# 07350100647/nvbio-gpl

Measured on AMD Instinct MI355X. Metric: aligned reads/sec (150 bp single-end, 3 Gbp ref); GCUPS of the banded extend pass in `extend`, higher is better.
Workload: dtype u32 (FM-index coordinates) / i16x2 (band-31 DP, two alignments per 32-bit lane: 16-bit integer scores, held in binary16 lanes where every score is an integer of magnitude <= 2040 -- exact -- and in int16 lanes otherwise; bound-checked on the host)

## Files before the change

### include/nvbio_amd.h

```cpp
#ifndef NVBIO_AMD_H
#define NVBIO_AMD_H

#include <stdint.h>

#ifdef __cplusplus
extern "C" {
#endif

#define NVBIO_AMD_VERSION 100

typedef enum
{
    NVBIO_OK              = 0,
    NVBIO_ERR_INVALID     = 1,
    NVBIO_ERR_HIP         = 2,
    NVBIO_ERR_NOMEM       = 3,
    NVBIO_ERR_UNSUPPORTED = 4,
    NVBIO_ERR_NO_DEVICE   = 5
} nvbio_status;

int         nvbio_amd_version(void);
const char* nvbio_amd_last_error(void);
nvbio_status nvbio_amd_device_count(int* count);
nvbio_status nvbio_amd_device_arch(int device, char* name, uint32_t name_len);
// ... 350 lines not shown
nvbio_status nvbio_best_approx_init(int device, uint32_t n_reads, int32_t worst_score, int32_t* best_dev, uint8_t* best_rc_dev, void* stream);
nvbio_status nvbio_read_queue_begin(int device, const uint32_t* queue_dev, uint32_t n, uint32_t read_len, uint32_t first_offset, uint32_t top_seed,
                                    uint32_t max_effort_init, uint32_t* seed_offsets_dev, uint32_t* active_dev, uint32_t* trys_dev, void* stream);
nvbio_status nvbio_read_queue_filter(int device, const uint32_t* queue_dev, uint32_t n, const uint8_t* read_flags_dev, uint32_t* queue_out_dev,
                                     uint32_t* count_dev, void* stream);

typedef struct
{
    const uint32_t* read_offsets_dev;
    const uint32_t* seed_intervals_dev;
    uint32_t        seeds_per_read;
    uint32_t        seeding_pass;
    uint32_t        max_reseed;
    uint32_t        seed_len;
    uint32_t        min_read_len;
} nvbio_ragged_seed_layout;

nvbio_status nvbio_read_queue_begin_ragged(int device, const uint32_t* queue_dev, uint32_t n, const nvbio_ragged_seed_layout* layout, uint32_t n_symbols,
                                           uint32_t top_seed, uint32_t max_effort_init, uint32_t* seed_offsets_dev, uint32_t* active_dev, uint32_t* trys_dev,
                                           void* stream);
nvbio_status nvbio_seed_hits_map_ragged(int device, const nvbio_uint2* fw_ranges_dev, const nvbio_uint2* rc_ranges_dev, const uint32_t* read_queue_dev,
                                        uint32_t n_reads, const nvbio_ragged_seed_layout* layout, uint32_t max_hits, uint32_t rep_seeds,
                                        nvbio_uint2* deques_dev, uint32_t* sizes_dev, uint8_t* reseed_dev, void* stream);
nvbio_status nvbio_best_approx_init_ragged(int device, uint32_t n_reads, const int32_t* min_scores_dev, int32_t* best_dev, uint8_t* best_rc_dev, void* stream);
nvbio_status nvbio_score_reduce_effort_ragged(int device, const uint32_t* active_dev, const nvbio_hit_queues* hits, const uint32_t* read_offsets_dev,
                                              uint32_t n_ext, const nvbio_seed_hits_params* params, int32_t* best_dev, uint8_t* best_rc_dev,
                                              uint32_t* trys_dev, uint32_t* sizes_dev, void* stream);
nvbio_status nvbio_score_reduce_effort_multi_ragged(int device, const uint32_t* active_dev, uint32_t n_active, const uint32_t* hits_first_dev,
                                                    const uint32_t* hits_count_dev, const nvbio_hit_queues* hits, const uint32_t* read_offsets_dev,
                                                    uint32_t n_ext, const nvbio_seed_hits_params* params, int32_t* best_dev, uint8_t* best_rc_dev,
                                                    uint32_t* trys_dev, uint32_t* sizes_dev, void* stream);

typedef struct
{
    uint32_t seeds_per_read;
    uint32_t first_offset;
    uint32_t seed_interval;
    uint32_t seed_len;
    uint32_t read_len;
} nvbio_all_hits_params;

nvbio_status nvbio_all_hits_scan_temp_bytes(uint32_t n_reads, uint32_t seeds_per_read, uint64_t* bytes);
nvbio_status nvbio_all_hits_scan(int device, const nvbio_uint2* fw_ranges_dev, const nvbio_uint2* rc_ranges_dev, uint32_t n_reads,
                                 const nvbio_all_hits_params* params, uint64_t* slots_dev, uint64_t* n_hits_dev, void* temp_dev, uint64_t temp_bytes,
                                 void* stream);

nvbio_status nvbio_all_hits_select(int device, const nvbio_uint2* fw_ranges_dev, const nvbio_uint2* rc_ranges_dev, uint32_t n_reads,
                                   const nvbio_all_hits_params* params, const uint64_t* slots_dev, uint64_t begin, uint64_t end,
                                   const nvbio_hit_queues* hits, void* stream);

nvbio_status nvbio_all_hits_unique_temp_bytes(uint32_t n, uint64_t* bytes);
nvbio_status nvbio_all_hits_unique(int device, const nvbio_hit_queues* hits, const nvbio_hit_queues* hits_out, uint32_t* n_out_dev, void* temp_dev,
                                   uint64_t temp_bytes, void* stream);

nvbio_status nvbio_all_score_output_temp_bytes(uint32_t n, uint64_t* bytes);
nvbio_status nvbio_all_score_output(int device, const nvbio_hit_queues* hits, const int32_t* scores_dev, int32_t min_score, uint32_t* out_read_id_dev,
                                    uint8_t* out_rc_dev, uint32_t* out_loc_dev, int32_t* out_score_dev, uint64_t out_offset, uint64_t out_capacity,
                                    uint64_t* count_dev, void* temp_dev, uint64_t temp_bytes, void* stream);

nvbio_status nvbio_all_traceback_flatten(int device, const uint32_t* rec_read_id_dev, const uint8_t* rec_rc_dev, const uint32_t* rec_loc_dev, uint32_t n,
                                         const uint32_t* read_index_dev, uint32_t band_len, uint32_t genome_len, uint32_t reads_reversed,
                                         uint32_t* read_id_dev, uint8_t* flags_dev, uint32_t* win_begin_dev, uint32_t* win_end_dev, void* stream);

typedef struct
{
    uint32_t anchor;
    uint32_t anchor_len, opposite_len;
    int32_t  anchor_perfect_score, opposite_perfect_score;
    int32_t  anchor_min_score, opposite_min_score;
    int32_t  score_limit;
    int32_t  worst_score;
    int32_t  match, txt_gap_open, txt_gap_ext;
    uint32_t band, genome_len;
    uint32_t policy, min_frag_len, max_frag_len, overlap, unpaired;
    uint32_t max_effort, min_ext, max_ext;
} nvbio_pe_params;
nvbio_status nvbio_pe_init(int device, uint32_t n_reads, int32_t worst_score_mate1, int32_t worst_score_mate2, int32_t* best_a_dev, int32_t* best_o_dev, void* stream);
nvbio_status nvbio_pe_anchor_flatten(int device, const nvbio_pe_params* params, const nvbio_hit_queues* hits, const int32_t* best_a_dev, const int32_t* best_o_dev,
                                     uint32_t* read_id_dev, uint8_t* flags_dev, uint32_t* win_begin_dev, uint32_t* win_end_dev, int32_t* min_scores_dev,
                                     void* stream);
nvbio_status nvbio_pe_anchor_output(int device, const nvbio_pe_params* params, const nvbio_hit_queues* hits, const int32_t* scores_dev, const nvbio_uint2* sinks_dev,
                                    const uint32_t* win_begin_dev, const int32_t* min_scores_dev, int32_t* hit_opposite_score_dev, uint8_t* valid_dev,
                                    void* stream);
nvbio_status nvbio_pe_opposite_flatten(int device, const nvbio_pe_params* params, const uint32_t* queue_dev, uint32_t n, const nvbio_hit_queues* hits,
                                       const int32_t* best_a_dev, const int32_t* best_o_dev, uint32_t* read_id_dev, uint8_t* flags_dev,
                                       uint32_t* win_begin_dev, uint32_t* win_end_dev, int32_t* min_scores_dev, void* stream);
nvbio_status nvbio_pe_opposite_output(int device, const nvbio_pe_params* params, const uint32_t* queue_dev, uint32_t n, const int32_t* scores_dev,
                                      const nvbio_uint2* sinks_dev, const uint32_t* win_begin_dev, const uint32_t* win_end_dev, const int32_t* min_scores_dev,
                                      int32_t* hit_opposite_score_dev, uint32_t* hit_opposite_loc_dev, uint32_t* hit_opposite_sink_dev, void* stream);
nvbio_status nvbio_pe_score_reduce(int device, const nvbio_pe_params* params, const uint32_t* active_dev, uint32_t n_active, const uint32_t* hits_first_dev,
                                   const uint32_t* hits_count_dev, const nvbio_hit_queues* hits, const int32_t* hit_opposite_score_dev,
                                   const uint32_t* hit_opposite_loc_dev, const uint32_t* hit_opposite_sink_dev, uint32_t n_ext, int32_t* best_a_dev,
                                   int32_t* best_o_dev, uint32_t* trys_dev, uint32_t* sizes_dev, void* stream);
nvbio_status nvbio_select_flagged_indices(int device, const uint8_t* flags_dev, uint32_t n, uint32_t* queue_out_dev, uint32_t* count_dev, void* stream);

nvbio_status nvbio_text_2bit_le_to_be(int device, const uint32_t* in_dev, uint32_t n_words, uint32_t* out_dev, void* stream);
nvbio_status nvbio_scores_to_int16(int device, const int32_t* scores_dev, uint32_t n, int16_t* out_dev, void* stream);

typedef enum { NVBIO_GLOBAL = 0, NVBIO_LOCAL = 1, NVBIO_SEMI_GLOBAL = 2 } nvbio_alignment_type;

typedef struct
{
    int32_t match;
    int32_t mm_min, mm_max;
    int32_t pat_gap_open, pat_gap_ext;
    int32_t txt_gap_open, txt_gap_ext;
} nvbio_gotoh_scheme;

typedef struct
{
    int32_t match, mismatch, deletion, insertion;
} nvbio_sw_scheme;

#define NVBIO_SCORE_MIN (-(1 << 30))

typedef struct
{
    const void*     reads_dev;
    uint32_t        read_bits;
    const uint32_t* read_offsets_dev;
    const uint8_t*  quals_dev;
    const uint32_t* read_id_dev;
    const uint8_t*  flags_dev;
    const void*     text_dev;
    uint32_t        text_bits;
    const uint32_t* win_begin_dev;
    const uint32_t* win_end_dev;
    uint32_t        n;
    uint32_t        max_read_len;
    uint32_t        algo_flags;
} nvbio_alignment_batch;


enum
{
    NVBIO_ALN_NO_UNGAPPED_SCORE     = 1,
    NVBIO_ALN_NO_THIRD_CHANCE       = 2,
    NVBIO_ALN_NO_PACKED_DP          = 4,
    NVBIO_ALN_FORCE_PACKED_DP       = 8,
    NVBIO_ALN_NO_UNGAPPED_TRACEBACK = 16,
    NVBIO_ALN_PK_THREE_WAVES        = 32,
    NVBIO_ALN_NO_SECOND_CHANCE      = 128,
    NVBIO_ALN_NO_NARROW_SCORE       = 512,
    NVBIO_ALN_NO_BAND_ROUTE         = 1024,
    NVBIO_ALN_PK_STRIPE8            = 256,
    NVBIO_ALN_RAGGED_READS          = 4096,
    NVBIO_ALN_NO_LENGTH_SORT        = 8192,
    NVBIO_ALN_NO_QUALITY_SHORTCUT   = 2048,
    NVBIO_ALN_NO_GAP_CHANCE         = 65536,
    NVBIO_ALN_NO_COOPERATIVE_DP     = 32768,
    NVBIO_ALN_NO_F16_DP             = 16384,
    NVBIO_ALN_SPLIT_CHANCES         = 131072,
    NVBIO_ALN_NO_PAIRED_GAP_CHANCE  = 262144,
    NVBIO_ALN_NO_NARROW_TRACEBACK   = 64
};

enum { NVBIO_READ_REVERSE = 1, NVBIO_READ_COMPLEMENT = 2 };

nvbio_status nvbio_best_candidate_reduce(int device, const uint64_t* keys_dev, const int32_t* scores_dev, const nvbio_uint2* sinks_dev,
                                         const uint32_t* win_begin_dev, uint64_t n, uint64_t* best_dev, void* stream);

nvbio_status nvbio_best_candidate_unpack(int device, const uint64_t* best_dev, uint32_t n_reads, int32_t* scores_dev,
                                         int64_t* end_pos_dev, uint8_t* rc_dev, void* stream);

nvbio_status nvbio_best_candidate_windows(int device, const uint64_t* keys_dev, const int32_t* scores_dev, const nvbio_uint2* sinks_dev,
                                          const uint32_t* win_begin_dev, uint64_t n, const uint64_t* best_dev, int64_t* best_wb_dev,
                                          int64_t* best_locus_dev, void* stream);

nvbio_status nvbio_traceback_best_batch(int device, const uint64_t* best_dev, const int64_t* best_wb_dev, uint32_t n_reads, uint32_t read_len,
                                        uint32_t band, uint32_t genome_len, int32_t min_score, uint8_t* flags_dev, uint32_t* win_begin_dev,
                                        uint32_t* win_end_dev, int32_t* scores_dev, nvbio_uint2* sinks_dev, void* stream);

nvbio_status nvbio_second_candidate_reduce(int device, const uint64_t* keys_dev, const int32_t* scores_dev, const nvbio_uint2* sinks_dev,
                                           const uint32_t* win_begin_dev, uint64_t n, const uint64_t* best_dev,
                                           uint32_t distinct_dist, int32_t worst_score, uint64_t* second_dev, void* stream);

typedef struct
{
    int32_t version;
    int32_t monotone;
    int32_t perfect_score;
    int32_t min_score;
} nvbio_mapq_params;
nvbio_status nvbio_mapq(int device, const uint64_t* best_dev, const uint64_t* second_dev, uint32_t n_reads,
                        const nvbio_mapq_params* params, int32_t* second_scores_dev, uint8_t* mapq_dev, void* stream);

nvbio_status nvbio_finish_reads_tiles_per_group(uint32_t reads_per_tile, uint32_t* tiles_per_group);
nvbio_status nvbio_finish_reads(int device, const uint64_t* keys_dev, const int32_t* scores_dev, const nvbio_uint2* sinks_dev,
                                const uint32_t* win_begin_dev, uint64_t n, const uint32_t* tile_offsets_dev, uint32_t n_tiles,
                                uint32_t reads_per_tile, uint32_t n_reads, uint32_t distinct_dist, int32_t worst_score,
                                const nvbio_mapq_params* params, int32_t match, const uint32_t* read_offsets_dev, const int32_t* min_scores_dev,
                                uint64_t* best_dev, uint64_t* second_dev, int32_t* scores_out_dev, int64_t* end_pos_dev, uint8_t* rc_dev,
                                uint8_t* mapq_dev, int32_t* second_scores_dev, uint32_t* status_dev, void* stream);

enum { NVBIO_PE_POLICY_FF = 0, NVBIO_PE_POLICY_FR = 1, NVBIO_PE_POLICY_RF = 2, NVBIO_PE_POLICY_RR = 3 };
nvbio_status nvbio_opposite_mate_windows(int device, const uint32_t* g_pos_dev, const uint8_t* anchor_rc_dev, uint32_t n,
                                         uint32_t anchor_len, uint32_t opposite_gapped_len, uint32_t anchor, uint32_t policy,
                                         uint32_t min_frag_len, uint32_t max_frag_len, uint32_t overlap, uint32_t genome_len,
                                         uint32_t* win_begin_dev, uint32_t* win_end_dev, uint8_t* flags_dev, uint8_t* valid_dev,
                                         void* stream);

#define NVBIO_GAP_PAIR_MAX_SHIFT 5
nvbio_status nvbio_banded_gap_pairs(int device, const nvbio_alignment_batch* batch, uint32_t* partner_dev, void* stream);

nvbio_status nvbio_banded_gotoh_score(int device, uint32_t band, nvbio_alignment_type type,
                                      const nvbio_gotoh_scheme* scheme, const nvbio_alignment_batch* batch,
                                      int32_t* scores_dev, nvbio_uint2* sinks_dev, void* stream);

nvbio_status nvbio_banded_gotoh_score_staged(int device, uint32_t band, nvbio_alignment_type type,
                                             const nvbio_gotoh_scheme* scheme, const nvbio_alignment_batch* batch,
                                             const int32_t* min_scores_dev, int32_t min_score,
                                             int32_t* scores_dev, nvbio_uint2* sinks_dev, void* stream);

enum { NVBIO_TRACEBACK_SINKS_GIVEN = 1 };
nvbio_status nvbio_banded_gotoh_traceback_temp_bytes(const nvbio_alignment_batch* batch_host_sizes, uint32_t band, uint64_t* bytes);
nvbio_status nvbio_banded_gotoh_traceback(int device, uint32_t band, nvbio_alignment_type type,
                                          const nvbio_gotoh_scheme* scheme, const nvbio_alignment_batch* batch,
                                          int32_t* scores_dev, nvbio_uint2* sources_dev, nvbio_uint2* sinks_dev,
                                          uint16_t* cigars_dev, uint32_t cigar_stride, uint32_t* cigar_lens_dev,
                                          uint32_t flags, void* temp_dev, uint64_t temp_bytes, void* stream);

nvbio_status nvbio_banded_sw_traceback(int device, uint32_t band, nvbio_alignment_type type,
                                       const nvbio_sw_scheme* scheme, const nvbio_alignment_batch* batch,
                                       int32_t* scores_dev, nvbio_uint2* sources_dev, nvbio_uint2* sinks_dev,
                                       uint16_t* cigars_dev, uint32_t cigar_stride, uint32_t* cigar_lens_dev,
                                       uint32_t flags, void* temp_dev, uint64_t temp_bytes, void* stream);

nvbio_status nvbio_full_gotoh_traceback_temp_bytes(const nvbio_alignment_batch* batch_host_sizes, uint32_t max_pattern_len,
                                                   uint32_t max_text_len, uint64_t* bytes);
nvbio_status nvbio_full_gotoh_traceback(int device, nvbio_alignment_type type, const nvbio_gotoh_scheme* scheme,
                                        const nvbio_alignment_batch* batch, uint32_t max_pattern_len, uint32_t max_text_len,
                                        const int32_t* min_scores_dev,
                                        int32_t* scores_dev, nvbio_uint2* sources_dev, nvbio_uint2* sinks_dev,
                                        uint16_t* cigars_dev, uint32_t cigar_stride, uint32_t* cigar_lens_dev,
                                        uint32_t flags, void* temp_dev, uint64_t temp_bytes, void* stream);

nvbio_status nvbio_full_sw_traceback(int device, nvbio_alignment_type type, const nvbio_sw_scheme* scheme,
                                     const nvbio_alignment_batch* batch, uint32_t max_pattern_len, uint32_t max_text_len,
                                     const int32_t* min_scores_dev,
                                     int32_t* scores_dev, nvbio_uint2* sources_dev, nvbio_uint2* sinks_dev,
                                     uint16_t* cigars_dev, uint32_t cigar_stride, uint32_t* cigar_lens_dev,
                                     uint32_t flags, void* temp_dev, uint64_t temp_bytes, void* stream);

nvbio_status nvbio_finish_alignment(int device, const nvbio_alignment_batch* batch, const nvbio_uint2* sources_dev,
                                    const uint16_t* cigars_dev, uint32_t cigar_stride, const uint32_t* cigar_lens_dev,
                                    uint32_t* ed_dev, uint8_t* mds_dev, uint32_t mds_stride, uint32_t* mds_lens_dev, void* stream);

nvbio_status nvbio_full_gotoh_temp_bytes(const nvbio_alignment_batch* batch_host_sizes, uint32_t max_pattern_len,
                                         uint32_t max_text_len, int text_blocking, uint64_t* bytes);
nvbio_status nvbio_full_gotoh_score(int device, nvbio_alignment_type type, int text_blocking,
                                    const nvbio_gotoh_scheme* scheme, const nvbio_alignment_batch* batch,
                                    uint32_t max_pattern_len, uint32_t max_text_len,
                                    const int32_t* min_scores_dev, int32_t* scores_dev, nvbio_uint2* sinks_dev,
                                    void* temp_dev, uint64_t temp_bytes, void* stream);

nvbio_status nvbio_banded_myers_score(int device, uint32_t band, nvbio_alignment_type type, const nvbio_alignment_batch* batch, int32_t min_score,
                                      int32_t* scores_dev, nvbio_uint2* sinks_dev, void* stream);

nvbio_status nvbio_banded_gotoh_score_best2(int device, uint32_t band, nvbio_alignment_type type,
                                            const nvbio_gotoh_scheme* scheme, const nvbio_alignment_batch* batch, uint32_t distinct_dist,
                                            int32_t* scores_dev, nvbio_uint2* sinks_dev, int32_t* scores2_dev, nvbio_uint2* sinks2_dev,
                                            void* stream);
nvbio_status nvbio_full_gotoh_score_best2(int device, nvbio_alignment_type type, int text_blocking,
                                          const nvbio_gotoh_scheme* scheme, const nvbio_alignment_batch* batch,
                                          uint32_t max_pattern_len, uint32_t max_text_len, const int32_t* min_scores_dev,
                                          uint32_t distinct_dist, int32_t* scores_dev, nvbio_uint2* sinks_dev,
                                          int32_t* scores2_dev, nvbio_uint2* sinks2_dev, void* stream);

nvbio_status nvbio_banded_sw_score(int device, uint32_t band, nvbio_alignment_type type,
                                   const nvbio_sw_scheme* scheme, const nvbio_alignment_batch* batch,
                                   int32_t* scores_dev, nvbio_uint2* sinks_dev, void* stream);
nvbio_status nvbio_full_sw_score(int device, nvbio_alignment_type type, int text_blocking,
                                 const nvbio_sw_scheme* scheme, const nvbio_alignment_batch* batch,
                                 uint32_t max_pattern_len, uint32_t max_text_len,
                                 const int32_t* min_scores_dev, int32_t* scores_dev, nvbio_uint2* sinks_dev,
                                 void* temp_dev, uint64_t temp_bytes, void* stream);

#ifdef __cplusplus
}
#endif
#endif
```

### nvbio-gpl_amd/__init__.py

```python
import ctypes
import os

import numpy as np

_HERE = os.path.dirname(os.path.abspath(__file__))
LIB_PATH = os.path.join(_HERE, "lib", "libnvbio_amd.so")
HEADER_PATH = os.path.join(os.path.dirname(_HERE), "include", "nvbio_amd.h")

GLOBAL, LOCAL, SEMI_GLOBAL = 0, 1, 2
SCORE_MIN = -(1 << 30)
FM_SCAN_FORWARD, FM_COMPLEMENT, FM_NO_KMER_TABLE, FM_NO_VERIFY, FM_COUNT_SECTORS, FM_NO_PIPELINE, FM_DEFER_HEAVY = 1, 2, 4, 8, 16, 32, 64
FM_TABLE_NO_DIRECT, FM_TABLE_NO_CONTEXT, FM_TABLE_NO_GROUPS, FM_TABLE_CANONICAL, FM_TABLE_CANONICAL_WIDE = 1, 2, 4, 8, 16
READ_REVERSE, READ_COMPLEMENT = 1, 2
TRACEBACK_SINKS_GIVEN = 1
ALN_NO_UNGAPPED_SCORE, ALN_NO_THIRD_CHANCE, ALN_NO_PACKED_DP, ALN_FORCE_PACKED_DP, ALN_NO_UNGAPPED_TRACEBACK, ALN_PK_THREE_WAVES = 1, 2, 4, 8, 16, 32
ALN_NO_NARROW_TRACEBACK, ALN_NO_SECOND_CHANCE, ALN_PK_STRIPE8, ALN_NO_NARROW_SCORE, ALN_NO_BAND_ROUTE = 64, 128, 256, 512, 1024
ALN_NO_QUALITY_SHORTCUT, ALN_RAGGED_READS, ALN_NO_LENGTH_SORT, ALN_NO_F16_DP, ALN_NO_COOPERATIVE_DP, ALN_NO_GAP_CHANCE = 2048, 4096, 8192, 16384, 32768, 65536
ALN_SPLIT_CHANCES, ALN_NO_PAIRED_GAP_CHANCE = 131072, 262144
DEFAULT_ALGO_FLAGS = 0
BACKTRACK_REFERENCE_QUIRKS = 1

_STATUS = {0: "OK", 1: "INVALID", 2: "HIP", 3: "NOMEM", 4: "UNSUPPORTED", 5: "NO_DEVICE"}


class NvbioError(RuntimeError):
    def __init__(self, status, msg):
        super().__init__("nvbio_amd: %s: %s" % (_STATUS.get(status, status), msg))
        self.status = status


class _View(ctypes.Structure):
    _fields_ = [("length", ctypes.c_uint32), ("primary", ctypes.c_uint32), ("L2", ctypes.c_uint32 * 5),
                ("bwt_occ_dev", ctypes.c_void_p), ("bwt_occ_words", ctypes.c_uint64),
                ("ssa_dev", ctypes.c_void_p), ("ssa_words", ctypes.c_uint64), ("sa_int", ctypes.c_uint32)]


class _BuildOptions(ctypes.Structure):
    _fields_ = [("kmer_len", ctypes.c_uint32), ("sa_int", ctypes.c_uint32), ("max_lcp", ctypes.c_uint32),
                ("verify", ctypes.c_uint32), ("table_flags", ctypes.c_uint32), ("bucket_symbols", ctypes.c_uint32)]


class _StringSet(ctypes.Structure):
    _fields_ = [("symbols_dev", ctypes.c_void_p), ("symbol_bits", ctypes.c_uint32),
                ("offsets_dev", ctypes.c_void_p), ("offsets_are_ranges", ctypes.c_uint32),
                ("fixed_len", ctypes.c_uint32), ("stride", ctypes.c_uint32), ("n", ctypes.c_uint32),
                ("seeds_per_string", ctypes.c_uint32), ("seed_interval", ctypes.c_uint32),
                ("seed_intervals_dev", ctypes.c_void_p)]


class _Scheme(ctypes.Structure):
    _fields_ = [("match", ctypes.c_int32), ("mm_min", ctypes.c_int32), ("mm_max", ctypes.c_int32),
                ("pat_gap_open", ctypes.c_int32), ("pat_gap_ext", ctypes.c_int32),
                ("txt_gap_open", ctypes.c_int32), ("txt_gap_ext", ctypes.c_int32)]


class _SWScheme(ctypes.Structure):
    _fields_ = [("match", ctypes.c_int32), ("mismatch", ctypes.c_int32), ("deletion", ctypes.c_int32),
                ("insertion", ctypes.c_int32)]


class _Batch(ctypes.Structure):
    _fields_ = [("reads_dev", ctypes.c_void_p), ("read_bits", ctypes.c_uint32),
                ("read_offsets_dev", ctypes.c_void_p), ("quals_dev", ctypes.c_void_p),
                ("read_id_dev", ctypes.c_void_p), ("flags_dev", ctypes.c_void_p),
                ("text_dev", ctypes.c_void_p), ("text_bits", ctypes.c_uint32),
                ("win_begin_dev", ctypes.c_void_p), ("win_end_dev", ctypes.c_void_p), ("n", ctypes.c_uint32),
                ("max_read_len", ctypes.c_uint32), ("algo_flags", ctypes.c_uint32)]


class _HitQueues(ctypes.Structure):
    _fields_ = [("idx_queue_dev", ctypes.c_void_p), ("hit_read_id_dev", ctypes.c_void_p), ("hit_seed_dev", ctypes.c_void_p),
                ("hit_loc_dev", ctypes.c_void_p), ("hit_score_dev", ctypes.c_void_p), ("hit_sink_dev", ctypes.c_void_p),
                ("n", ctypes.c_uint32)]


class _SeedHitsParams(ctypes.Structure):
    _fields_ = [(n, ctypes.c_uint32) for n in ("seeds_per_read", "first_offset", "seed_interval", "seed_len", "read_len", "max_hits",
                                                "rep_seeds", "max_effort", "min_ext", "max_ext")]


class _RaggedSeedLayout(ctypes.Structure):
    _fields_ = [("read_offsets_dev", ctypes.c_void_p), ("seed_intervals_dev", ctypes.c_void_p)] + \
               [(n, ctypes.c_uint32) for n in ("seeds_per_read", "seeding_pass", "max_reseed", "seed_len", "min_read_len")]


class _RankDict(ctypes.Structure):
    _fields_ = [("text_dev", ctypes.c_void_p), ("word_bits", ctypes.c_uint32), ("occ_dev", ctypes.c_void_p), ("index_bits", ctypes.c_uint32),
                ("K", ctypes.c_uint32), ("length", ctypes.c_uint64)]


_lib = None


def lib():
    global _lib
    if _lib is None:
        if not os.path.exists(LIB_PATH):
            raise NvbioError(5, "%s is missing: build it with __graft_entry__.build() "
                                "(there is no CPU fallback)" % LIB_PATH)
        import torch
        L = ctypes.CDLL(LIB_PATH)
        L.nvbio_amd_last_error.restype = ctypes.c_char_p
        L.nvbio_amd_version.restype = ctypes.c_int
        _lib = L
    return _lib


def release_scratch():
    _check(lib().nvbio_amd_release_scratch())


def set_scratch_check(enable, fill_byte=0):
    _check(lib().nvbio_amd_set_scratch_check(ctypes.c_int(1 if enable else 0), ctypes.c_uint32(fill_byte)))


def scratch_check_report():
    buf = ctypes.create_string_buffer(1 << 16)
    _check(lib().nvbio_amd_scratch_check_report(buf, ctypes.c_uint64(len(buf))))
    out = {}
    for line in buf.value.decode().splitlines():
        tag, checked, damaged, sub, off = line.split()
        out[tag] = (int(checked), int(damaged), None if sub == "-" else int(sub), None if off == "-" else int(off))
    return out


def _check(status):
    if status != 0:
        raise NvbioError(status, lib().nvbio_amd_last_error().decode())


def _torch():
    import torch
    return torch


_SCRATCH = {}


def _scratch(device, nbytes, cap=8 << 30):
    torch = _torch()
    nbytes = int(min(max(nbytes, 1 << 20), cap))
    key = str(device)
    t = _SCRATCH.get(key)
    if t is None or t.numel() < nbytes:
        _SCRATCH[key] = None
        t = _SCRATCH[key] = torch.empty(nbytes, dtype=torch.uint8, device=device)
    return t


def _ptr(t):
    return None if t is None else ctypes.c_void_p(t.data_ptr())


def _stream_ptr(device):
    torch = _torch()
    return ctypes.c_void_p(torch.cuda.current_stream(device).cuda_stream)


def device_count():
    n = ctypes.c_int(0)
    lib().nvbio_amd_device_count(ctypes.byref(n))
    return n.value


def _dev_tensor(a, dtype, device):
    torch = _torch()
    if a is None:
        return None
    if isinstance(a, torch.Tensor):
        t = a
        if t.dtype != dtype:
# ... 733 lines not shown
        cols = 4 if self._index.IS_SET else 2
        if hits is None:
            hits = torch.empty((max(end - begin, 0), cols), dtype=torch.int32, device=self._index.device)
        if end > begin:
            _check(lib().nvbio_qgram_filter_locate(self._index._h, _ptr(self._ranges), _ptr(self._slots), _ptr(self._indices),
                                                   ctypes.c_uint32(self._n_queries), ctypes.c_uint64(begin), ctypes.c_uint64(end), _ptr(hits),
                                                   _stream_ptr(self._index.device)))
        return hits

    def merge(self, interval, hits, is_set=None):
        torch = _torch()
        if is_set is None:
            is_set = hits.dim() == 2 and hits.shape[1] == 4
        dev = hits.device
        n = hits.shape[0]
        tb = ctypes.c_uint64(0)
        _check(lib().nvbio_qgram_filter_merge_temp_bytes(ctypes.c_int(1 if is_set else 0), ctypes.c_uint32(n), ctypes.byref(tb)))
        self._grow_temp(tb.value, dev)
        if self._merged is None or self._merged.shape[0] < max(n, 1) or self._merged.device != dev:
            self._merged = torch.empty((max(n, 1), 2), dtype=torch.int32, device=dev)
            self._counts = torch.empty(max(n, 1), dtype=torch.int32, device=dev)
        nm = ctypes.c_uint32(0)
        hits = hits.contiguous()
        _check(lib().nvbio_qgram_filter_merge(FMIndex._dev_index(dev), ctypes.c_int(1 if is_set else 0), ctypes.c_uint32(interval), _ptr(hits),
                                              ctypes.c_uint32(n), _ptr(self._merged), _ptr(self._counts), ctypes.byref(nm), _ptr(self._temp),
                                              ctypes.c_uint64(self._temp.numel()), _stream_ptr(dev)))
        m = nm.value
        merged = self._merged.view(-1)[:2 * m].view(m, 2) if is_set else self._merged.view(-1)[:m]
        return merged.clone(), self._counts[:m].clone()


class GotohScheme:

    def __init__(self, match, mm_min, mm_max, pat_gap_open, pat_gap_ext, txt_gap_open, txt_gap_ext):
        self.c = _Scheme(match, mm_min, mm_max, pat_gap_open, pat_gap_ext, txt_gap_open, txt_gap_ext)


def SimpleGotohScheme(match, mismatch, gap_open, gap_ext):
    return GotohScheme(match, -mismatch, -mismatch, gap_open, gap_ext, gap_open, gap_ext)


def EditDistanceScheme():
    return GotohScheme(0, 1, 1, -1, -1, -1, -1)


class SimpleSmithWatermanScheme:

    def __init__(self, match, mismatch, deletion, insertion):
        self.c = _SWScheme(match, mismatch, deletion, insertion)


class SmithWatermanAligner:

    def __init__(self, type, scheme):
        self.type, self.sw = type, scheme
        c = scheme.c
        self.scheme = (GotohScheme(c.match, -c.mismatch, -c.mismatch, c.deletion, c.deletion, c.deletion, c.deletion)
                       if c.deletion == c.insertion else None)


def make_smith_waterman_aligner(type, scheme):
    return SmithWatermanAligner(type, scheme)


def make_edit_distance_aligner(type):
    return SmithWatermanAligner(type, SimpleSmithWatermanScheme(0, -1, -1, -1))


class GotohAligner:

    def __init__(self, type, scheme):
        self.type, self.scheme = type, scheme


def make_gotoh_aligner(type, scheme):
    return GotohAligner(type, scheme)


class AlignmentBatch:

    def __init__(self, reads, read_bits, read_offsets, text, text_bits, win_begin, win_end, quals=None, read_id=None,
                 flags=None, device="cuda:0", max_read_len=0, algo_flags=None):
        torch = _torch()
        self.device = device
        self.algo_flags = DEFAULT_ALGO_FLAGS if algo_flags is None else int(algo_flags)
        self.read_bits, self.text_bits = int(read_bits), int(text_bits)
        self.reads = _dev_tensor(reads, torch.uint8 if read_bits == 8 else torch.int32, device)
        self.read_offsets = _dev_tensor(read_offsets, torch.int32, device)
        self.text = _dev_tensor(text, torch.uint8 if text_bits == 8 else torch.int32, device)
        self.win_begin = _dev_tensor(win_begin, torch.int32, device)
        self.win_end = _dev_tensor(win_end, torch.int32, device)
        self.quals = _dev_tensor(quals, torch.uint8, device)
        self.read_id = _dev_tensor(read_id, torch.int32, device)
        self.flags = _dev_tensor(flags, torch.uint8, device)
        self.n = int(self.win_begin.numel())
        self.max_read_len = int(max_read_len)

    def size(self):
        return self.n

    def c_struct(self):
        return _Batch(_ptr(self.reads), self.read_bits, _ptr(self.read_offsets), _ptr(self.quals), _ptr(self.read_id),
                      _ptr(self.flags), _ptr(self.text), self.text_bits, _ptr(self.win_begin), _ptr(self.win_end),
                      self.n, self.max_read_len, self.algo_flags)


DEVICE_THREAD_SCHEDULER = "DeviceThreadScheduler"
DEVICE_STAGED_THREAD_SCHEDULER = "DeviceStagedThreadScheduler"


class BatchedBandedAlignmentScore:

    def __init__(self, band_len, aligner, scheduler=DEVICE_THREAD_SCHEDULER):
        self.band_len, self.aligner, self.scheduler = int(band_len), aligner, scheduler
        if scheduler not in (DEVICE_THREAD_SCHEDULER, DEVICE_STAGED_THREAD_SCHEDULER):
            raise NvbioError(1, "unknown scheduler %r" % (scheduler,))

    def min_temp_storage(self, max_pattern_len, max_text_len, stream_size):
        return 0

    max_temp_storage = min_temp_storage

    def enact(self, batch, scores=None, sinks=None, min_scores=None):
        torch = _torch()
        if scores is None:
            scores = torch.empty(batch.n, dtype=torch.int32, device=batch.device)
        if sinks is None:
            sinks = torch.empty((batch.n, 2), dtype=torch.int32, device=batch.device)
        bs = batch.c_struct()
        sw = getattr(self.aligner, "sw", None)
        if self.scheduler == DEVICE_STAGED_THREAD_SCHEDULER:
            if sw is not None:
                raise NvbioError(4, "the staged scheduler is instantiated for Gotoh aligners")
            per_job = min_scores is not None and not isinstance(min_scores, int)
            if per_job and (min_scores.dtype != torch.int32 or min_scores.numel() != batch.n):
                raise NvbioError(1, "min_scores: int32 per job")
            _check(lib().nvbio_banded_gotoh_score_staged(
                FMIndex._dev_index(batch.device), ctypes.c_uint32(self.band_len), ctypes.c_int(self.aligner.type),
                ctypes.byref(self.aligner.scheme.c), ctypes.byref(bs), _ptr(min_scores) if per_job else None,
                ctypes.c_int32(SCORE_MIN if min_scores is None else (0 if per_job else int(min_scores))),
                _ptr(scores), _ptr(sinks), _stream_ptr(batch.device)))
            return scores, sinks
        fn = lib().nvbio_banded_sw_score if sw is not None else lib().nvbio_banded_gotoh_score
        _check(fn(FMIndex._dev_index(batch.device), ctypes.c_uint32(self.band_len), ctypes.c_int(self.aligner.type),
                  ctypes.byref(sw.c if sw is not None else self.aligner.scheme.c),
                  ctypes.byref(bs), _ptr(scores), _ptr(sinks), _stream_ptr(batch.device)))
        return scores, sinks


def batch_banded_alignment_score(band_len, aligner, batch):
    return BatchedBandedAlignmentScore(band_len, aligner).enact(batch)


GAP_PAIR_MAX_SHIFT = 5
NO_PARTNER = 0xFFFFFFFF


def banded_gap_pairs(batch):
    torch = _torch()
    partner = torch.empty(batch.n, dtype=torch.int32, device=batch.device)
    bs = batch.c_struct()
    _check(lib().nvbio_banded_gap_pairs(FMIndex._dev_index(batch.device), ctypes.byref(bs), _ptr(partner), _stream_ptr(batch.device)))
    return partner


class BatchedBandedAlignmentTraceback:

    def __init__(self, band_len, aligner):
        self.band_len, self.aligner = int(band_len), aligner

    def min_temp_storage(self, batch):
        out = ctypes.c_uint64(0)
        bs = batch.c_struct()
        _check(lib().nvbio_banded_gotoh_traceback_temp_bytes(ctypes.byref(bs), ctypes.c_uint32(self.band_len), ctypes.byref(out)))
        return int(out.value)

    def enact(self, batch, cigar_stride=64, temp=None, scores=None, sinks=None):
        torch = _torch()
        n, dev = batch.n, batch.device
        given = scores is not None and sinks is not None
        if not given:
            scores = torch.empty(n, dtype=torch.int32, device=dev)
            sinks = torch.empty((n, 2), dtype=torch.int32, device=dev)
        sources = torch.empty((n, 2), dtype=torch.int32, device=dev)
        cigars = torch.zeros((n, cigar_stride), dtype=torch.int16, device=dev)
        lens = torch.empty(n, dtype=torch.int32, device=dev)
        bs = batch.c_struct()
        sw = getattr(self.aligner, "sw", None)
        fn = lib().nvbio_banded_sw_traceback if sw is not None else lib().nvbio_banded_gotoh_traceback
        _check(fn(
            FMIndex._dev_index(dev), ctypes.c_uint32(self.band_len), ctypes.c_int(self.aligner.type),
            ctypes.byref(sw.c if sw is not None else self.aligner.scheme.c), ctypes.byref(bs), _ptr(scores), _ptr(sources), _ptr(sinks), _ptr(cigars),
            ctypes.c_uint32(cigar_stride), _ptr(lens), ctypes.c_uint32(TRACEBACK_SINKS_GIVEN if given else 0), _ptr(temp),
            ctypes.c_uint64(0 if temp is None else temp.numel() * temp.element_size()), _stream_ptr(dev)))
        return scores, sources, sinks, cigars, lens


class BatchedAlignmentTraceback:

    def __init__(self, aligner):
        self.aligner = aligner

    def min_temp_storage(self, batch, max_pattern_len, max_text_len):
        out = ctypes.c_uint64(0)
        bs = batch.c_struct()
        _check(lib().nvbio_full_gotoh_traceback_temp_bytes(ctypes.byref(bs), ctypes.c_uint32(max_pattern_len),
                                                           ctypes.c_uint32(max_text_len), ctypes.byref(out)))
        return int(out.value)

    def enact(self, batch, max_pattern_len, max_text_len, min_scores=None, cigar_stride=64, temp=None, scores=None, sinks=None):
        torch = _torch()
        n, dev = batch.n, batch.device
        given = scores is not None and sinks is not None
        if not given:
            scores = torch.empty(n, dtype=torch.int32, device=dev)
            sinks = torch.empty((n, 2), dtype=torch.int32, device=dev)
        sources = torch.empty((n, 2), dtype=torch.int32, device=dev)
        cigars = torch.zeros((n, cigar_stride), dtype=torch.int16, device=dev)
        lens = torch.empty(n, dtype=torch.int32, device=dev)
        ms = _dev_tensor(min_scores, torch.int32, dev)
        bs = batch.c_struct()
        if temp is None and n:
            temp = _scratch(dev, self.min_temp_storage(batch, max_pattern_len, max_text_len))
        sw = getattr(self.aligner, "sw", None)
        fn = lib().nvbio_full_sw_traceback if sw is not None else lib().nvbio_full_gotoh_traceback
        _check(fn(
            FMIndex._dev_index(dev), ctypes.c_int(self.aligner.type), ctypes.byref(sw.c if sw is not None else self.aligner.scheme.c), ctypes.byref(bs),
            ctypes.c_uint32(max_pattern_len), ctypes.c_uint32(max_text_len), _ptr(ms), _ptr(scores), _ptr(sources), _ptr(sinks),
            _ptr(cigars), ctypes.c_uint32(cigar_stride), _ptr(lens), ctypes.c_uint32(TRACEBACK_SINKS_GIVEN if given else 0),
            _ptr(temp), ctypes.c_uint64(0 if temp is None else temp.numel() * temp.element_size()), _stream_ptr(dev)))
        return scores, sources, sinks, cigars, lens


def finish_alignment(batch, sources, cigars, cigar_lens, mds_stride=0):
    torch = _torch()
    n, dev = batch.n, batch.device
    ed = torch.empty(n, dtype=torch.int32, device=dev)
    mds = torch.zeros((n, mds_stride), dtype=torch.uint8, device=dev) if mds_stride else None
    ml = torch.empty(n, dtype=torch.int32, device=dev) if mds_stride else None
    bs = batch.c_struct()
    _check(lib().nvbio_finish_alignment(FMIndex._dev_index(dev), ctypes.byref(bs), _ptr(sources), _ptr(cigars), ctypes.c_uint32(cigars.shape[1]),
                                        _ptr(cigar_lens), _ptr(ed), _ptr(mds), ctypes.c_uint32(mds_stride), _ptr(ml), _stream_ptr(dev)))
    return ed, mds, ml


def cigar_string(cigar_row, length, forward=True):
    els = [int(c) & 0xFFFF for c in cigar_row[:length]]
    if forward:
        els = els[::-1]
    return "".join("%d%s" % (c >> 2, "MIDS"[c & 3]) for c in els)


class BatchedAlignmentScore:

    def __init__(self, aligner, text_blocking=True):
        self.aligner, self.text_blocking = aligner, bool(text_blocking)

    def enact(self, batch, max_pattern_len, max_text_len, min_scores=None, scores=None, sinks=None):
        torch = _torch()
        if scores is None:
            scores = torch.empty(batch.n, dtype=torch.int32, device=batch.device)
        if sinks is None:
            sinks = torch.empty((batch.n, 2), dtype=torch.int32, device=batch.device)
        ms = _dev_tensor(min_scores, torch.int32, batch.device)
        bs = batch.c_struct()
        sw = getattr(self.aligner, "sw", None)
        fn = lib().nvbio_full_sw_score if sw is not None else lib().nvbio_full_gotoh_score
        rows = max_pattern_len if self.text_blocking else max_text_len
        temp = _scratch(batch.device, batch.n * max(rows, 1) * 4)
        _check(fn(FMIndex._dev_index(batch.device), ctypes.c_int(self.aligner.type),
                  ctypes.c_int(1 if self.text_blocking else 0),
                  ctypes.byref(sw.c if sw is not None else self.aligner.scheme.c), ctypes.byref(bs),
                  ctypes.c_uint32(max_pattern_len), ctypes.c_uint32(max_text_len), _ptr(ms),
                  _ptr(scores), _ptr(sinks), _ptr(temp), ctypes.c_uint64(temp.numel()), _stream_ptr(batch.device)))
        return scores, sinks


def batch_banded_alignment_score_best2(band_len, aligner, batch, distinct_dist=0):
    torch = _torch()
    sc = [torch.empty(batch.n, dtype=torch.int32, device=batch.device) for _ in range(2)]
    sk = [torch.empty((batch.n, 2), dtype=torch.int32, device=batch.device) for _ in range(2)]
    bs = batch.c_struct()
    _check(lib().nvbio_banded_gotoh_score_best2(FMIndex._dev_index(batch.device), ctypes.c_uint32(band_len), ctypes.c_int(aligner.type),
                                                ctypes.byref(aligner.scheme.c), ctypes.byref(bs), ctypes.c_uint32(distinct_dist),
                                                _ptr(sc[0]), _ptr(sk[0]), _ptr(sc[1]), _ptr(sk[1]), _stream_ptr(batch.device)))
    return sc[0], sk[0], sc[1], sk[1]


def batch_alignment_score_best2(aligner, batch, max_pattern_len, max_text_len, distinct_dist=0, text_blocking=False, min_scores=None):
    torch = _torch()
    sc = [torch.empty(batch.n, dtype=torch.int32, device=batch.device) for _ in range(2)]
    sk = [torch.empty((batch.n, 2), dtype=torch.int32, device=batch.device) for _ in range(2)]
    ms = _dev_tensor(min_scores, torch.int32, batch.device)
    bs = batch.c_struct()
    _check(lib().nvbio_full_gotoh_score_best2(FMIndex._dev_index(batch.device), ctypes.c_int(aligner.type), ctypes.c_int(1 if text_blocking else 0),
                                              ctypes.byref(aligner.scheme.c), ctypes.byref(bs), ctypes.c_uint32(max_pattern_len),
                                              ctypes.c_uint32(max_text_len), _ptr(ms), ctypes.c_uint32(distinct_dist),
                                              _ptr(sc[0]), _ptr(sk[0]), _ptr(sc[1]), _ptr(sk[1]), _stream_ptr(batch.device)))
    return sc[0], sk[0], sc[1], sk[1]


def hits_to_diagonals(hits, seeds_per_read, seed_interval, seed_len, read_len, strand):
    torch = _torch()
    keys = torch.empty(hits.shape[0], dtype=torch.int64, device=hits.device)
    _check(lib().nvbio_hits_to_diagonals(FMIndex._dev_index(hits.device), _ptr(hits), ctypes.c_uint64(hits.shape[0]),
                                         ctypes.c_uint32(seeds_per_read), ctypes.c_uint32(seed_interval),
# ... 503 lines not shown
```

### nvbio-gpl_amd/csrc/gotoh_banded.hip

```cpp
#include "gotoh_common.h"
#include "bitplanes.h"
#include <hipcub/hipcub.hpp>
#include <stdlib.h>

namespace nvbio_amd {

template <int BAND, int TYPE, int RBITS, int TBITS, bool BEST2 = false, bool STAGED = false>
__global__ void __launch_bounds__(128)
banded_gotoh_kernel(const BatchDev b, const SchemeDev sc, int32_t* __restrict__ scores, uint2* __restrict__ sinks,
                    const uint32_t distinct_dist, int32_t* __restrict__ scores2, uint2* __restrict__ sinks2,
                    const int32_t* __restrict__ min_scores, const int32_t min_score_all)
{
    __shared__ int32_t s_mm[64];
    if (threadIdx.x < 64) s_mm[threadIdx.x] = mismatch_score( sc, threadIdx.x );
    __syncthreads();

    const uint32_t job = blockIdx.x * blockDim.x + threadIdx.x;
    if (job >= b.n) return;

    const uint32_t rid   = b.read_id ? b.read_id[job] : job;
    const uint32_t first = b.read_offsets[rid];
    const uint32_t M     = b.read_offsets[rid + 1] - first;
    const uint32_t fl    = b.flags ? b.flags[job] : 0u;
    const bool     rev   = (fl & NVBIO_READ_REVERSE) != 0;
// ... 34 lines not shown
    }

    const int32_t G_o = sc.pat_go, G_e = sc.pat_ge;
    const int32_t I_o = sc.ins_go, I_e = sc.ins_ge;
    const int32_t infimum = -32768 - max2( max2( G_o, G_e ), max2( sc.txt_go, sc.txt_ge ) );
    const int32_t V = sc.match;

    int32_t H[BAND], F[BAND];
    H[0] = 0;
    #pragma unroll
    for (int j = 1; j < BAND; ++j) H[j] = (TYPE == NVBIO_GLOBAL) ? sc.txt_go + (j - 1) * sc.txt_ge : 0;
    #pragma unroll
    for (int j = 0; j < BAND; ++j) F[j] = infimum;

    bool stopped = false;
    const int32_t min_score = STAGED ? (min_scores ? min_scores[job] : min_score_all) : 0;
    for (uint32_t i = 0; i < M; ++i)
    {
        if (STAGED && i && (i & 31u) == 0u)
        {
            int32_t mx = H[0];
            #pragma unroll
            for (int j = 1; j < BAND; ++j) mx = max2( mx, H[j] );
            const int32_t thr = (int32_t)((uint32_t)min_score + (M - i) * (uint32_t)V);
            if (mx < thr) { stopped = true; break; }
            #pragma unroll
            for (int j = 0; j < BAND; ++j)
            {
                H[j] = (int32_t)(int16_t)max2( H[j], -32768 + 32 );
                F[j] = (int32_t)(int16_t)max2( F[j], -32768 + 32 );
            }
        }
        const uint32_t pidx = rev ? first + M - 1u - i : first + i;
        uint32_t q = prd.get( pidx );
        if (comp && q < 4u) q = 3u - q;
        const uint32_t qq = b.quals ? b.quals[pidx] : 0u;
        const int32_t  S  = s_mm[qq < 63u ? qq : 63u];

        const uint32_t g_new = (i + (uint32_t)(BAND - 1) < N) ? trd.get( tb + i + (BAND - 1) ) : 255u;

        uint64_t eq_bits = 0;
        if (PACKED)
        {
            if (q < 4u)
            {
                const uint64_t t = cache_bits ^ ((uint64_t)q * 0x5555555555555555ull);
                eq_bits = ~(t | (t >> 1)) & 0x5555555555555555ull;
            }
        }

        int32_t E = 0;
        int32_t row_key = -1;
        #pragma unroll
        for (int j = 0; j < BAND; ++j)
        {
            const int32_t f = (j < BAND - 1) ? max2( F[j + 1] + G_e, H[j + 1] + G_o ) : infimum;
            F[j] = f;

            bool eq;
            if (j == BAND - 1)   eq = (g_new == q);
            else if (PACKED)     eq = ((eq_bits >> (2 * j)) & 1ull) != 0;
            else                 eq = (cache_raw[j] == q);
            const int32_t d = H[j] + (eq ? V : S);

            int32_t h;
            if (j == 0)             h = max2( f, d );
            else if (j == BAND - 1) h = max2( E, d );
            else                    h = max3( f, E, d );
            if (TYPE == NVBIO_LOCAL)
            {
                h = max2( h, 0 );
                if (BEST2) report2( h, i + (uint32_t)j + 1u, i + 1u );
                else       row_key = max2( row_key, (h << 5) | j );
            }
            H[j] = h;
            E = (j == 0) ? h + I_o : max2( h + I_o, E + I_e );
        }

        if (PACKED) cache_bits = (cache_bits >> 2) | ((uint64_t)(g_new & 3u) << (2 * (BAND - 2)));
        else
        {
            #pragma unroll
            for (int j = 0; j < BAND - 2; ++j) cache_raw[j] = cache_raw[j + 1];
            cache_raw[BAND - 2] = g_new;
        }

        if (TYPE == NVBIO_LOCAL && !BEST2)
        {
            const int32_t h = row_key >> 5;
            if (h >= best) { best = h; best_x = i + (uint32_t)(row_key & 31) + 1u; best_y = i + 1u; }
        }
    }

    if (STAGED && stopped) {  }
    else if (TYPE == NVBIO_GLOBAL)
    {
        if (BEST2) report2( H[BAND - 1], M + BAND - 1, M );
        else if (best <= H[BAND - 1]) { best = H[BAND - 1]; best_x = M + BAND - 1; best_y = M; }
    }
    else if (TYPE == NVBIO_SEMI_GLOBAL)
    {
        const uint32_t mb = M + (uint32_t)(BAND - 1);
        const uint32_t m  = (mb < N ? mb : N) - (M - 1u);
        #pragma unroll
        for (int j = 0; j < BAND; ++j)
            if (j == 0 || (uint32_t)j < m)
            {
                if (BEST2) report2( H[j], M + j, M );
                else if (best <= H[j]) { best = H[j]; best_x = M + j; best_y = M; }
            }
    }
    scores[job] = best;
    sinks[job]  = make_uint2( best_x, best_y );
    if (BEST2) { scores2[job] = sec; sinks2[job] = make_uint2( sec_x, sec_y ); }
}

typedef short    v2s __attribute__((ext_vector_type(2)));
typedef unsigned short v2u __attribute__((ext_vector_type(2)));

__device__ __forceinline__ v2s pk(const int a, const int b) { v2s r; r.x = (short)a; r.y = (short)b; return r; }
__device__ __forceinline__ v2s pk_max(const v2s a, const v2s b) { return __builtin_elementwise_max( a, b ); }
__device__ __forceinline__ v2s pk_from_bits(const uint32_t u) { return __builtin_bit_cast( v2s, u ); }
typedef _Float16 v2h __attribute__((ext_vector_type(2)));
__device__ __forceinline__ v2h pk_max(const v2h a, const v2h b) { return __builtin_elementwise_maximum( a, b ); }
__device__ __forceinline__ v2s pk_max3(const v2s a, const v2s b, const v2s c) { return pk_max( pk_max( a, b ), c ); }
__device__ __forceinline__ v2h pk_max3(const v2h a, const v2h b, const v2h c) { return __builtin_elementwise_maximum( __builtin_elementwise_maximum( a, b ), c ); }
template <typename V> __device__ __forceinline__ V pk_of(const int a, const int b);
template <> __device__ __forceinline__ v2s pk_of<v2s>(const int a, const int b) { return pk( a, b ); }
template <> __device__ __forceinline__ v2h pk_of<v2h>(const int a, const int b) { v2h r; r.x = (_Float16)a; r.y = (_Float16)b; return r; }
template <bool FP> struct PkLanes { typedef v2s type; };
template <> struct PkLanes<true> { typedef v2h type; };

__device__ __forceinline__ uint32_t funnel32(const uint32_t a, const uint32_t b, const uint32_t bit)
{
    const uint32_t sh = bit & 31u;
    return sh ? ((a << sh) | (b >> (32u - sh))) : a;
}
__device__ __forceinline__ uint32_t clamp_u32(const int64_t v, const uint32_t lo, const uint32_t hi)
{
    return v < (int64_t)lo ? lo : (v > (int64_t)hi ? hi : (uint32_t)v);
}

__device__ __forceinline__ uint32_t even_bits64(uint64_t x)
{
    x &= 0x5555555555555555ull;
    x = (x | (x >> 1)) & 0x3333333333333333ull;
    x = (x | (x >> 2)) & 0x0F0F0F0F0F0F0F0Full;
    x = (x | (x >> 4)) & 0x00FF00FF00FF00FFull;
    x = (x | (x >> 8)) & 0x0000FFFF0000FFFFull;
    x = (x | (x >> 16));
    return (uint32_t)x;
}

template <int TYPE, int RBITS, int MINW = 3, bool M0 = false, bool RAGGED = false, bool FP = false>
__global__ void __launch_bounds__(128) __attribute__((amdgpu_waves_per_eu(MINW, 3)))
banded_gotoh_band31_pk_kernel(const BatchDev b, const SchemeDev sc, int32_t* __restrict__ scores, uint2* __restrict__ sinks,
                              const uint32_t* __restrict__ job_list, const uint32_t* __restrict__ job_count)
{
    constexpr int BAND = 31;
    constexpr uint32_t RMASK = (1u << RBITS) - 1u;
    static_assert( !FP || (M0 && TYPE != NVBIO_LOCAL), "the binary16 build: match = 0, GLOBAL / SEMI_GLOBAL" );
    typedef typename PkLanes<FP>::type v2;
    __shared__ int32_t s_mm[64];
    if (threadIdx.x < 64) s_mm[threadIdx.x] = mismatch_score( sc, threadIdx.x );
    __syncthreads();

    const uint32_t n_jobs = job_list ? *job_count : b.n;
    const uint32_t pair = blockIdx.x * blockDim.x + threadIdx.x;
    if (2u * pair >= n_jobs) return;
    const uint32_t* __restrict__ rwords = (const uint32_t*)b.reads;
    const uint32_t* __restrict__ twords = (const uint32_t*)b.text;

    uint32_t first[2], M[2], tb[2], N[2], rows_all[2], out_id[2];
    bool     rev[2], comp[2], valid[2];
    #pragma unroll
    for (int u = 0; u < 2; ++u)
    {
        const uint32_t slot = 2u * pair + u;
        valid[u] = slot < n_jobs;
        const uint32_t ss  = valid[u] ? slot : 2u * pair;
        const uint32_t jj  = job_list ? job_list[ss] : ss;
        out_id[u] = jj;
        const uint32_t rid = b.read_id ? b.read_id[jj] : jj;
        first[u] = b.read_offsets[rid];
        M[u]     = b.read_offsets[rid + 1] - first[u];
        const uint32_t fl = b.flags ? b.flags[jj] : 0u;
        rev[u]  = (fl & NVBIO_READ_REVERSE) != 0;
        comp[u] = (fl & NVBIO_READ_COMPLEMENT) != 0;
        tb[u]   = b.win_begin[jj];
        N[u]    = (b.max_read_len && M[u] > b.max_read_len) ? 0u : b.win_end[jj] - tb[u];
        rows_all[u] = (valid[u] && N[u] >= M[u]) ? M[u] : 0u;
    }

    uint32_t r_lo[2], r_hi[2], t_lo[2], t_hi[2];
    #pragma unroll
    for (int u = 0; u < 2; ++u)
    {
        r_lo[u] = (uint32_t)(((uint64_t)first[u] * RBITS) >> 5);
        r_hi[u] = (uint32_t)(((uint64_t)(first[u] + (M[u] ? M[u] - 1u : 0u)) * RBITS) >> 5);
        t_lo[u] = tb[u] >> 4;
        t_hi[u] = (tb[u] + (N[u] ? N[u] - 1u : 0u)) >> 4;
    }

    auto read_chunk_start = [&](const int u, const uint32_t r0) -> int64_t {
        return rev[u] ? (int64_t)first[u] + (int64_t)M[u] - 1 - (int64_t)r0 - 7 : (int64_t)first[u] + r0;
    };
    auto read_chunk_start_at = [&](const int u, const int64_t r0) -> int64_t {
        return rev[u] ? (int64_t)first[u] + (int64_t)M[u] - 1 - r0 - 7 : (int64_t)first[u] + r0;
    };

    const uint32_t qadj = (uint32_t)((uintptr_t)b.quals & 3u);
    const uint32_t* __restrict__ qwords = (const uint32_t*)((uintptr_t)b.quals - qadj);
    const bool has_quals = (b.quals != nullptr);

    const v2 GO = pk_of<v2>( sc.pat_go, sc.pat_go ), GE = pk_of<v2>( sc.pat_ge, sc.pat_ge );
    const v2 INF = pk_of<v2>( -16384, -16384 ), ZERO = pk_of<v2>( 0, 0 );
    const v2s K32 = pk( 32, 32 );
    const int V = sc.match;
    const int S_noq = s_mm[0];
    uint32_t cx[2], lim[2];
    #pragma unroll
    for (int u = 0; u < 2; ++u)
    {
        cx[u]  = comp[u] ? 3u : 0u;
        lim[u] = N[u] > (uint32_t)(BAND - 1) ? N[u] - (uint32_t)(BAND - 1) : 0u;
    }

    int32_t  best[2]   = { NVBIO_SCORE_MIN, NVBIO_SCORE_MIN };
    uint32_t best_x[2] = { 0xFFFFFFFFu, 0xFFFFFFFFu }, best_y[2] = { 0xFFFFFFFFu, 0xFFFFFFFFu };

    const bool want0 = valid[0] && N[0] >= M[0], want1 = valid[1] && N[1] >= M[1];
    const bool split = (TYPE != NVBIO_LOCAL) && !RAGGED && want0 && want1 && M[0] != M[1];
    const uint32_t rows_max = rows_all[0] > rows_all[1] ? rows_all[0] : rows_all[1];
    uint32_t pad[2] = { 0u, 0u };
    if (RAGGED && TYPE != NVBIO_LOCAL) { pad[0] = rows_max - rows_all[0]; pad[1] = rows_max - rows_all[1]; }

    for (int pass = 0; pass < (split ? 2 : 1); ++pass)
    {
        uint32_t rows_u[2];
        rows_u[0] = (split && pass != 0) ? 0u : rows_all[0];
        rows_u[1] = (split && pass != 1) ? 0u : rows_all[1];
        const uint32_t rows = rows_u[0] > rows_u[1] ? rows_u[0] : rows_u[1];

        uint32_t c0[2], c1[2], c0i[2] = { 0, 0 }, c1i[2] = { 0, 0 };
        #pragma unroll
        for (int u = 0; u < 2; ++u)
        {
            const uint32_t w  = tb[u] >> 4;
            const uint32_t w0 = twords[clamp_u32( w,      t_lo[u], t_hi[u] )];
            const uint32_t w1 = twords[clamp_u32( w + 1u, t_lo[u], t_hi[u] )];
            const uint32_t w2 = twords[clamp_u32( w + 2u, t_lo[u], t_hi[u] )];
            const uint32_t bit = (tb[u] & 15u) * 2u;
            const uint64_t hi = ((uint64_t)funnel32( w0, w1, bit ) << 32) | funnel32( w1, w2, bit );
            uint64_t c = hi & ~0xFull;
            if (N[u] < 30u) c |= (~0ull >> (2u * N[u])) & ~0xFull;
            c0[u] = even_bits64( c ) >> 2;
            c1[u] = even_bits64( c >> 1 ) >> 2;
            if (RAGGED) { c0i[u] = c0[u]; c1i[u] = c1[u]; }
        }

        uint32_t ra[2], rb[2], ta[2], tbw[2];
        uint32_t qa[2] = { 0, 0 }, qb[2] = { 0, 0 }, qc[2] = { 0, 0 };
        auto issue_loads = [&](const uint32_t r0) {
            if (has_quals)
            {
                #pragma unroll
                for (int u = 0; u < 2; ++u)
                {
                    const int64_t qw  = ((RAGGED ? read_chunk_start_at( u, (int64_t)r0 - pad[u] ) : read_chunk_start( u, r0 )) + qadj) >> 2;
                    const uint32_t lo = (first[u] + qadj) >> 2, hi = (first[u] + qadj + (M[u] ? M[u] - 1u : 0u)) >> 2;
                    qa[u] = qwords[clamp_u32( qw,     lo, hi )];
                    qb[u] = qwords[clamp_u32( qw + 1, lo, hi )];
                    qc[u] = qwords[clamp_u32( qw + 2, lo, hi )];
                }
            }
            #pragma unroll
            for (int u = 0; u < 2; ++u)
            {
                const int64_t  rbit = (RAGGED ? read_chunk_start_at( u, (int64_t)r0 - pad[u] ) : read_chunk_start( u, r0 )) * RBITS;
                const int64_t  rw   = rbit >> 5;
                ra[u]  = rwords[clamp_u32( rw,     r_lo[u], r_hi[u] )];
                rb[u]  = rwords[clamp_u32( rw + 1, r_lo[u], r_hi[u] )];
                const int64_t  tw   = RAGGED ? (((int64_t)tb[u] + (int64_t)r0 - pad[u] + (BAND - 1)) >> 4)
                                             : (int64_t)(((uint64_t)tb[u] + r0 + (BAND - 1)) >> 4);
                ta[u]  = twords[clamp_u32( tw,     t_lo[u], t_hi[u] )];
                tbw[u] = twords[clamp_u32( tw + 1, t_lo[u], t_hi[u] )];
            }
        };
        issue_loads( 0 );

        v2 H[BAND], Hg[BAND], F[BAND];
        #pragma unroll
        for (int j = 0; j < BAND; ++j)
        {
            const int h0 = (TYPE == NVBIO_GLOBAL && j > 0) ? sc.txt_go + (j - 1) * sc.txt_ge : 0;
            H[j] = pk_of<v2>( h0, h0 ); F[j] = INF; Hg[j] = H[j] + GO;
        }

        for (uint32_t r0 = 0; r0 < rows; r0 += 8u)
        {
            uint32_t rchunk[2], tchunk[2], tchunk1[2]; int rsh[2], rstep[2];
            uint64_t qchunk[2] = { 0, 0 }; int qsh[2], qstep[2];
            #pragma unroll
            for (int u = 0; u < 2; ++u)
            {
                if (has_quals)
                {
                    const uint32_t bs = ((uint32_t)(((RAGGED ? read_chunk_start_at( u, (int64_t)r0 - pad[u] ) : read_chunk_start( u, r0 )) + qadj) & 3)) * 8u;
                    const uint32_t lo = bs ? ((qa[u] >> bs) | (qb[u] << (32u - bs))) : qa[u];
                    const uint32_t hi = bs ? ((qb[u] >> bs) | (qc[u] << (32u - bs))) : qb[u];
                    qchunk[u] = ((uint64_t)hi << 32) | lo;
                }
                qsh[u] = rev[u] ? 56 : 0; qstep[u] = rev[u] ? -8 : 8;
                const int64_t rbit = (RAGGED ? read_chunk_start_at( u, (int64_t)r0 - pad[u] ) : read_chunk_start( u, r0 )) * RBITS;
                rchunk[u] = funnel32( ra[u], rb[u], (uint32_t)(rbit & 31) );
                rsh[u]    = rev[u] ? (32 - RBITS) - 7 * RBITS : (32 - RBITS);
                rstep[u]  = rev[u] ? RBITS : -RBITS;
                const uint32_t tsym = RAGGED ? (uint32_t)(((int64_t)tb[u] + (int64_t)r0 - pad[u] + (BAND - 1)) & 15)
                                             : (uint32_t)(((uint64_t)tb[u] + r0 + (BAND - 1)) & 15u);
                uint32_t tc = funnel32( ta[u], tbw[u], tsym * 2u );
                const int64_t kk = RAGGED ? (int64_t)N[u] - (int64_t)(BAND - 1) - ((int64_t)r0 - pad[u]) : (int64_t)N[u] - (int64_t)(BAND - 1) - (int64_t)r0;
                if (kk < 16) tc |= (kk <= 0) ? 0xFFFFFFFFu : (0xFFFFFFFFu >> (2u * (uint32_t)kk));
                tchunk[u]  = tc;
                tchunk1[u] = tc << 1;
            }
            if (r0 + 8u < rows) issue_loads( r0 + 8u );

            const uint32_t r_end = (r0 + 8u < rows) ? 8u : rows - r0;
            for (uint32_t t = 0; t < r_end; ++t)
            {
                const uint32_t i = r0 + t;
                if (RAGGED && TYPE != NVBIO_LOCAL)
                {
                    const bool s0 = pad[0] != 0u && i == pad[0], s1 = pad[1] != 0u && i == pad[1];
                    if (s0 || s1)
                    {
                        #pragma unroll
                        for (int j = 0; j < BAND; ++j)
                        {
                            const int h0 = (TYPE == NVBIO_GLOBAL && j > 0) ? sc.txt_go + (j - 1) * sc.txt_ge : 0;
                            const v2 hh = pk_of<v2>( h0, h0 ), hhg = pk_of<v2>( h0 + sc.pat_go, h0 + sc.pat_go );
                            if (s0) { H[j].x = hh.x; F[j].x = INF.x; Hg[j].x = hhg.x; }
                            if (s1) { H[j].y = hh.y; F[j].y = INF.y; Hg[j].y = hhg.y; }
                        }
                        if (s0) { c0[0] = c0i[0]; c1[0] = c1i[0]; }
                        if (s1) { c0[1] = c0i[1]; c1[1] = c1i[1]; }
                    }
                }
                uint32_t nq[2]; int S[2];
                if (has_quals)
                {
                    #pragma unroll
                    for (int u = 0; u < 2; ++u)
                    {
                        const uint32_t ql = (uint32_t)(qchunk[u] >> qsh[u]) & 0xFFu; qsh[u] += qstep[u];
                        S[u] = s_mm[ql < 63u ? ql : 63u];
                    }
                }
                else S[0] = S[1] = S_noq;
                #pragma unroll
                for (int u = 0; u < 2; ++u)
                {
                    const uint32_t q = ((rchunk[u] >> rsh[u]) & RMASK) ^ cx[u]; rsh[u] += rstep[u];
                    c1[u] = __builtin_amdgcn_alignbit( c1[u], tchunk[u],  31 );
                    c0[u] = __builtin_amdgcn_alignbit( c0[u], tchunk1[u], 31 );
                    tchunk[u] <<= 2; tchunk1[u] <<= 2;
                    uint32_t x = (c0[u] ^ (0u - (q & 1u))) | (c1[u] ^ (0u - ((q >> 1) & 1u)));
                    if (RBITS > 2 && q >= 4u) x = 0xFFFFFFFFu;
                    if (i >= (RAGGED ? lim[u] + pad[u] : lim[u])) x |= 1u;
                    nq[u] = x;
                }
                const uint32_t NWa = __builtin_amdgcn_perm( nq[1], nq[0], 0x05040100u );
                const uint32_t NWb = __builtin_amdgcn_perm( nq[1], nq[0], 0x07060302u );

                const v2 SS = FP ? pk_of<v2>( S[0] * 128, S[1] * 128 ) : pk_of<v2>( S[0], S[1] );
                const v2 SD = pk_of<v2>( S[0] - V, S[1] - V );
                const v2 VV = pk_of<v2>( V, V );
                auto flags_at = [&](const int j) -> uint32_t {
                    const uint32_t w = (j < 15) ? NWb : NWa;
                    const int bit = (j < 15) ? 14 - j : 30 - j;
                    const int to  = FP ? 13 : 0;
                    return bit >= to ? w >> (bit - to) : w << (to - bit);
                };
                auto flags_in = [&](const uint32_t q) -> v2 { return __builtin_bit_cast( v2, q & (FP ? 0x20002000u : 0x00010001u) ); };
                auto flags_of = [&](const int j) -> v2 { return flags_in( flags_at( j ) ); };
                auto diag_of = [&](const v2 h, const v2 t) -> v2 {
                    if (FP) return __builtin_bit_cast( v2, __builtin_elementwise_fma( __builtin_bit_cast( v2h, t ), __builtin_bit_cast( v2h, SS ), __builtin_bit_cast( v2h, h ) ) );
                    return M0 ? h + t * SS : (h + VV) + t * SD;
                };

                v2 E = ZERO, a = ZERO, tt, ff = INF, dd = ZERO;
                v2s key = pk( -1, -1 );
                {
                    const v2 x  = F[1] + GE;
                    const v2 t0 = flags_of( 0 );
                    const v2 d  = diag_of( H[0], t0 );
                    const v2 f  = pk_max( x, Hg[1] );
                    F[0] = f;
                    if (FP) { ff = f; dd = d; tt = ZERO; }
                    else
                    {
                        tt = pk_max( f, d );
                        if (TYPE == NVBIO_LOCAL) tt = pk_max( tt, ZERO );
                    }
                }
                #pragma unroll
                for (int j = 0; j < BAND; ++j)
                {
                    constexpr int Z = 0;
                    const int j1 = j + 1, j2 = j + 2;
                    v2 x = INF, d = ZERO, f = INF, t1 = ZERO, tn = ZERO, an = ZERO;
                    uint32_t q1 = 0;
                    if (j2 < BAND) x  = F[j2] + GE;
                    __builtin_amdgcn_sched_barrier( Z );
                    const v2 h = FP ? ((j == 0) ? pk_max( ff, dd ) : pk_max3( ff, dd, E )) : ((j == 0) ? tt : pk_max( tt, E ));
                    if (j1 < BAND) q1 = flags_at( j1 );
                    __builtin_amdgcn_sched_barrier( Z );
                    const v2 hg = h + GO;
                    if (!FP && j1 < BAND) t1 = flags_in( q1 );
                    if (j2 < BAND) f  = pk_max( x, Hg[j2] );
                    __builtin_amdgcn_sched_barrier( Z );
                    const v2 En = (j == 0) ? hg : pk_max( hg, a );
                    if (FP) __builtin_amdgcn_sched_barrier( Z );
                    if (FP && j1 < BAND) t1 = flags_in( q1 );
                    if (j1 < BAND) d  = diag_of( H[j1], t1 );
                    __builtin_amdgcn_sched_barrier( Z );
                    if (j1 < BAND) an = En + GE;
                    if (TYPE == NVBIO_LOCAL) key = pk_max( key, __builtin_bit_cast( v2s, h ) * K32 + pk( j, j ) );
                    __builtin_amdgcn_sched_barrier( Z );
                    if (j1 < BAND)
                    {
                        if (FP) { ff = (j2 < BAND) ? f : d; dd = d; }
                        else
                        {
                            tn = (j2 < BAND) ? pk_max( f, d ) : d;
                            if (TYPE == NVBIO_LOCAL) tn = pk_max( tn, ZERO );
                        }
                        F[j1] = f;
                    }
                    H[j] = h; Hg[j] = hg;
                    E = En; a = an; tt = tn;
                    __builtin_amdgcn_sched_barrier( Z );
                }

                if (TYPE == NVBIO_LOCAL)
                {
                    const int k0 = key.x, k1 = key.y;
                    if (i < rows_u[0] && (k0 >> 5) >= best[0]) { best[0] = k0 >> 5; best_x[0] = i + (uint32_t)(k0 & 31) + 1u; best_y[0] = i + 1u; }
                    if (i < rows_u[1] && (k1 >> 5) >= best[1]) { best[1] = k1 >> 5; best_x[1] = i + (uint32_t)(k1 & 31) + 1u; best_y[1] = i + 1u; }
                }
            }
        }

        if (TYPE != NVBIO_LOCAL)
        {
            #pragma unroll
            for (int u = 0; u < 2; ++u)
            {
                const bool active = (u ? want1 : want0) && (!split || u == pass);
                if (!active) continue;
                if (TYPE == NVBIO_GLOBAL)
                {
                    const int v = u ? (int)H[BAND - 1].y : (int)H[BAND - 1].x;
                    if (best[u] <= v) { best[u] = v; best_x[u] = M[u] + BAND - 1; best_y[u] = M[u]; }
                }
                else
                {
                    const uint32_t mb = M[u] + (uint32_t)(BAND - 1);
                    const uint32_t m  = (mb < N[u] ? mb : N[u]) - (M[u] - 1u);
                    #pragma unroll
                    for (int j = 0; j < BAND; ++j)
                        if (j == 0 || (uint32_t)j < m)
                        {
                            const int v = u ? (int)H[j].y : (int)H[j].x;
                            if (best[u] <= v) { best[u] = v; best_x[u] = M[u] + j; best_y[u] = M[u]; }
                        }
                }
            }
        }
    }
    #pragma unroll
    for (int u = 0; u < 2; ++u)
        if (valid[u]) { scores[out_id[u]] = best[u]; sinks[out_id[u]] = make_uint2( best_x[u], best_y[u] ); }
}

constexpr int GAP_CHANCE_GA = 5;
__host__ __device__ __forceinline__ int32_t gap_chance_unknown_cost(const int32_t P, const int32_t go, const int32_t ge)
{
    auto cg = [&](const int g) -> int32_t { return -(go + (g - 1) * ge); };
    int32_t c = cg( 1 ) + 3 * P;
    const int32_t others[] = { cg( GAP_CHANCE_GA + 1 ), 3 * cg( 1 ), 2 * cg( 1 ) + P, cg( 1 ) + cg( 3 ), 2 * cg( 2 ) };
    #pragma unroll
    for (int k = 0; k < 5; ++k) c = others[k] < c ? others[k] : c;
    return c;
}
struct GapLadder { int32_t c_unk_u, c_unk_n; };
static GapLadder gap_ladder(const int32_t P, const int32_t G, const int32_t go, const int32_t ge)
{
    const int64_t floor_u = 3 * (int64_t)(G < go ? G : go) - P;
    const int32_t cap = P > 0 ? (int32_t)((-floor_u - 1) / (int64_t)P) : 0;
    GapLadder l;
    l.c_unk_u = gap_chance_unknown_cost( P, go, ge );
    l.c_unk_n = (cap + 1) * P < l.c_unk_u ? (cap + 1) * P : l.c_unk_u;
    return l;
}

constexpr uint32_t JOB_COUNT_STRIDE = 32u;
constexpr uint32_t JOB_LIST_COUNT   = 4u;
#ifndef NVB_JOB_LIST_CHUNKS
#define NVB_JOB_LIST_CHUNKS 1
#endif
constexpr int JOB_LIST_CHUNKS = NVB_JOB_LIST_CHUNKS;
static inline uint32_t job_list_grid(const uint32_t n) { return (n + 256u * JOB_LIST_CHUNKS - 1u) / (256u * JOB_LIST_CHUNKS); }

struct JobLists { uint32_t *dp, *second, *third, *pairs; uint32_t* counts; };

template <int NL>
struct JobAppend
{
    static_assert( NL >= 1 && NL <= 4 && JOB_LIST_CHUNKS >= 1 && JOB_LIST_CHUNKS <= 4, "JobAppend: up to 4 lists, up to 4 chunks" );
    struct Lds { uint32_t cnt[NL][4 * JOB_LIST_CHUNKS]; uint32_t base[NL]; };
    static constexpr int SLOT = NL <= 3 ? 8 : 16;
    typedef typename std::conditional<NL <= 3, uint32_t, uint64_t>::type Mine;
    Mine mine = 0;
    __device__ __forceinline__ void note(Lds& lds, const int k, const int which)
    {
        const uint32_t lane = threadIdx.x & 63u, wave = threadIdx.x >> 6;
        #pragma unroll
        for (int l = 0; l < NL; ++l)
        {
            const uint64_t m = __ballot( which == l );
            if (lane == 0) lds.cnt[l][4 * k + wave] = (uint32_t)__popcll( m );
            if (which == l) mine |= (Mine)(((uint32_t)(l + 1) << 6) | (uint32_t)__popcll( m & ((1ull << lane) - 1ull) )) << (SLOT * k);
        }
    }
    template <typename JobOf>
    __device__ __forceinline__ void flush(Lds& lds, const JobLists& out, JobOf job_of)
    {
        __syncthreads();
        if (threadIdx.x < (uint32_t)NL)
        {
            uint32_t tot = 0;
            for (int i = 0; i < 4 * JOB_LIST_CHUNKS; ++i) { const uint32_t c = lds.cnt[threadIdx.x][i]; lds.cnt[threadIdx.x][i] = tot; tot += c; }
            lds.base[threadIdx.x] = tot ? atomicAdd( out.counts + JOB_COUNT_STRIDE * threadIdx.x, (unsigned int)tot ) : 0u;
        }
        __syncthreads();
        const uint32_t wave = threadIdx.x >> 6;
        #pragma unroll
        for (int k = 0; k < JOB_LIST_CHUNKS; ++k)
        {
            const uint32_t e = (uint32_t)(mine >> (SLOT * k)) & ((1u << SLOT) - 1u);
            if (e)
            {
                const uint32_t l = (e >> 6) - 1u;
                uint32_t* const list = l == 0u ? out.dp : (l == 1u ? out.second : (l == 2u ? out.third : out.pairs));
                list[lds.base[l] + lds.cnt[l][4 * k + wave] + (e & 63u)] = job_of( k );
            }
        }
    }
};

struct JobAppendTwo
{
    struct Lds { uint32_t cnt[2 * 4 * JOB_LIST_CHUNKS]; uint32_t base; };
    uint64_t mine = 0;
    __device__ __forceinline__ void note(Lds& lds, const int k, const bool first, const bool second)
    {
        const uint32_t lane = threadIdx.x & 63u, wave = threadIdx.x >> 6;
        #pragma unroll
        for (int r = 0; r < 2; ++r)
        {
            const bool on = r ? second : first;
            const uint64_t m = __ballot( on );
            if (lane == 0) lds.cnt[4 * (2 * k + r) + wave] = (uint32_t)__popcll( m );
            if (on) mine |= (uint64_t)(64u | (uint32_t)__popcll( m & ((1ull << lane) - 1ull) )) << (16 * k + 8 * r);
        }
    }
    template <typename JobOf>
    __device__ __forceinline__ void flush(Lds& lds, const JobLists& out, JobOf job_of)
    {
        __syncthreads();
        if (threadIdx.x == 0)
        {
            uint32_t tot = 0;
            for (int i = 0; i < 2 * 4 * JOB_LIST_CHUNKS; ++i) { const uint32_t c = lds.cnt[i]; lds.cnt[i] = tot; tot += c; }
            lds.base = tot ? atomicAdd( out.counts, (unsigned int)tot ) : 0u;
        }
        __syncthreads();
        const uint32_t wave = threadIdx.x >> 6;
        #pragma unroll
        for (int k = 0; k < JOB_LIST_CHUNKS; ++k)
            #pragma unroll
            for (int r = 0; r < 2; ++r)
            {
                const uint32_t e = (uint32_t)(mine >> (16 * k + 8 * r)) & 255u;
                if (e) out.dp[lds.base + lds.cnt[4 * (2 * k + r) + wave] + (e & 63u)] = job_of( k, r );
            }
    }
};

constexpr uint32_t PAIR_MAX_SHIFT = NVBIO_GAP_PAIR_MAX_SHIFT;

__device__ __forceinline__ int gap_pair_role(const BatchDev& b, const uint32_t job, const bool live)
{
    uint32_t rid = 0, fl = 0, tb = 0, whole = 0;
    if (live)
    {
        rid = b.read_id ? b.read_id[job] : job;
        const uint32_t M = b.read_offsets[rid + 1] - b.read_offsets[rid];
        fl = b.flags ? b.flags[job] : 0u;
        tb = b.win_begin[job];
        whole = (M >= 1u && M <= PLANE_MAX_READ && b.win_end[job] - tb == M + 31u) ? 1u : 0u;
    }
    const uint32_t lane = threadIdx.x & 63u;
    const uint32_t rid_n = __shfl_down( rid, 1 ), fl_n = __shfl_down( fl, 1 ), tb_n = __shfl_down( tb, 1 ), whole_n = __shfl_down( whole, 1 );
    const uint32_t shift = tb_n > tb ? tb_n - tb : tb - tb_n;
    const bool link = lane < 63u && whole && whole_n && rid_n == rid && fl_n == fl && shift >= 1u && shift <= PAIR_MAX_SHIFT;
    const uint64_t links = __ballot( link );
    const uint32_t run = lane ? (uint32_t)__clzll( (long long)~(links << (64u - lane)) ) : 0u;
    const bool lower = link && !(run & 1u);
    const uint64_t lowers = __ballot( lower );
    if (lower) return 1;
    return (lane && ((lowers >> (lane - 1u)) & 1ull)) ? -1 : 0;
}

__global__ void __launch_bounds__(256)
gap_pairs_kernel(const BatchDev b, uint32_t* __restrict__ partner)
{
    const uint32_t job = blockIdx.x * 256u + threadIdx.x;
    const int role = gap_pair_role( b, job, job < b.n );
    if (job < b.n) partner[job] = role ? (role > 0 ? job + 1u : job - 1u) : 0xFFFFFFFFu;
}

template <int RBITS, int MODE, bool QUAL>
__device__ __forceinline__ uint32_t
ungapped_e2e31_job(const BatchDev& b, const int32_t P, const int32_t G, const int32_t gap_open, const int32_t gap_ext,
                   int32_t* __restrict__ scores, uint2* __restrict__ sinks, const uint32_t job, const int32_t* s_pen)
{
    constexpr bool LIST = MODE != 0;
    const uint32_t rid   = b.read_id ? b.read_id[job] : job;
    const uint32_t first = b.read_offsets[rid];
    const uint32_t M     = b.read_offsets[rid + 1] - first;
    const uint32_t fl    = b.flags ? b.flags[job] : 0u;
    const bool     rev   = (fl & NVBIO_READ_REVERSE) != 0;
    const bool     comp  = (fl & NVBIO_READ_COMPLEMENT) != 0;
    const uint32_t tb    = b.win_begin[job];
    const uint32_t N     = (b.max_read_len && M > b.max_read_len) ? 0u : b.win_end[job] - tb;

    if (N < M)
    {
        scores[job] = NVBIO_SCORE_MIN; sinks[job] = make_uint2( 0xFFFFFFFFu, 0xFFFFFFFFu );
        return 0u;
    }
    if (M == 0u || M > 161u) return 1u;

    uint64_t rlo[3], rhi[3], rn[3], tlo[4], thi[4];
    {
        ReadWords<RBITS> rw; TextWords13 tw;
        load_read_words<RBITS>( b.reads, first, M, rw );
        load_text_words13( b.text, tb, N < 192u ? N : 192u, tw );
        read_planes192<RBITS>( rw, first, M, rev, comp, rlo, rhi, rn );
        text_planes208( tw, tb, tlo, thi );
    }
    uint64_t rmask[3];
    #pragma unroll
    for (int k = 0; k < 3; ++k)
    {
        const int32_t left = (int32_t)M - 64 * k;
        rmask[k] = left >= 64 ? ~0ull : (left > 0 ? ((1ull << left) - 1ull) : 0ull);
    }

    const uint32_t mb = M + 30u;
    const uint32_t m  = (mb < N ? mb : N) - (M - 1u);
    uint32_t pl[6], ph[6], pn[6], pm[6], ql[7], qh[7];
    #pragma unroll
    for (int k = 0; k < 3; ++k)
    {
        pl[2*k] = (uint32_t)rlo[k]; pl[2*k+1] = (uint32_t)(rlo[k] >> 32);
        ph[2*k] = (uint32_t)rhi[k]; ph[2*k+1] = (uint32_t)(rhi[k] >> 32);
        pm[2*k] = (uint32_t)rmask[k]; pm[2*k+1] = (uint32_t)(rmask[k] >> 32);
        pn[2*k] = (uint32_t)rn[k] & pm[2*k]; pn[2*k+1] = (uint32_t)(rn[k] >> 32) & pm[2*k+1];
    }
    #pragma unroll
    for (int k = 0; k < 3; ++k)
    {
        ql[2*k] = (uint32_t)tlo[k]; ql[2*k+1] = (uint32_t)(tlo[k] >> 32);
        qh[2*k] = (uint32_t)thi[k]; qh[2*k+1] = (uint32_t)(thi[k] >> 32);
    }
    ql[6] = (uint32_t)tlo[3]; qh[6] = (uint32_t)thi[3];
    uint32_t ql0[7], qh0[7];
    #pragma unroll
    for (int k = 0; k < 7; ++k) { ql0[k] = ql[k]; qh0[k] = qh[k]; }

    uint32_t best_cnt = 0xFFFFFFFFu, best_d = 0;
    int64_t U = 0;
    if (LIST)
    {
        U      = scores[job];
        best_d = sinks[job].x - M;
    }
    else
    {
        const int64_t floor_u = 3 * (int64_t)(G < gap_open ? G : gap_open) - P;
        const uint32_t cap = P > 0 ? (uint32_t)((-floor_u - 1) / (int64_t)P) : 0xFFFFFFFEu;
        uint32_t cnt_d[QUAL ? 31 : 1];
        #pragma unroll
        for (uint32_t d = 0; d < 31u; ++d)
        {
            const bool on = (d == 0u || d < m);
            uint32_t cnt;
            {
                const uint32_t tl = d ? __builtin_amdgcn_alignbit( ql0[1], ql0[0], d ) : ql0[0], th = d ? __builtin_amdgcn_alignbit( qh0[1], qh0[0], d ) : qh0[0];
                cnt = (uint32_t)__popc( (((pl[0] ^ tl) | (ph[0] ^ th)) & pm[0]) | pn[0] );
            }
            const uint32_t thr = QUAL ? cap : (best_cnt < cap ? best_cnt : cap);
            if (__any( on && cnt <= thr ))
            {
                #pragma unroll
                for (int k = 1; k < 6; ++k)
                {
                    const uint32_t tl = d ? __builtin_amdgcn_alignbit( ql0[k + 1], ql0[k], d ) : ql0[k], th = d ? __builtin_amdgcn_alignbit( qh0[k + 1], qh0[k], d ) : qh0[k];
                    cnt += (uint32_t)__popc( (((pl[k] ^ tl) | (ph[k] ^ th)) & pm[k]) | pn[k] );
                }
            }
            else cnt = 0xFFFFFFFFu;
            if (QUAL) cnt_d[d] = on ? cnt : 0xFFFFFFFFu;
            if (on && cnt <= best_cnt) { best_cnt = cnt; best_d = d; }
        }
        if (best_cnt > cap)
        {
            const bool gap_chance = !QUAL && P > 0 && N >= M + 30u && gap_ext < 0 && gap_open <= gap_ext && !(b.algo & NVBIO_ALN_NO_GAP_CHANCE);
            return gap_chance ? 4u : 1u;
        }
        U = -(int64_t)P * (int64_t)best_cnt;
        if (QUAL)
        {
            if (U <= 3 * (int64_t)G - P) return 1u;
            const uint32_t pmax  = (uint32_t)s_pen[63];
            const uint64_t bound = (uint64_t)pmax * best_cnt;
            uint32_t cand = 0;
            #pragma unroll
            for (uint32_t d = 0; d < 31u; ++d)
                if (cnt_d[d] != 0xFFFFFFFFu && (uint64_t)(uint32_t)P * cnt_d[d] <= bound) cand |= 1u << d;
            uint32_t best_w = 0xFFFFFFFFu;
            while (cand)
            {
                const uint32_t d = (uint32_t)__builtin_ctz( cand );
                cand &= cand - 1u;
                uint32_t w = 0;
                #pragma unroll
                for (int k = 0; k < 6; ++k)
                {
                    const uint32_t tl = __builtin_amdgcn_alignbit( ql0[k + 1], ql0[k], d ), th = __builtin_amdgcn_alignbit( qh0[k + 1], qh0[k], d );
                    uint32_t mm = (((pl[k] ^ tl) | (ph[k] ^ th)) & pm[k]) | pn[k];
                    while (mm)
                    {
                        const uint32_t row = 32u * k + (uint32_t)__builtin_ctz( mm );
                        mm &= mm - 1u;
                        const uint32_t qq = b.quals[rev ? first + M - 1u - row : first + row];
                        w += (uint32_t)s_pen[qq < 63u ? qq : 63u];
                    }
                }
                if (w <= best_w) { best_w = w; best_d = d; }
            }
            U = -(int64_t)best_w;
        }
    }
    bool settled = U > (int64_t)G;
    auto stash = [&]() { scores[job] = (int32_t)U; sinks[job] = make_uint2( M + best_d, M ); };
    const bool second_applies = !settled && (int64_t)G - P < U && 2 * (int64_t)G < U && N >= M + 30u && !(b.algo & NVBIO_ALN_NO_SECOND_CHANCE);
    if (MODE == 0 && second_applies)
    {
        int32_t gmax = 0;
        while (gmax < 5 && (int64_t)gap_open + (int64_t)gmax * gap_ext >= U) ++gmax;
        if (gmax >= 1 && gmax <= 4) { stash(); return 3u; }
    }
    if (MODE == 1 && second_applies)
    {
        int32_t gmax = 0;
        while (gmax < 5 && (int64_t)gap_open + (int64_t)gmax * gap_ext >= U) ++gmax;
        if (gmax >= 1 && gmax <= 4)
        {
            #pragma unroll
            for (int k = 0; k < 7; ++k) { ql[k] = ql0[k]; qh[k] = qh0[k]; }
            uint32_t lead_prev[4] = { 0, 0, 0, 0 }, tail_prev[4] = { 0, 0, 0, 0 };
            bool gapped = false;
            for (uint32_t d = 0; d < 31u && !gapped; ++d)
            {
                uint32_t first = M, last = 0xFFFFFFFFu;
                #pragma unroll
                for (int k = 0; k < 6; ++k)
                    if (first == M)
                    {
                        const uint32_t mm = (((pl[k] ^ ql[k]) | (ph[k] ^ qh[k])) & pm[k]) | pn[k];
                        if (mm) first = 32u * k + (uint32_t)__builtin_ctz( mm );
                    }
                #pragma unroll
                for (int k = 5; k >= 0; --k)
                    if (last == 0xFFFFFFFFu)
                    {
                        const uint32_t mm = (((pl[k] ^ ql[k]) | (ph[k] ^ qh[k])) & pm[k]) | pn[k];
                        if (mm) last = 32u * k + 31u - (uint32_t)__builtin_clz( mm );
                    }
                const uint32_t lead = first;
                const uint32_t tail = (last == 0xFFFFFFFFu) ? M : M - 1u - last;
                #pragma unroll
                for (int g = 1; g <= 4; ++g)
                    if (g <= gmax && d >= (uint32_t)g)
                    {
                        if (lead_prev[g - 1] + tail >= M) gapped = true;
                        if (lead + tail_prev[g - 1] + (uint32_t)g >= M) gapped = true;
                    }
                #pragma unroll
                for (int k = 3; k > 0; --k) { lead_prev[k] = lead_prev[k - 1]; tail_prev[k] = tail_prev[k - 1]; }
                lead_prev[0] = lead; tail_prev[0] = tail;
                #pragma unroll
                for (int k = 0; k < 6; ++k)
                {
                    ql[k] = __builtin_amdgcn_alignbit( ql[k + 1], ql[k], 1u );
                    qh[k] = __builtin_amdgcn_alignbit( qh[k + 1], qh[k], 1u );
                }
                ql[6] >>= 1; qh[6] >>= 1;
            }
            settled = !gapped;
        }
    }
    const int64_t go = gap_open, ge = gap_ext;
    int32_t gmax0 = 0, gmax1 = 0;
    while (gmax0 < 5 && go + (int64_t)gmax0 * ge >= U) ++gmax0;
    while (gmax1 < 5 && go + (int64_t)gmax1 * ge - P >= U) ++gmax1;
    const bool two11  = 2 * go >= U;
    const bool beyond = gmax0 > 4 || gmax1 > 4 || go - 2 * (int64_t)P >= U || 2 * go + ge >= U || 2 * go - P >= U || 3 * go >= U || ge < go;
    const bool third_applies = !settled && N >= M + 30u && !beyond && gmax0 >= 1 && (gmax1 >= 1 || two11);
    if (MODE == 0 && third_applies)
    {
        stash();
        return 2u;
    }
    if (MODE != 0 && third_applies)
    {
        #pragma unroll
        for (int k = 0; k < 7; ++k) { ql[k] = ql0[k]; qh[k] = qh0[k]; }
        uint32_t lead0_p[4] = { 0, 0, 0, 0 }, lead1_p[4] = { 0, 0, 0, 0 }, tail0_p[4] = { 0, 0, 0, 0 }, tail1_p[4] = { 0, 0, 0, 0 };
        bool gapped = false;
        uint32_t mwp[6] = { 0, 0, 0, 0, 0, 0 };
        for (uint32_t d = 0; d <= 31u && !gapped; ++d)
        {
            const bool have = d < 31u;
            uint32_t first = M, second = M, last = 0xFFFFFFFFu, last2 = 0xFFFFFFFFu;
            #pragma unroll
            for (int k = 0; k < 6; ++k)
                if (have && __any( second == M ))
                {
                    uint32_t w = (second == M) ? ((((pl[k] ^ ql[k]) | (ph[k] ^ qh[k])) & pm[k]) | pn[k]) : 0u;
                    if (first == M && w) { first = 32u * k + (uint32_t)__builtin_ctz( w ); w &= w - 1u; }
                    if (first != M && second == M && w) second = 32u * k + (uint32_t)__builtin_ctz( w );
                }
            #pragma unroll
            for (int k = 5; k >= 0; --k)
                if (have && __any( last2 == 0xFFFFFFFFu ))
                {
                    uint32_t w = (last2 == 0xFFFFFFFFu) ? ((((pl[k] ^ ql[k]) | (ph[k] ^ qh[k])) & pm[k]) | pn[k]) : 0u;
                    if (last == 0xFFFFFFFFu && w) { const uint32_t t = 31u - (uint32_t)__builtin_clz( w ); last = 32u * k + t; w &= ~(1u << t); }
                    if (last != 0xFFFFFFFFu && last2 == 0xFFFFFFFFu && w) last2 = 32u * k + 31u - (uint32_t)__builtin_clz( w );
                }
            const uint32_t lead0 = first, lead1 = second;
            const uint32_t tail0 = (last  == 0xFFFFFFFFu) ? M : M - 1u - last;
            const uint32_t tail1 = (last2 == 0xFFFFFFFFu) ? M : M - 1u - last2;
            if (have)
            {
                #pragma unroll
                for (int g = 1; g <= 4; ++g)
                    if (d >= (uint32_t)g)
                    {
                        if (g <= gmax0)
                        {
                            if (lead0_p[g - 1] + tail0 >= M) gapped = true;
                            if (lead0 + tail0_p[g - 1] + (uint32_t)g >= M) gapped = true;
                        }
                        if (g <= gmax1)
                        {
                            if (lead0_p[g - 1] + tail1 >= M || lead1_p[g - 1] + tail0 >= M) gapped = true;
                            if (lead0 + tail1_p[g - 1] + (uint32_t)g >= M || lead1 + tail0_p[g - 1] + (uint32_t)g >= M) gapped = true;
                        }
                    }
            }
            if (two11 && d >= 1u)
            {
                int32_t lo_c[2], hi_c[2]; int n_lo = 0, n_hi = 0;
                if (d >= 2u) { lo_c[n_lo++] = (int32_t)lead0_p[1];        hi_c[n_hi++] = (int32_t)M - (int32_t)tail0_p[1] - 1; }
                if (have)    { lo_c[n_lo++] = (int32_t)lead0 + 1;         hi_c[n_hi++] = (int32_t)M - (int32_t)tail0; }
                for (int x = 0; x < n_lo; ++x)
                    for (int y = 0; y < n_hi; ++y)
                    {
                        const int32_t lo = lo_c[x], hi = hi_c[y];
                        if (lo >= hi) { gapped = true; continue; }
                        const int32_t bf = (int32_t)lead0_p[0], bl = (int32_t)M - 1 - (int32_t)tail0_p[0];
                        bool any = (bf >= lo && bf < hi) || (tail0_p[0] < M && bl >= lo && bl < hi);
                        bool full = !any;
                        if (__any( !any ))
                        {
                            const uint32_t wi = (uint32_t)lo >> 5;
                            uint32_t w_lo = mwp[0], w_hi = mwp[1];
                            #pragma unroll
                            for (int k = 1; k < 6; ++k)
                            {
                                const uint32_t next = k < 5 ? mwp[k < 5 ? k + 1 : 5] : 0u;
                                w_lo = wi == (uint32_t)k ? mwp[k] : w_lo;
                                w_hi = wi == (uint32_t)k ? next   : w_hi;
                            }
                            uint32_t rows32 = __builtin_amdgcn_alignbit( w_hi, w_lo, (uint32_t)lo & 31u );
                            const int32_t span = hi - lo;
                            if (span < 32) rows32 &= (1u << span) - 1u;
                            if (!any && wi < 6u) { if (rows32) { any = true; full = false; } else if (span <= 32) full = false; }
                        }
                        if (full)
                        {
                            #pragma unroll
                            for (int k = 0; k < 6; ++k)
                            {
                                const int32_t a0 = lo - 32 * k > 0 ? lo - 32 * k : 0, a1 = hi - 32 * k < 32 ? hi - 32 * k : 32;
                                if (a0 < a1)
                                {
                                    const uint32_t hi_m = (a1 >= 32) ? 0xFFFFFFFFu : ((1u << a1) - 1u);
                                    const uint32_t lo_m = (1u << a0) - 1u;
                                    any = any || ((mwp[k] & hi_m & ~lo_m) != 0u);
                                }
                            }
                        }
                        if (!any) gapped = true;
                    }
            }
            #pragma unroll
            for (int k = 3; k > 0; --k) { lead0_p[k] = lead0_p[k - 1]; lead1_p[k] = lead1_p[k - 1]; tail0_p[k] = tail0_p[k - 1]; tail1_p[k] = tail1_p[k - 1]; }
            lead0_p[0] = lead0; lead1_p[0] = lead1; tail0_p[0] = tail0; tail1_p[0] = tail1;
            if (two11 && have)
            {
                #pragma unroll
                for (int k = 0; k < 6; ++k) mwp[k] = (((pl[k] ^ ql[k]) | (ph[k] ^ qh[k])) & pm[k]) | pn[k];
            }
            #pragma unroll
            for (int k = 0; k < 6; ++k)
            {
                ql[k] = __builtin_amdgcn_alignbit( ql[k + 1], ql[k], 1u );
                qh[k] = __builtin_amdgcn_alignbit( qh[k + 1], qh[k], 1u );
            }
            ql[6] >>= 1; qh[6] >>= 1;
        }
        settled = !gapped;
    }
    if (settled)
    {
        scores[job] = (int32_t)U; sinks[job] = make_uint2( M + best_d, M );
        return 0u;
    }
    return 1u;
}

template <int RBITS, int MODE, bool QUAL = false>
__global__ void __launch_bounds__(256)
ungapped_e2e31_kernel(const BatchDev b, const int32_t P, const int32_t G, const int32_t gap_open, const int32_t gap_ext,
                      int32_t* __restrict__ scores, uint2* __restrict__ sinks, uint8_t* __restrict__ need_dp,
                      const uint32_t* __restrict__ job_list, const uint32_t* __restrict__ job_count,
                      const SchemeDev sc, const JobLists out, const uint32_t third_mask)
{
    constexpr bool LIST = MODE != 0;
    constexpr int  NL   = LIST ? 1 : 4;
    __shared__ int32_t s_pen[QUAL ? 64 : 1];
    __shared__ typename JobAppend<NL>::Lds s_lists;
    const uint32_t n    = LIST ? *job_count : b.n;
    const uint32_t slot0 = blockIdx.x * (256u * JOB_LIST_CHUNKS);
    if (slot0 >= n) return;
    if (QUAL)
    {
        if (threadIdx.x < 64) s_pen[threadIdx.x] = -mismatch_score( sc, threadIdx.x );
        __syncthreads();
    }
    JobAppend<NL> app;
    auto job_of = [&](const int k) -> uint32_t { const uint32_t slot = slot0 + 256u * k + threadIdx.x; return LIST ? job_list[slot] : slot; };
    const bool pairing = ((third_mask >> 4) & 1u) && !(b.algo & (NVBIO_ALN_NO_PAIRED_GAP_CHANCE | NVBIO_ALN_RAGGED_READS));
    #pragma unroll 1
    for (int k = 0; k < JOB_LIST_CHUNKS; ++k)
    {
        int which = -1;
        uint32_t flag = 0;
        if (slot0 + 256u * k + threadIdx.x < n)
        {
            const uint32_t job  = job_of( k );
            flag = ungapped_e2e31_job<RBITS,MODE,QUAL>( b, P, G, gap_open, gap_ext, scores, sinks, job, s_pen );
            need_dp[job] = (uint8_t)flag;
            if (flag) which = LIST ? 0 : (flag == 3u ? 1 : (((third_mask >> flag) & 1u) ? 2 : 0));
        }
        if (MODE == 0 && !QUAL && pairing && __any( flag == 4u ))
        {
            const uint32_t slot = slot0 + 256u * k + threadIdx.x;
            const int role = gap_pair_role( b, slot, slot < n );
            const uint32_t flag_up = __shfl_down( flag, 1 ), flag_dn = __shfl_up( flag, 1 );
            if (role > 0 && flag == 4u && flag_up == 4u) which = 3;
            if (role < 0 && flag == 4u && flag_dn == 4u) which = -1;
        }
        app.note( s_lists, k, which );
    }
    app.flush( s_lists, out, job_of );
}

template <int RBITS>
__device__ __forceinline__ uint32_t
gap_chance_e2e31_job(const BatchDev& b, const int32_t P, const GapLadder lad, const int32_t gap_open, const int32_t gap_ext,
                     int32_t* __restrict__ scores, uint2* __restrict__ sinks, const uint32_t job, const bool has_u)
{
    const uint32_t rid   = b.read_id ? b.read_id[job] : job;
    const uint32_t first = b.read_offsets[rid];
    const uint32_t M     = b.read_offsets[rid + 1] - first;
    const uint32_t fl    = b.flags ? b.flags[job] : 0u;
    const bool     rev   = (fl & NVBIO_READ_REVERSE) != 0;
    const bool     comp  = (fl & NVBIO_READ_COMPLEMENT) != 0;
    const uint32_t tb    = b.win_begin[job];
    const uint32_t N     = b.win_end[job] - tb;
    const int32_t  cu   = has_u ? -scores[job] : 0x7FFFFFFF;
    const uint32_t cu_end = has_u ? sinks[job].x - M : 0u;

    uint32_t pl[6], ph[6], pn[6], pm[6], ql[7], qh[7];
    {
        uint64_t rlo[3], rhi[3], rn[3], tlo[4], thi[4];
        {
            ReadWords<RBITS> rw; TextWords13 tw;
            load_read_words<RBITS>( b.reads, first, M, rw );
            load_text_words13( b.text, tb, N < 192u ? N : 192u, tw );
            read_planes192<RBITS>( rw, first, M, rev, comp, rlo, rhi, rn );
            text_planes208( tw, tb, tlo, thi );
        }
        #pragma unroll
        for (int k = 0; k < 3; ++k)
        {
            const int32_t left = (int32_t)M - 64 * k;
            const uint64_t mask = left >= 64 ? ~0ull : (left > 0 ? ((1ull << left) - 1ull) : 0ull);
            pl[2*k] = (uint32_t)rlo[k]; pl[2*k+1] = (uint32_t)(rlo[k] >> 32);
            ph[2*k] = (uint32_t)rhi[k]; ph[2*k+1] = (uint32_t)(rhi[k] >> 32);
            pm[2*k] = (uint32_t)mask;   pm[2*k+1] = (uint32_t)(mask >> 32);
            pn[2*k] = (uint32_t)rn[k] & pm[2*k]; pn[2*k+1] = (uint32_t)(rn[k] >> 32) & pm[2*k+1];
            ql[2*k] = (uint32_t)tlo[k]; ql[2*k+1] = (uint32_t)(tlo[k] >> 32);
            qh[2*k] = (uint32_t)thi[k]; qh[2*k+1] = (uint32_t)(thi[k] >> 32);
        }
        ql[6] = (uint32_t)tlo[3]; qh[6] = (uint32_t)thi[3];
    }

    constexpr int GA = GAP_CHANCE_GA;
    const int32_t go = gap_open, ge = gap_ext;
    int32_t cg[GA + 2];
    #pragma unroll
    for (int g = 1; g <= GA + 1; ++g) cg[g] = -(go + (g - 1) * ge);
    cg[0] = 0;
    const int32_t c_unk = has_u ? lad.c_unk_u : lad.c_unk_n;
    const int32_t cost11 = 2 * cg[1], cost12 = cg[1] + cg[2];

    auto mmw = [&](const int k, const uint32_t x) -> uint32_t {
        const uint32_t tl = __builtin_amdgcn_alignbit( ql[k + 1], ql[k], x ), th = __builtin_amdgcn_alignbit( qh[k + 1], qh[k], x );
        return (((pl[k] ^ tl) | (ph[k] ^ th)) & pm[k]) | pn[k];
    };
    const uint32_t base = M >= 32u ? M - 32u : 0u;
    uint32_t plT, phT, pnT, pmT, qlT[2], qhT[2];
    {
        const uint32_t bw = base >> 5, bs = base & 31u;
        uint32_t a[4] = { 0, 0, 0, 0 }, c[4] = { 0, 0, 0, 0 }, t[3] = { 0, 0, 0 }, u[3] = { 0, 0, 0 };
        #pragma unroll
        for (int k = 0; k < 6; ++k)
            if (bw == (uint32_t)k)
            {
                a[0] = pl[k]; a[1] = k + 1 < 6 ? pl[k + 1] : 0u; a[2] = ph[k]; a[3] = k + 1 < 6 ? ph[k + 1] : 0u;
                c[0] = pn[k]; c[1] = k + 1 < 6 ? pn[k + 1] : 0u; c[2] = pm[k]; c[3] = k + 1 < 6 ? pm[k + 1] : 0u;
                t[0] = ql[k]; t[1] = k + 1 < 7 ? ql[k + 1] : 0u; t[2] = k + 2 < 7 ? ql[k + 2] : 0u;
                u[0] = qh[k]; u[1] = k + 1 < 7 ? qh[k + 1] : 0u; u[2] = k + 2 < 7 ? qh[k + 2] : 0u;
            }
        plT = __builtin_amdgcn_alignbit( a[1], a[0], bs ); phT = __builtin_amdgcn_alignbit( a[3], a[2], bs );
        pnT = __builtin_amdgcn_alignbit( c[1], c[0], bs ); pmT = __builtin_amdgcn_alignbit( c[3], c[2], bs );
        qlT[0] = __builtin_amdgcn_alignbit( t[1], t[0], bs ); qlT[1] = __builtin_amdgcn_alignbit( t[2], t[1], bs );
        qhT[0] = __builtin_amdgcn_alignbit( u[1], u[0], bs ); qhT[1] = __builtin_amdgcn_alignbit( u[2], u[1], bs );
    }
    auto pen_of = [&](const int32_t) -> int32_t { return P; };
    uint32_t Lp[GA], Tp[GA];
    #pragma unroll
    for (int k = 0; k < GA; ++k) { Lp[k] = 0; Tp[k] = 0; }
    uint32_t hot = 0;
    int32_t best_cost = 0x7FFFFFFF; uint32_t best_end = 0;
    bool ex11 = false, ex12 = false;
    uint32_t lng = 0, nmid = 0;
    const int32_t Mi = (int32_t)M;
    const int32_t hot_thr = (Mi - GA) / 2;

    auto clean = [&](const uint32_t x, const int32_t bf, const int32_t bl, const int32_t lo, const int32_t hi) -> bool {
        if (lo >= hi) return true;
        if ((bf >= lo && bf < hi) || (bl >= lo && bl < hi)) return false;
        bool any = false;
        #pragma unroll
        for (int k = 0; k < 6; ++k)
        {
            const int32_t a0 = lo - 32 * k > 0 ? lo - 32 * k : 0, a1 = hi - 32 * k < 32 ? hi - 32 * k : 32;
            if (a0 < a1)
            {
                const uint32_t hi_m = (a1 >= 32) ? 0xFFFFFFFFu : ((1u << a1) - 1u);
                const uint32_t lo_m = (1u << a0) - 1u;
                any = any || ((mmw( k, x ) & hi_m & ~lo_m) != 0u);
            }
        }
        return !any;
    };

    for (uint32_t d = 0; d <= 32u; ++d)
    {
        const bool have = d < 31u;
        uint32_t f0 = M, f1 = M, f2 = M, l0 = 0xFFFFFFFFu, l1 = 0xFFFFFFFFu, l2 = 0xFFFFFFFFu;
        bool mid_d = false;
        if (have)
        {
            uint32_t w = mmw( 0, d );
            if (w) { f0 = (uint32_t)__builtin_ctz( w ); w &= w - 1u; }
            if (w) { f1 = (uint32_t)__builtin_ctz( w ); w &= w - 1u; }
            if (w) f2 = (uint32_t)__builtin_ctz( w );
            const uint32_t tl = __builtin_amdgcn_alignbit( qlT[1], qlT[0], d ), th = __builtin_amdgcn_alignbit( qhT[1], qhT[0], d );
            w = (((plT ^ tl) | (phT ^ th)) & pmT) | pnT;
            if (w) { const uint32_t t = 31u - (uint32_t)__builtin_clz( w ); l0 = base + t; w &= ~(1u << t); }
            if (w) { const uint32_t t = 31u - (uint32_t)__builtin_clz( w ); l1 = base + t; w &= ~(1u << t); }
            if (w) l2 = base + 31u - (uint32_t)__builtin_clz( w );
            mid_d = M >= 96u && mmw( 1, d ) != 0u;
        }
        if (have && __any( M > 32u && (f2 == M || l2 == 0xFFFFFFFFu) ))
        {
            f0 = f1 = f2 = M; l0 = l1 = l2 = 0xFFFFFFFFu;
            #pragma unroll
            for (int k = 0; k < 6; ++k)
                if (__any( f2 == M && pm[k] != 0u ))
                {
                    uint32_t w = (f2 == M) ? mmw( k, d ) : 0u;
                    if (f0 == M && w) { f0 = 32u * k + (uint32_t)__builtin_ctz( w ); w &= w - 1u; }
                    if (f0 != M && f1 == M && w) { f1 = 32u * k + (uint32_t)__builtin_ctz( w ); w &= w - 1u; }
                    if (f1 != M && f2 == M && w) f2 = 32u * k + (uint32_t)__builtin_ctz( w );
                }
            #pragma unroll
            for (int k = 5; k >= 0; --k)
                if (__any( l2 == 0xFFFFFFFFu && pm[k] != 0u ))
                {
                    uint32_t w = (l2 == 0xFFFFFFFFu) ? mmw( k, d ) : 0u;
                    if (l0 == 0xFFFFFFFFu && w) { const uint32_t t = 31u - (uint32_t)__builtin_clz( w ); l0 = 32u * k + t; w &= ~(1u << t); }
                    if (l0 != 0xFFFFFFFFu && l1 == 0xFFFFFFFFu && w) { const uint32_t t = 31u - (uint32_t)__builtin_clz( w ); l1 = 32u * k + t; w &= ~(1u << t); }
// ... 399 lines not shown
template <int RBITS>
__global__ void __launch_bounds__(256) __attribute__((amdgpu_waves_per_eu(5)))
gap_chance_e2e31_kernel(const BatchDev b, const int32_t P, const GapLadder lad, const int32_t gap_open, const int32_t gap_ext,
                        int32_t* __restrict__ scores, uint2* __restrict__ sinks, uint8_t* __restrict__ need_dp,
                        const uint32_t* __restrict__ job_list, const uint32_t* __restrict__ job_count,
                        const uint32_t* __restrict__ list_p, const uint32_t* __restrict__ count_p, const JobLists out)
{
    __shared__ JobAppend<1>::Lds s_lists;
    __shared__ JobAppendTwo::Lds s_two;
    constexpr uint32_t W = 256u * JOB_LIST_CHUNKS;
    const uint32_t n = *job_count, np = *count_p;
    const uint32_t nbp = (np + W - 1u) / W;
    if (blockIdx.x < nbp)
    {
        gap_chance_pairs_chunks<RBITS>( b, P, lad, gap_open, gap_ext, scores, sinks, need_dp, list_p, np, blockIdx.x * W, out, s_two );
        return;
    }
    const uint32_t slot0 = (blockIdx.x - nbp) * W;
    if (slot0 >= n) return;
    JobAppend<1> app;
    auto job_of = [&](const int k) -> uint32_t { return job_list[slot0 + 256u * k + threadIdx.x]; };
    #pragma unroll 1
    for (int k = 0; k < JOB_LIST_CHUNKS; ++k)
    {
        int which = -1;
        if (slot0 + 256u * k + threadIdx.x < n)
        {
            const uint32_t job  = job_of( k );
            const uint32_t flag = gap_chance_e2e31_job<RBITS>( b, P, lad, gap_open, gap_ext, scores, sinks, job, need_dp[job] == 2 );
            need_dp[job] = (uint8_t)flag;
            if (flag) which = 0;
        }
        app.note( s_lists, k, which );
    }
    app.flush( s_lists, out, job_of );
}

template <int RBITS>
__global__ void __launch_bounds__(256) __attribute__((amdgpu_waves_per_eu(5)))
chances_e2e31_kernel(const BatchDev b, const int32_t P, const int32_t G, const GapLadder lad, const int32_t gap_open, const int32_t gap_ext,
                     int32_t* __restrict__ scores, uint2* __restrict__ sinks, uint8_t* __restrict__ need_dp,
                     const uint32_t* __restrict__ list_s, const uint32_t* __restrict__ count_s,
                     const uint32_t* __restrict__ list_t, const uint32_t* __restrict__ count_t,
                     const uint32_t* __restrict__ list_p, const uint32_t* __restrict__ count_p, const JobLists out)
{
    __shared__ JobAppend<1>::Lds s_lists;
    __shared__ JobAppendTwo::Lds s_two;
    constexpr uint32_t W = 256u * JOB_LIST_CHUNKS;
    const uint32_t n2 = *count_s, n3 = *count_t, np = *count_p;
    const uint32_t nb2 = (n2 + W - 1u) / W, nbp = (np + W - 1u) / W, nb3 = (n3 + W - 1u) / W + nbp, nb = nb2 + nb3;
    if (blockIdx.x >= nb) return;
    const uint32_t before = (uint32_t)((uint64_t)blockIdx.x * nb2 / nb);
    const bool     second = (uint32_t)((uint64_t)(blockIdx.x + 1u) * nb2 / nb) > before;
    if (!second && blockIdx.x - before < nbp)
    {
        gap_chance_pairs_chunks<RBITS>( b, P, lad, gap_open, gap_ext, scores, sinks, need_dp, list_p, np, (blockIdx.x - before) * W, out, s_two );
        return;
    }
    const uint32_t n      = second ? n2 : n3;
    const uint32_t* __restrict__ job_list = second ? list_s : list_t;
    const uint32_t slot0  = (second ? before : blockIdx.x - before - nbp) * W;
    JobAppend<1> app;
    auto job_of = [&](const int k) -> uint32_t { return job_list[slot0 + 256u * k + threadIdx.x]; };
    #pragma unroll 1
    for (int k = 0; k < JOB_LIST_CHUNKS; ++k)
    {
        int which = -1;
        if (slot0 + 256u * k + threadIdx.x < n)
        {
            const uint32_t job  = job_of( k );
            const uint32_t flag = second ? ungapped_e2e31_job<RBITS,1,false>( b, P, G, gap_open, gap_ext, scores, sinks, job, nullptr )
                                         : gap_chance_e2e31_job<RBITS>( b, P, lad, gap_open, gap_ext, scores, sinks, job, need_dp[job] == 2 );
            need_dp[job] = (uint8_t)flag;
            if (flag) which = 0;
        }
        app.note( s_lists, k, which );
    }
    app.flush( s_lists, out, job_of );
}

static bool ungapped_ok(const SchemeDev& sc, const BatchDev& b, int32_t* P, bool* by_quality)
{
    if (sc.match != 0) return false;
    if (sc.mm_min < 0 || sc.mm_max < 0) return false;
    *by_quality = b.quals != nullptr && sc.mm_min != sc.mm_max;
    if (*by_quality && (sc.mm_min <= 0 || sc.mm_max < sc.mm_min || (b.algo & NVBIO_ALN_NO_QUALITY_SHORTCUT))) return false;
    if (sc.pat_go >= 0 || sc.txt_go >= 0 || sc.pat_ge > 0 || sc.txt_ge > 0) return false;
    *P = sc.mm_min;
    return true;
}

static bool packed_ok(const int type, const SchemeDev& sc, const uint32_t max_read_len)
{
    if (max_read_len == 0) return false;
    const int lim = 4096;
    if (sc.mm_min < 0 || sc.mm_max < 0 || sc.mm_min > lim || sc.mm_max > lim) return false;
    if (sc.pat_go > 0 || sc.pat_ge > 0 || sc.pat_go < -lim || sc.pat_ge < -lim) return false;
    if (sc.match < 0) return false;
    if (type == NVBIO_LOCAL) return (uint64_t)sc.match * max_read_len <= 1000u;
    if (sc.txt_go > 0 || sc.txt_ge > 0 || sc.txt_go < -lim || sc.txt_ge < -lim) return false;
    int64_t step = sc.match;
    const int c[] = { sc.mm_min, sc.mm_max, -sc.pat_go, -sc.pat_ge, -sc.txt_go, -sc.txt_ge };
    for (int v : c) if (v > step) step = v;
    return ((int64_t)max_read_len + 32) * step <= 8000;
}

struct IsTwo { __host__ __device__ __forceinline__ uint8_t operator()(const uint8_t v) const { return v == 2u ? 1u : 0u; } };


__global__ void __launch_bounds__(256)
job_length_keys_kernel(const BatchDev b, const uint32_t* __restrict__ jobs, const uint32_t* __restrict__ job_count, uint16_t* __restrict__ keys,
                       uint32_t* __restrict__ jobs_all, uint32_t* __restrict__ count_all)
{
    const uint32_t n = jobs ? *job_count : b.n;
    if (!jobs && blockIdx.x == 0 && threadIdx.x == 0) *count_all = b.n;
    for (uint32_t i = blockIdx.x * blockDim.x + threadIdx.x; i < b.n; i += gridDim.x * blockDim.x)
    {
        uint32_t key = 0xFFFFu;
        if (i < n)
        {
            const uint32_t job = jobs ? jobs[i] : i;
            const uint32_t rid = b.read_id ? b.read_id[job] : job;
            const uint32_t M   = b.read_offsets[rid + 1] - b.read_offsets[rid];
            key = M < 0xFFFEu ? M : 0xFFFEu;
        }
        keys[i] = (uint16_t)key;
        if (!jobs) jobs_all[i] = i;
    }
}

static nvbio_status sort_jobs_by_length(const BatchDev& b, const uint32_t* job_list, const uint32_t* job_count, const uint32_t** list_out,
                                        const uint32_t** count_out, ScratchBlock* aux, hipStream_t s)
{
    size_t sort_bytes = 0;
    int bits = 1; while ((1u << bits) <= (b.max_read_len ? b.max_read_len : 0xFFFEu) && bits < 16) ++bits;
    bits = 16;
    NVB_HIP( hipcub::DeviceRadixSort::SortPairs( nullptr, sort_bytes, (const uint16_t*)nullptr, (uint16_t*)nullptr, (const uint32_t*)nullptr, (uint32_t*)nullptr,
                                                 (int)b.n, 0, bits, s ) );
    uint16_t *k_in, *k_out; uint32_t *l_all, *l_out, *c_all; void* tmp;
    NVB_CHECK( aux->alloc_layout( "banded_length_sort", s, "banded score: out of device memory for the length-sorted job list", [&](ScratchLayout& c)
    {
        k_in  = c.take<uint16_t>( b.n ); k_out = c.take<uint16_t>( b.n );
        l_all = c.take<uint32_t>( b.n ); l_out = c.take<uint32_t>( b.n );
        c_all = c.take<uint32_t>( 1 );
        tmp   = c.take<uint8_t>( sort_bytes );
    } ) );
    NVB_CHECK( NVB_LAUNCH( job_length_keys_kernel, dim3( (b.n + 255u) / 256u < 65536u ? (b.n + 255u) / 256u : 65536u ), dim3( 256 ), s, b, job_list, job_count, k_in, l_all, c_all ) );
    const hipError_t e = hipcub::DeviceRadixSort::SortPairs( tmp, sort_bytes, (const uint16_t*)k_in, k_out, job_list ? job_list : (const uint32_t*)l_all, l_out, (int)b.n, 0, bits, s );
    if (e != hipSuccess) { set_error( "job sort failed: %s", hipGetErrorString( e ) ); return NVBIO_ERR_HIP; }
    *list_out = l_out; *count_out = job_list ? job_count : c_all;
    return NVBIO_OK;
}

template <int TYPE, int RB>
static nvbio_status launch_pk_kernel(const BatchDev& b, const SchemeDev& sc, const uint32_t pairs, int32_t* scores, uint2* sinks,
                                     const uint32_t* job_list, const uint32_t* job_count, hipStream_t s)
{
    const dim3 grid( (pairs + 127u) / 128u ), block( 128 );
    const bool two = (b.algo & NVBIO_ALN_PK_THREE_WAVES) == 0;
    int64_t step = 0;
    { const int c[] = { sc.mm_min, sc.mm_max, -sc.pat_go, -sc.pat_ge, -sc.txt_go, -sc.txt_ge }; for (int v : c) if (v > step) step = v; }
    const bool fp = two && sc.match == 0 && TYPE == NVBIO_SEMI_GLOBAL && !(b.algo & NVBIO_ALN_NO_F16_DP) && ((int64_t)b.max_read_len + 32) * step <= 2040 && sc.mm_max <= 400;
    if (TYPE == NVBIO_SEMI_GLOBAL && sc.match == 0 && (b.algo & NVBIO_ALN_RAGGED_READS))
    {
        constexpr int T = (TYPE == NVBIO_SEMI_GLOBAL) ? TYPE : NVBIO_SEMI_GLOBAL;
        if (fp) return NVB_LAUNCH( (banded_gotoh_band31_pk_kernel<T,RB,2,true,true,true>), grid, block, s, b, sc, scores, sinks, job_list, job_count );
        return         NVB_LAUNCH( (banded_gotoh_band31_pk_kernel<T,RB,2,true,true>), grid, block, s, b, sc, scores, sinks, job_list, job_count );
    }
    if (TYPE != NVBIO_LOCAL && sc.match == 0)
    {
        constexpr int T = (TYPE == NVBIO_LOCAL) ? NVBIO_SEMI_GLOBAL : TYPE;
        if (fp)  return NVB_LAUNCH( (banded_gotoh_band31_pk_kernel<NVBIO_SEMI_GLOBAL,RB,2,true,false,true>), grid, block, s, b, sc, scores, sinks, job_list, job_count );
        if (two) return NVB_LAUNCH( (banded_gotoh_band31_pk_kernel<T,RB,2,true>), grid, block, s, b, sc, scores, sinks, job_list, job_count );
        return          NVB_LAUNCH( (banded_gotoh_band31_pk_kernel<T,RB,3,true>), grid, block, s, b, sc, scores, sinks, job_list, job_count );
    }
    if (two) return NVB_LAUNCH( (banded_gotoh_band31_pk_kernel<TYPE,RB,2,false>), grid, block, s, b, sc, scores, sinks, job_list, job_count );
    return          NVB_LAUNCH( (banded_gotoh_band31_pk_kernel<TYPE,RB,3,false>), grid, block, s, b, sc, scores, sinks, job_list, job_count );
}

template <int TYPE, int RB>
static nvbio_status launch_pk(const BatchDev& b, const SchemeDev& sc, int32_t* scores, uint2* sinks, hipStream_t s)
{
    const uint32_t pairs = (b.n + 1u) / 2u;
    int32_t P = 0; bool by_quality = false;
    if (TYPE == NVBIO_SEMI_GLOBAL && ungapped_ok( sc, b, &P, &by_quality ) && !(b.algo & NVBIO_ALN_NO_UNGAPPED_SCORE))
    {
        const int32_t G = sc.pat_go > sc.txt_go ? sc.pat_go : sc.txt_go;
        const bool third = !(b.algo & NVBIO_ALN_NO_THIRD_CHANCE);
        uint8_t* need_dp; uint32_t *job_list, *list_s, *list_t, *list_p, *counts;
        ScratchBlock aux;
        NVB_CHECK( aux.alloc_layout( "banded_job_list", s, "banded score: out of device memory for the job list", [&](ScratchLayout& c)
        {
            need_dp  = c.take<uint8_t>( b.n );
            job_list = c.take<uint32_t>( b.n );
            list_s   = c.take<uint32_t>( b.n );
            list_t   = c.take<uint32_t>( b.n );
            list_p   = c.take<uint32_t>( (b.n + 1u) / 2u );
            counts   = c.take<uint32_t>( JOB_LIST_COUNT * JOB_COUNT_STRIDE );
        } ) );
        const JobLists out = { job_list, list_s, list_t, list_p, counts };
        const uint32_t* job_count = counts;
        const uint32_t* count_s   = counts + JOB_COUNT_STRIDE;
        const uint32_t* count_t   = counts + 2u * JOB_COUNT_STRIDE;
        const uint32_t* count_p   = counts + 3u * JOB_COUNT_STRIDE;
        const bool gapc = !by_quality && !(b.algo & NVBIO_ALN_NO_GAP_CHANCE);
        const uint32_t third_mask = gapc ? ((third ? 1u << 2 : 0u) | 1u << 4) : (third ? 1u << 2 : 0u);
        const bool fused = gapc && third && !(b.algo & (NVBIO_ALN_NO_SECOND_CHANCE | NVBIO_ALN_SPLIT_CHANCES));
        const GapLadder lad = gap_ladder( P, G, sc.pat_go, sc.pat_ge );
        const dim3 grid( job_list_grid( b.n ) ), block( 256 );
        NVB_HIP( hipMemsetAsync( counts, 0, JOB_LIST_COUNT * JOB_COUNT_STRIDE * sizeof(uint32_t), s ) );
        if (by_quality)
            NVB_CHECK( NVB_LAUNCH( (ungapped_e2e31_kernel<RB,0,true>), grid, block, s, b, P, G, sc.pat_go, sc.pat_ge, scores, sinks, need_dp,
                                   (const uint32_t*)nullptr, (const uint32_t*)nullptr, sc, out, third_mask ) );
        else
            NVB_CHECK( NVB_LAUNCH( (ungapped_e2e31_kernel<RB,0>), grid, block, s, b, P, G, sc.pat_go, sc.pat_ge, scores, sinks, need_dp,
                                   (const uint32_t*)nullptr, (const uint32_t*)nullptr, sc, out, third_mask ) );
        if (fused)
            NVB_CHECK( NVB_LAUNCH( (chances_e2e31_kernel<RB>), dim3( job_list_grid( b.n ) + 2u ), block, s, b, P, G, lad, sc.pat_go, sc.pat_ge, scores, sinks,
                                   need_dp, (const uint32_t*)list_s, count_s, (const uint32_t*)list_t, count_t, (const uint32_t*)list_p, count_p, out ) );
        else
            NVB_CHECK( NVB_LAUNCH( (ungapped_e2e31_kernel<RB,1>), grid, block, s, b, P, G, sc.pat_go, sc.pat_ge, scores, sinks, need_dp,
                                   (const uint32_t*)list_s, count_s, SchemeDev{}, out, 0u ) );
        if (fused)
            ;
        else if (gapc)
            NVB_CHECK( NVB_LAUNCH( (gap_chance_e2e31_kernel<RB>), dim3( job_list_grid( b.n ) + 1u ), block, s, b, P, lad, sc.pat_go, sc.pat_ge, scores, sinks,
                                   need_dp, (const uint32_t*)list_t, count_t, (const uint32_t*)list_p, count_p, out ) );
        else if (third)
            NVB_CHECK( NVB_LAUNCH( (ungapped_e2e31_kernel<RB,2>), grid, block, s, b, P, G, sc.pat_go, sc.pat_ge, scores, sinks, need_dp,
                                   (const uint32_t*)list_t, count_t, SchemeDev{}, out, 0u ) );
        const uint32_t* jl = job_list; const uint32_t* jc = job_count; ScratchBlock sorted;
        if (TYPE == NVBIO_SEMI_GLOBAL && sc.match == 0 && (b.algo & NVBIO_ALN_RAGGED_READS) && !(b.algo & NVBIO_ALN_NO_LENGTH_SORT))
            NVB_CHECK( sort_jobs_by_length( b, job_list, job_count, &jl, &jc, &sorted, s ) );
        NVB_CHECK( (launch_pk_kernel<TYPE,RB>( b, sc, pairs, scores, sinks, jl, jc, s )) );
        return NVBIO_OK;
    }
    if (TYPE == NVBIO_SEMI_GLOBAL && sc.match == 0 && (b.algo & NVBIO_ALN_RAGGED_READS) && !(b.algo & NVBIO_ALN_NO_LENGTH_SORT) && b.n > 1u)
    {
        const uint32_t* jl = nullptr; const uint32_t* jc = nullptr; ScratchBlock sorted;
        NVB_CHECK( sort_jobs_by_length( b, nullptr, nullptr, &jl, &jc, &sorted, s ) );
        return launch_pk_kernel<TYPE,RB>( b, sc, pairs, scores, sinks, jl, jc, s );
    }
    return launch_pk_kernel<TYPE,RB>( b, sc, pairs, scores, sinks, nullptr, nullptr, s );
}

template <int BAND>
static nvbio_status launch_score(int type, const BatchDev& b, const SchemeDev& sc, uint32_t rbits, uint32_t tbits,
                                 int32_t* scores, uint2* sinks, hipStream_t s)
{
    return with_value( AlnTypes(), type, [&](auto TYPE)
    {
        if (BAND == 31 && plain_gotoh( sc ) && packed_ok( TYPE, sc, b.max_read_len ) && !(b.algo & NVBIO_ALN_NO_PACKED_DP) &&
            tbits == 2 && (rbits == 4 || rbits == 2))
            return rbits == 4 ? launch_pk<TYPE,4>( b, sc, scores, sinks, s ) : launch_pk<TYPE,2>( b, sc, scores, sinks, s );
        const dim3 grid( (b.n + 127u) / 128u ), block( 128 );
        return with_bits( BitsAll(), rbits, tbits, [&](auto P)
        {
            return NVB_LAUNCH( (banded_gotoh_kernel<BAND,TYPE,P.r,P.t>), grid, block, s, b, sc, scores, sinks, 0u, nullptr, nullptr, nullptr, 0 );
        }, [&] { return invalid_bits( rbits, tbits ); } );
    }, [&] { return invalid_type( type ); } );
}

template <int BAND>
static nvbio_status launch_staged(int type, const BatchDev& b, const SchemeDev& sc, uint32_t rbits, uint32_t tbits,
                                  const int32_t* min_scores, int32_t min_score, int32_t* scores, uint2* sinks, hipStream_t s)
{
    const dim3 grid( (b.n + 127u) / 128u ), block( 128 );
    return with_value( AlnTypes(), type, [&](auto TYPE)
    {
        return with_bits( BitsStaged(), rbits, tbits, [&](auto P)
        {
            return NVB_LAUNCH( (banded_gotoh_kernel<BAND,TYPE,P.r,P.t,false,true>), grid, block, s, b, sc, scores, sinks,
                               0u, (int32_t*)nullptr, (uint2*)nullptr, min_scores, min_score );
        }, [&] { set_error( "staged scoring: read_bits/text_bits %u/%u not instantiated (4/2, 2/2, 8/8)", rbits, tbits ); return NVBIO_ERR_UNSUPPORTED; } );
    }, [&] { return invalid_type( type ); } );
}

bool banded31_packed_ok(const SchemeDev& sc, const uint32_t max_read_len)
{
    return plain_gotoh( sc ) && packed_ok( NVBIO_SEMI_GLOBAL, sc, max_read_len );
}
nvbio_status banded31_packed_launch(const BatchDev& b, const SchemeDev& sc, const uint32_t read_bits, const uint32_t max_jobs, int32_t* scores, uint2* sinks,
                                    const uint32_t* job_list, const uint32_t* job_count, hipStream_t s)
{
    const uint32_t pairs = (max_jobs + 1u) / 2u;
    if (read_bits == 4) return launch_pk_kernel<NVBIO_SEMI_GLOBAL,4>( b, sc, pairs, scores, sinks, job_list, job_count, s );
    return                     launch_pk_kernel<NVBIO_SEMI_GLOBAL,2>( b, sc, pairs, scores, sinks, job_list, job_count, s );
}

nvbio_status make_batch(const nvbio_alignment_batch* in, BatchDev* b)
{
    NVB_REQUIRE( in != nullptr, "batch is NULL" );
    NVB_REQUIRE( in->read_bits == 2 || in->read_bits == 4 || in->read_bits == 8, "read_bits must be 2, 4 or 8" );
    NVB_REQUIRE( in->text_bits == 2 || in->text_bits == 8, "text_bits must be 2 or 8" );
    NVB_REQUIRE( in->n < (1u << 31), "at most 2^31 - 1 jobs per batch (the job lists are compacted with 32-bit signed counts)" );
    if (in->n)
    {
        NVB_REQUIRE( in->reads_dev && in->read_offsets_dev && in->text_dev && in->win_begin_dev && in->win_end_dev,
                     "NULL device pointer in batch" );
    }
    b->reads = in->reads_dev; b->read_offsets = in->read_offsets_dev; b->quals = in->quals_dev;
    b->read_id = in->read_id_dev; b->flags = in->flags_dev; b->text = in->text_dev;
    b->win_begin = in->win_begin_dev; b->win_end = in->win_end_dev; b->n = in->n; b->max_read_len = in->max_read_len; b->algo = in->algo_flags;
    return NVBIO_OK;
}

}

using namespace nvbio_amd;

template <int BAND>
static nvbio_status launch_best2(int type, const BatchDev& b, const SchemeDev& sc, uint32_t rbits, uint32_t tbits, uint32_t dist,
                                 int32_t* scores, uint2* sinks, int32_t* scores2, uint2* sinks2, hipStream_t s)
{
    const dim3 grid( (b.n + 127u) / 128u ), block( 128 );
    return with_value( AlnTypes(), type, [&](auto TYPE)
    {
        return with_bits( BitsBest2(), rbits, tbits, [&](auto P)
        {
            return NVB_LAUNCH( (banded_gotoh_kernel<BAND,TYPE,P.r,P.t,true>), grid, block, s, b, sc, scores, sinks, dist, scores2, sinks2, nullptr, 0 );
        }, [&] { set_error( "Best2Sink scoring: read_bits/text_bits %u/%u not instantiated (4/2, 2/2, 8/2, 8/8)", rbits, tbits ); return NVBIO_ERR_UNSUPPORTED; } );
    }, [&] { return invalid_type( type ); } );
}

extern "C" nvbio_status nvbio_banded_gotoh_score_best2(int device, uint32_t band, nvbio_alignment_type type,
                                                       const nvbio_gotoh_scheme* scheme, const nvbio_alignment_batch* batch, uint32_t distinct_dist,
                                                       int32_t* scores_dev, nvbio_uint2* sinks_dev, int32_t* scores2_dev, nvbio_uint2* sinks2_dev,
                                                       void* stream)
{
    NVB_REQUIRE( scheme != nullptr, "scheme is NULL" );
    BatchDev b; NVB_CHECK( make_batch( batch, &b ) );
    NVB_CHECK( check_band( band, NVBIO_ERR_UNSUPPORTED ) );
    if (b.n == 0) return NVBIO_OK;
    NVB_REQUIRE( scores_dev && sinks_dev && scores2_dev && sinks2_dev, "NULL output pointer" );
    DeviceGuard g( device ); if (!g.ok) return NVBIO_ERR_NO_DEVICE;
    const SchemeDev sc = scheme_dev( scheme );
    hipStream_t s = (hipStream_t)stream;
    return with_value( Bands(), band, [&](auto BAND)
    {
        return launch_best2<BAND>( type, b, sc, batch->read_bits, batch->text_bits, distinct_dist, scores_dev, (uint2*)sinks_dev, scores2_dev,
                                   (uint2*)sinks2_dev, s );
    }, [] { return NVBIO_ERR_UNSUPPORTED; } );
}

static nvbio_status banded_score(int device, uint32_t band, int type, const SchemeDev sc, const BatchDev& b, const nvbio_alignment_batch* batch,
                                 int32_t* scores_dev, nvbio_uint2* sinks_dev, void* stream)
{
    DeviceGuard g( device ); if (!g.ok) return NVBIO_ERR_NO_DEVICE;
    hipStream_t s = (hipStream_t)stream;
    return with_value( Bands(), band, [&](auto BAND)
    {
        return launch_score<BAND>( type, b, sc, batch->read_bits, batch->text_bits, scores_dev, (uint2*)sinks_dev, s );
    }, [] { return NVBIO_ERR_UNSUPPORTED; } );
}

extern "C" nvbio_status nvbio_banded_gotoh_score(int device, uint32_t band, nvbio_alignment_type type,
                                                 const nvbio_gotoh_scheme* scheme, const nvbio_alignment_batch* batch,
                                                 int32_t* scores_dev, nvbio_uint2* sinks_dev, void* stream)
{
    NVB_REQUIRE( scheme != nullptr, "scheme is NULL" );
    BatchDev b; NVB_CHECK( make_batch( batch, &b ) );
    NVB_CHECK( check_band( band, NVBIO_ERR_UNSUPPORTED ) );
    if (b.n == 0) return NVBIO_OK;
    NVB_REQUIRE( scores_dev && sinks_dev, "NULL output pointer" );
    return banded_score( device, band, type, scheme_dev( scheme ), b, batch, scores_dev, sinks_dev, stream );
}

extern "C" nvbio_status nvbio_banded_gap_pairs(int device, const nvbio_alignment_batch* batch, uint32_t* partner_dev, void* stream)
{
    BatchDev b; NVB_CHECK( make_batch( batch, &b ) );
    if (b.n == 0) return NVBIO_OK;
    NVB_REQUIRE( partner_dev != nullptr, "NULL output pointer" );
    DeviceGuard g( device ); if (!g.ok) return NVBIO_ERR_NO_DEVICE;
    return NVB_LAUNCH( gap_pairs_kernel, dim3( (b.n + 255u) / 256u ), dim3( 256 ), (hipStream_t)stream, b, partner_dev );
}

extern "C" nvbio_status nvbio_banded_gotoh_score_staged(int device, uint32_t band, nvbio_alignment_type type,
                                                        const nvbio_gotoh_scheme* scheme, const nvbio_alignment_batch* batch,
                                                        const int32_t* min_scores_dev, int32_t min_score,
                                                        int32_t* scores_dev, nvbio_uint2* sinks_dev, void* stream)
{
    NVB_REQUIRE( scheme != nullptr, "scheme is NULL" );
    BatchDev b; NVB_CHECK( make_batch( batch, &b ) );
    NVB_CHECK( check_band( band, NVBIO_ERR_UNSUPPORTED ) );
    if (b.n == 0) return NVBIO_OK;
    NVB_REQUIRE( scores_dev && sinks_dev, "NULL output pointer" );
    DeviceGuard g( device ); if (!g.ok) return NVBIO_ERR_NO_DEVICE;
    hipStream_t s = (hipStream_t)stream;
    const SchemeDev sc = scheme_dev( scheme );
    return with_value( Bands(), band, [&](auto BAND)
    {
        return launch_staged<BAND>( type, b, sc, batch->read_bits, batch->text_bits, min_scores_dev, min_score, scores_dev, (uint2*)sinks_dev, s );
    }, [] { return NVBIO_ERR_UNSUPPORTED; } );
}

extern "C" nvbio_status nvbio_banded_sw_score(int device, uint32_t band, nvbio_alignment_type type,
                                              const nvbio_sw_scheme* scheme, const nvbio_alignment_batch* batch,
                                              int32_t* scores_dev, nvbio_uint2* sinks_dev, void* stream)
{
    NVB_REQUIRE( scheme != nullptr, "scheme is NULL" );
    BatchDev b; NVB_CHECK( make_batch( batch, &b ) );
    NVB_CHECK( check_band( band, NVBIO_ERR_UNSUPPORTED ) );
    if (b.n == 0) return NVBIO_OK;
    NVB_REQUIRE( scores_dev && sinks_dev, "NULL output pointer" );
    SchemeDev sc = scheme_dev( scheme, false );
    sc.wide = 0;
    return banded_score( device, band, type, sc, b, batch, scores_dev, sinks_dev, stream );
}
```

Baseline: 1.949 billion.

## Add narrowed-band DP roles with monitored escape and redo list for band-31

Adds a NARROW variant of the packed binary16 band-31 SEMI_GLOBAL kernel. Jobs that the ungapped pre-pass classifies as near-diagonal (classes A and B) run the full band only for the first rows, then compute only the central 13 or 17 diagonals. A monitor tracks the best score that could leak in from the dropped diagonals; if that bound is not below the stored score, the job is pushed to a redo list instead of writing a result. The aim is to cut per-row DP work for most reads, at the cost of a classification step, extra job lists, a redo pass and many more kernel instantiations. It also adds a route-reporting score entry point.

Measured after the change: 1.989 billion (median of 6 runs). +2.0%, better.

```diff
diff --git a/include/nvbio_amd.h b/include/nvbio_amd.h
--- a/include/nvbio_amd.h
+++ b/include/nvbio_amd.h
@@ -526,6 +526,7 @@
     NVBIO_ALN_NO_F16_DP             = 16384,
     NVBIO_ALN_SPLIT_CHANCES         = 131072,
     NVBIO_ALN_NO_PAIRED_GAP_CHANCE  = 262144,
+    NVBIO_ALN_NO_NARROW_DP          = 524288,
     NVBIO_ALN_NO_NARROW_TRACEBACK   = 64
 };
 
@@ -580,6 +581,10 @@
 nvbio_status nvbio_banded_gotoh_score(int device, uint32_t band, nvbio_alignment_type type,
                                       const nvbio_gotoh_scheme* scheme, const nvbio_alignment_batch* batch,
                                       int32_t* scores_dev, nvbio_uint2* sinks_dev, void* stream);
+
+nvbio_status nvbio_banded_gotoh_score_routes(int device, uint32_t band, nvbio_alignment_type type,
+                                             const nvbio_gotoh_scheme* scheme, const nvbio_alignment_batch* batch,
+                                             int32_t* scores_dev, nvbio_uint2* sinks_dev, uint8_t* routes_dev, void* stream);
 
 nvbio_status nvbio_banded_gotoh_score_staged(int device, uint32_t band, nvbio_alignment_type type,
                                              const nvbio_gotoh_scheme* scheme, const nvbio_alignment_batch* batch,
diff --git a/nvbio-gpl_amd/__init__.py b/nvbio-gpl_amd/__init__.py
--- a/nvbio-gpl_amd/__init__.py
+++ b/nvbio-gpl_amd/__init__.py
@@ -17,6 +17,8 @@
 ALN_NO_NARROW_TRACEBACK, ALN_NO_SECOND_CHANCE, ALN_PK_STRIPE8, ALN_NO_NARROW_SCORE, ALN_NO_BAND_ROUTE = 64, 128, 256, 512, 1024
 ALN_NO_QUALITY_SHORTCUT, ALN_RAGGED_READS, ALN_NO_LENGTH_SORT, ALN_NO_F16_DP, ALN_NO_COOPERATIVE_DP, ALN_NO_GAP_CHANCE = 2048, 4096, 8192, 16384, 32768, 65536
 ALN_SPLIT_CHANCES, ALN_NO_PAIRED_GAP_CHANCE = 131072, 262144
+ALN_NO_NARROW_DP = 524288
+ROUTE_SETTLED, ROUTE_FULL_BAND, ROUTE_CLASS_A, ROUTE_CLASS_B, ROUTE_REDONE = 0, 1, 2, 3, 8
 DEFAULT_ALGO_FLAGS = 0
 BACKTRACK_REFERENCE_QUIRKS = 1
 
@@ -1056,6 +1058,18 @@
     return BatchedBandedAlignmentScore(band_len, aligner).enact(batch)
 
 
+def banded_gotoh_score_routes(band_len, aligner, batch):
+    torch = _torch()
+    scores = torch.empty(batch.n, dtype=torch.int32, device=batch.device)
+    sinks = torch.empty((batch.n, 2), dtype=torch.int32, device=batch.device)
+    routes = torch.empty(batch.n, dtype=torch.uint8, device=batch.device)
+    bs = batch.c_struct()
+    _check(lib().nvbio_banded_gotoh_score_routes(FMIndex._dev_index(batch.device), ctypes.c_uint32(int(band_len)), ctypes.c_int(aligner.type),
+                                                 ctypes.byref(aligner.scheme.c), ctypes.byref(bs), _ptr(scores), _ptr(sinks), _ptr(routes),
+                                                 _stream_ptr(batch.device)))
+    return scores, sinks, routes
+
+
 GAP_PAIR_MAX_SHIFT = 5
 NO_PARTNER = 0xFFFFFFFF
 
diff --git a/nvbio-gpl_amd/csrc/gotoh_banded.hip b/nvbio-gpl_amd/csrc/gotoh_banded.hip
--- a/nvbio-gpl_amd/csrc/gotoh_banded.hip
+++ b/nvbio-gpl_amd/csrc/gotoh_banded.hip
@@ -210,21 +210,37 @@
     return (uint32_t)x;
 }
 
-template <int TYPE, int RBITS, int MINW = 3, bool M0 = false, bool RAGGED = false, bool FP = false>
+constexpr uint32_t NARROW_FULL_ROWS = 24u;
+constexpr int NARROW_A_HALF = 6, NARROW_B_HALF = 8;
+struct NarrowJobs { const uint32_t *list_b, *count_b, *list_a, *count_a; uint32_t *redo, *redo_count; };
+
+template <int TYPE, int RBITS, int MINW = 3, bool M0 = false, bool RAGGED = false, bool FP = false, bool NARROW = false>
 __global__ void __launch_bounds__(128) __attribute__((amdgpu_waves_per_eu(MINW, 3)))
 banded_gotoh_band31_pk_kernel(const BatchDev b, const SchemeDev sc, int32_t* __restrict__ scores, uint2* __restrict__ sinks,
-                              const uint32_t* __restrict__ job_list, const uint32_t* __restrict__ job_count)
+                              const uint32_t* __restrict__ job_list, const uint32_t* __restrict__ job_count, const NarrowJobs nj)
 {
     constexpr int BAND = 31;
     constexpr uint32_t RMASK = (1u << RBITS) - 1u;
     static_assert( !FP || (M0 && TYPE != NVBIO_LOCAL), "the binary16 build: match = 0, GLOBAL / SEMI_GLOBAL" );
+    static_assert( !NARROW || (FP && !RAGGED && TYPE == NVBIO_SEMI_GLOBAL), "the narrow roles: the binary16 SEMI_GLOBAL build, equal read lengths" );
     typedef typename PkLanes<FP>::type v2;
     __shared__ int32_t s_mm[64];
     if (threadIdx.x < 64) s_mm[threadIdx.x] = mismatch_score( sc, threadIdx.x );
     __syncthreads();
 
-    const uint32_t n_jobs = job_list ? *job_count : b.n;
-    const uint32_t pair = blockIdx.x * blockDim.x + threadIdx.x;
+    uint32_t n_jobs = job_list ? *job_count : b.n;
+    uint32_t group = blockIdx.x;
+    int role = 0;
+    if (NARROW)
+    {
+        const uint32_t nb_full = (n_jobs + 255u) / 256u, n_b = *nj.count_b, nb_b = (n_b + 255u) / 256u;
+        if (group >= nb_full)
+        {
+            group -= nb_full; role = 1; job_list = nj.list_b; n_jobs = n_b;
+            if (group >= nb_b) { group -= nb_b; role = 2; job_list = nj.list_a; n_jobs = *nj.count_a; }
+        }
+    }
+    const uint32_t pair = group * blockDim.x + threadIdx.x;
     if (2u * pair >= n_jobs) return;
     const uint32_t* __restrict__ rwords = (const uint32_t*)b.reads;
     const uint32_t* __restrict__ twords = (const uint32_t*)b.text;
@@ -269,7 +285,7 @@
 
     const uint32_t qadj = (uint32_t)((uintptr_t)b.quals & 3u);
     const uint32_t* __restrict__ qwords = (const uint32_t*)((uintptr_t)b.quals - qadj);
-    const bool has_quals = (b.quals != nullptr);
+    const bool has_quals = !NARROW && (b.quals != nullptr);
 
     const v2 GO = pk_of<v2>( sc.pat_go, sc.pat_go ), GE = pk_of<v2>( sc.pat_ge, sc.pat_ge );
     const v2 INF = pk_of<v2>( -16384, -16384 ), ZERO = pk_of<v2>( 0, 0 );
@@ -286,6 +302,7 @@
 
     int32_t  best[2]   = { NVBIO_SCORE_MIN, NVBIO_SCORE_MIN };
     uint32_t best_x[2] = { 0xFFFFFFFFu, 0xFFFFFFFFu }, best_y[2] = { 0xFFFFFFFFu, 0xFFFFFFFFu };
+    v2 mon = INF;
 
     const bool want0 = valid[0] && N[0] >= M[0], want1 = valid[1] && N[1] >= M[1];
     const bool split = (TYPE != NVBIO_LOCAL) && !RAGGED && want0 && want1 && M[0] != M[1];
@@ -293,6 +310,9 @@
     uint32_t pad[2] = { 0u, 0u };
     if (RAGGED && TYPE != NVBIO_LOCAL) { pad[0] = rows_max - rows_all[0]; pad[1] = rows_max - rows_all[1]; }
 
+    auto run_passes = [&](auto ROLE_)
+    {
+    constexpr int ROLE = decltype(ROLE_)::value;
     for (int pass = 0; pass < (split ? 2 : 1); ++pass)
     {
         uint32_t rows_u[2];
@@ -355,7 +375,7 @@
             H[j] = pk_of<v2>( h0, h0 ); F[j] = INF; Hg[j] = H[j] + GO;
         }
 
-        for (uint32_t r0 = 0; r0 < rows; r0 += 8u)
+        auto do_chunk = [&](const uint32_t r0, auto LO_, auto HI_)
         {
             uint32_t rchunk[2], tchunk[2], tchunk1[2]; int rsh[2], rstep[2];
             uint64_t qchunk[2] = { 0, 0 }; int qsh[2], qstep[2];
@@ -385,6 +405,9 @@
             if (r0 + 8u < rows) issue_loads( r0 + 8u );
 
             const uint32_t r_end = (r0 + 8u < rows) ? 8u : rows - r0;
+            auto chunk_rows = [&](auto LO_, auto HI_)
+            {
+            constexpr int LO = decltype(LO_)::value, HI = decltype(HI_)::value;
             for (uint32_t t = 0; t < r_end; ++t)
             {
                 const uint32_t i = r0 + t;
@@ -450,11 +473,12 @@
                 v2 E = ZERO, a = ZERO, tt, ff = INF, dd = ZERO;
                 v2s key = pk( -1, -1 );
                 {
-                    const v2 x  = F[1] + GE;
-                    const v2 t0 = flags_of( 0 );
-                    const v2 d  = diag_of( H[0], t0 );
-                    const v2 f  = pk_max( x, Hg[1] );
-                    F[0] = f;
+                    if (NARROW && LO > 0) mon = pk_max3( mon, Hg[LO], F[LO] + GE );
+                    const v2 x  = F[LO + 1] + GE;
+                    const v2 t0 = flags_of( LO );
+                    const v2 d  = diag_of( H[LO], t0 );
+                    const v2 f  = pk_max( x, Hg[LO + 1] );
+                    F[LO] = f;
                     if (FP) { ff = f; dd = d; tt = ZERO; }
                     else
                     {
@@ -463,35 +487,36 @@
                     }
                 }
                 #pragma unroll
-                for (int j = 0; j < BAND; ++j)
+                for (int j = LO; j <= HI; ++j)
                 {
                     constexpr int Z = 0;
                     const int j1 = j + 1, j2 = j + 2;
                     v2 x = INF, d = ZERO, f = INF, t1 = ZERO, tn = ZERO, an = ZERO;
                     uint32_t q1 = 0;
-                    if (j2 < BAND) x  = F[j2] + GE;
+                    if (j2 <= HI) x  = F[j2] + GE;
                     __builtin_amdgcn_sched_barrier( Z );
-                    const v2 h = FP ? ((j == 0) ? pk_max( ff, dd ) : pk_max3( ff, dd, E )) : ((j == 0) ? tt : pk_max( tt, E ));
-                    if (j1 < BAND) q1 = flags_at( j1 );
+                    const v2 h = FP ? ((j == LO) ? pk_max( ff, dd ) : pk_max3( ff, dd, E )) : ((j == LO) ? tt : pk_max( tt, E ));
+                    if (j1 <= HI) q1 = flags_at( j1 );
                     __builtin_amdgcn_sched_barrier( Z );
                     const v2 hg = h + GO;
-                    if (!FP && j1 < BAND) t1 = flags_in( q1 );
-                    if (j2 < BAND) f  = pk_max( x, Hg[j2] );
+                    if (!FP && j1 <= HI) t1 = flags_in( q1 );
+                    if (j2 <= HI) f  = pk_max( x, Hg[j2] );
                     __builtin_amdgcn_sched_barrier( Z );
-                    const v2 En = (j == 0) ? hg : pk_max( hg, a );
+                    const v2 En = (j == LO) ? hg : pk_max( hg, a );
                     if (FP) __builtin_amdgcn_sched_barrier( Z );
-                    if (FP && j1 < BAND) t1 = flags_in( q1 );
-                    if (j1 < BAND) d  = diag_of( H[j1], t1 );
+                    if (FP && j1 <= HI) t1 = flags_in( q1 );
+                    if (j1 <= HI) d  = diag_of( H[j1], t1 );
                     __builtin_amdgcn_sched_barrier( Z );
-                    if (j1 < BAND) an = En + GE;
+                    if (j1 <= HI) an = En + GE;
+                    if (NARROW && HI < BAND - 1 && j == HI) mon = pk_max( mon, En );
                     if (TYPE == NVBIO_LOCAL) key = pk_max( key, __builtin_bit_cast( v2s, h ) * K32 + pk( j, j ) );
                     __builtin_amdgcn_sched_barrier( Z );
-                    if (j1 < BAND)
+                    if (j1 <= HI)
                     {
-                        if (FP) { ff = (j2 < BAND) ? f : d; dd = d; }
+                        if (FP) { ff = (j2 <= HI) ? f : d; dd = d; }
                         else
                         {
-                            tn = (j2 < BAND) ? pk_max( f, d ) : d;
+                            tn = (j2 <= HI) ? pk_max( f, d ) : d;
                             if (TYPE == NVBIO_LOCAL) tn = pk_max( tn, ZERO );
                         }
                         F[j1] = f;
@@ -508,7 +533,32 @@
                     if (i < rows_u[1] && (k1 >> 5) >= best[1]) { best[1] = k1 >> 5; best_x[1] = i + (uint32_t)(k1 & 31) + 1u; best_y[1] = i + 1u; }
                 }
             }
-        }
+            };
+            chunk_rows( LO_, HI_ );
+        };
+        typedef std::integral_constant<int,0> C0; typedef std::integral_constant<int,BAND - 1> C30;
+        if (NARROW && ROLE != 0 && rows > NARROW_FULL_ROWS)
+        {
+            typedef std::integral_constant<int,15 - NARROW_A_HALF> ALO; typedef std::integral_constant<int,15 + NARROW_A_HALF> AHI;
+            typedef std::integral_constant<int,15 - NARROW_B_HALF> BLO; typedef std::integral_constant<int,15 + NARROW_B_HALF> BHI;
+            auto qualify = [&](auto LO_, auto HI_)
+            {
+                constexpr int LO = decltype(LO_)::value, HI = decltype(HI_)::value;
+                #pragma unroll
+                for (int j = 0; j < BAND; ++j)
+                    if (j < LO || j > HI)
+                    {
+                        mon = pk_max3( mon, H[j], F[j] );
+                        H[j] = INF; Hg[j] = INF; F[j] = INF;
+                    }
+                if (split) mon = ZERO;
+            };
+            for (uint32_t r0 = 0; r0 < NARROW_FULL_ROWS; r0 += 8u) do_chunk( r0, C0(), C30() );
+            if (ROLE == 2) { qualify( ALO(), AHI() ); for (uint32_t r0 = NARROW_FULL_ROWS; r0 < rows; r0 += 8u) do_chunk( r0, ALO(), AHI() ); }
+            else           { qualify( BLO(), BHI() ); for (uint32_t r0 = NARROW_FULL_ROWS; r0 < rows; r0 += 8u) do_chunk( r0, BLO(), BHI() ); }
+        }
+        else
+            for (uint32_t r0 = 0; r0 < rows; r0 += 8u) do_chunk( r0, C0(), C30() );
 
         if (TYPE != NVBIO_LOCAL)
         {
@@ -537,9 +587,21 @@
             }
         }
     }
+    };
+    if (NARROW && role == 1)      run_passes( std::integral_constant<int,1>() );
+    else if (NARROW && role == 2) run_passes( std::integral_constant<int,2>() );
+    else                          run_passes( std::integral_constant<int,0>() );
     #pragma unroll
     for (int u = 0; u < 2; ++u)
-        if (valid[u]) { scores[out_id[u]] = best[u]; sinks[out_id[u]] = make_uint2( best_x[u], best_y[u] ); }
+    {
+        if (!valid[u]) continue;
+        if (NARROW && role != 0 && !((u ? (float)mon.y : (float)mon.x) < (float)scores[out_id[u]]))
+        {
+            nj.redo[atomicAdd( nj.redo_count, 1u )] = out_id[u];
+            continue;
+        }
+        scores[out_id[u]] = best[u]; sinks[out_id[u]] = make_uint2( best_x[u], best_y[u] );
+    }
 }
 
 constexpr int GAP_CHANCE_GA = 5;
@@ -553,6 +615,24 @@
     return c;
 }
 struct GapLadder { int32_t c_unk_u, c_unk_n; };
+struct NarrowRule { int32_t thr_a, thr_b; uint32_t cnt_max; };
+static NarrowRule narrow_rule(const bool on, const int32_t P, const int32_t go, const int32_t ge)
+{
+    NarrowRule r = { 1, 1, 0u };
+    if (!on || ge >= 0 || P <= 0) return r;
+    const int64_t a = (int64_t)go + (int64_t)NARROW_A_HALF * ge + 1, bb = (int64_t)go + (int64_t)NARROW_B_HALF * ge + 1;
+    if (bb < -2000) return r;
+    r.thr_a = (int32_t)a; r.thr_b = (int32_t)bb;
+    r.cnt_max = (uint32_t)((-bb) / P);
+    return r;
+}
+__device__ __forceinline__ uint32_t narrow_class(const NarrowRule nr, const int64_t U, const uint32_t best_d, const int32_t gap_ext)
+{
+    const int64_t o = best_d > 15u ? best_d - 15u : 15u - best_d;
+    if (o <= NARROW_A_HALF && U >= (int64_t)nr.thr_a - o * gap_ext) return 2u;
+    if (o <= NARROW_B_HALF && U >= (int64_t)nr.thr_b - o * gap_ext) return 1u;
+    return 0u;
+}
 static GapLadder gap_ladder(const int32_t P, const int32_t G, const int32_t go, const int32_t ge)
 {
     const int64_t floor_u = 3 * (int64_t)(G < go ? G : go) - P;
@@ -564,19 +644,19 @@
 }
 
 constexpr uint32_t JOB_COUNT_STRIDE = 32u;
-constexpr uint32_t JOB_LIST_COUNT   = 4u;
+constexpr uint32_t JOB_LIST_COUNT   = 7u;
 #ifndef NVB_JOB_LIST_CHUNKS
 #define NVB_JOB_LIST_CHUNKS 1
 #endif
 constexpr int JOB_LIST_CHUNKS = NVB_JOB_LIST_CHUNKS;
 static inline uint32_t job_list_grid(const uint32_t n) { return (n + 256u * JOB_LIST_CHUNKS - 1u) / (256u * JOB_LIST_CHUNKS); }
 
-struct JobLists { uint32_t *dp, *second, *third, *pairs; uint32_t* counts; };
+struct JobLists { uint32_t *dp, *second, *third, *pairs; uint32_t* counts; uint32_t *class_b, *class_a, *redo; };
 
 template <int NL>
 struct JobAppend
 {
-    static_assert( NL >= 1 && NL <= 4 && JOB_LIST_CHUNKS >= 1 && JOB_LIST_CHUNKS <= 4, "JobAppend: up to 4 lists, up to 4 chunks" );
+    static_assert( NL >= 1 && NL <= 6 && JOB_LIST_CHUNKS >= 1 && JOB_LIST_CHUNKS <= 4, "JobAppend: up to 6 lists, up to 4 chunks" );
     struct Lds { uint32_t cnt[NL][4 * JOB_LIST_CHUNKS]; uint32_t base[NL]; };
     static constexpr int SLOT = NL <= 3 ? 8 : 16;
     typedef typename std::conditional<NL <= 3, uint32_t, uint64_t>::type Mine;
@@ -611,7 +691,7 @@
             if (e)
             {
                 const uint32_t l = (e >> 6) - 1u;
-                uint32_t* const list = l == 0u ? out.dp : (l == 1u ? out.second : (l == 2u ? out.third : out.pairs));
+                uint32_t* const list = l == 0u ? out.dp : (l == 1u ? out.second : (l == 2u ? out.third : (l == 3u ? out.pairs : (l == 4u ? out.class_b : out.class_a))));
                 list[lds.base[l] + lds.cnt[l][4 * k + wave] + (e & 63u)] = job_of( k );
             }
         }
@@ -693,7 +773,8 @@
 template <int RBITS, int MODE, bool QUAL>
 __device__ __forceinline__ uint32_t
 ungapped_e2e31_job(const BatchDev& b, const int32_t P, const int32_t G, const int32_t gap_open, const int32_t gap_ext,
-                   int32_t* __restrict__ scores, uint2* __restrict__ sinks, const uint32_t job, const int32_t* s_pen)
+                   int32_t* __restrict__ scores, uint2* __restrict__ sinks, const uint32_t job, const int32_t* s_pen,
+                   const NarrowRule nr = NarrowRule{ 1, 1, 0u })
 {
     constexpr bool LIST = MODE != 0;
     const uint32_t rid   = b.read_id ? b.read_id[job] : job;
@@ -761,6 +842,7 @@
     {
         const int64_t floor_u = 3 * (int64_t)(G < gap_open ? G : gap_open) - P;
         const uint32_t cap = P > 0 ? (uint32_t)((-floor_u - 1) / (int64_t)P) : 0xFFFFFFFEu;
+        const uint32_t cap_x = (!QUAL && nr.cnt_max > cap && N >= M + 30u) ? nr.cnt_max : cap;
         uint32_t cnt_d[QUAL ? 31 : 1];
         #pragma unroll
         for (uint32_t d = 0; d < 31u; ++d)
@@ -771,7 +853,7 @@
                 const uint32_t tl = d ? __builtin_amdgcn_alignbit( ql0[1], ql0[0], d ) : ql0[0], th = d ? __builtin_amdgcn_alignbit( qh0[1], qh0[0], d ) : qh0[0];
                 cnt = (uint32_t)__popc( (((pl[0] ^ tl) | (ph[0] ^ th)) & pm[0]) | pn[0] );
             }
-            const uint32_t thr = QUAL ? cap : (best_cnt < cap ? best_cnt : cap);
+            const uint32_t thr = QUAL ? cap : (best_cnt < cap_x ? best_cnt : cap_x);
             if (__any( on && cnt <= thr ))
             {
                 #pragma unroll
@@ -787,6 +869,11 @@
         }
         if (best_cnt > cap)
         {
+            if (!QUAL && best_cnt <= cap_x)
+            {
+                const uint32_t cls = narrow_class( nr, -(int64_t)P * (int64_t)best_cnt, best_d, gap_ext );
+                if (cls) { scores[job] = -P * (int32_t)best_cnt; sinks[job] = make_uint2( M + best_d, M ); return 1u | (cls << 8); }
+            }
             const bool gap_chance = !QUAL && P > 0 && N >= M + 30u && gap_ext < 0 && gap_open <= gap_ext && !(b.algo & NVBIO_ALN_NO_GAP_CHANCE);
             return gap_chance ? 4u : 1u;
         }
@@ -1012,6 +1099,11 @@
         scores[job] = (int32_t)U; sinks[job] = make_uint2( M + best_d, M );
         return 0u;
     }
+    if (MODE == 0 && !QUAL && N >= M + 30u)
+    {
+        const uint32_t cls = narrow_class( nr, U, best_d, gap_ext );
+        if (cls) { stash(); return 1u | (cls << 8); }
+    }
     return 1u;
 }
 
@@ -1020,10 +1112,10 @@
 ungapped_e2e31_kernel(const BatchDev b, const int32_t P, const int32_t G, const int32_t gap_open, const int32_t gap_ext,
                       int32_t* __restrict__ scores, uint2* __restrict__ sinks, uint8_t* __restrict__ need_dp,
                       const uint32_t* __restrict__ job_list, const uint32_t* __restrict__ job_count,
-                      const SchemeDev sc, const JobLists out, const uint32_t third_mask)
+                      const SchemeDev sc, const JobLists out, const uint32_t third_mask, const NarrowRule nr)
 {
     constexpr bool LIST = MODE != 0;
-    constexpr int  NL   = LIST ? 1 : 4;
+    constexpr int  NL   = LIST ? 1 : 6;
     __shared__ int32_t s_pen[QUAL ? 64 : 1];
     __shared__ typename JobAppend<NL>::Lds s_lists;
     const uint32_t n    = LIST ? *job_count : b.n;
@@ -1045,9 +1137,11 @@
         if (slot0 + 256u * k + threadIdx.x < n)
         {
             const uint32_t job  = job_of( k );
-            flag = ungapped_e2e31_job<RBITS,MODE,QUAL>( b, P, G, gap_open, gap_ext, scores, sinks, job, s_pen );
+            flag = ungapped_e2e31_job<RBITS,MODE,QUAL>( b, P, G, gap_open, gap_ext, scores, sinks, job, s_pen, nr );
+            const uint32_t cls = flag >> 8;
+            flag &= 255u;
             need_dp[job] = (uint8_t)flag;
-            if (flag) which = LIST ? 0 : (flag == 3u ? 1 : (((third_mask >> flag) & 1u) ? 2 : 0));
+            if (flag) which = LIST ? 0 : (flag == 3u ? 1 : (((third_mask >> flag) & 1u) ? 2 : (cls ? 3 + (int)cls : 0)));
         }
         if (MODE == 0 && !QUAL && pairing && __any( flag == 4u ))
         {
@@ -1753,34 +1847,62 @@
     return NVBIO_OK;
 }
 
-template <int TYPE, int RB>
-static nvbio_status launch_pk_kernel(const BatchDev& b, const SchemeDev& sc, const uint32_t pairs, int32_t* scores, uint2* sinks,
-                                     const uint32_t* job_list, const uint32_t* job_count, hipStream_t s)
-{
-    const dim3 grid( (pairs + 127u) / 128u ), block( 128 );
+template <bool REDO>
+__global__ void __launch_bounds__(256)
+job_routes_kernel(const JobLists l, const uint32_t n, const bool classes, uint8_t* __restrict__ routes)
+{
+    const uint32_t n_dp = REDO ? 0u : l.counts[0], n_b = (REDO || !classes) ? 0u : l.counts[4u * JOB_COUNT_STRIDE], n_a = (REDO || !classes) ? 0u : l.counts[5u * JOB_COUNT_STRIDE];
+    const uint32_t n_r = (REDO && classes) ? l.counts[6u * JOB_COUNT_STRIDE] : 0u;
+    for (uint32_t i = blockIdx.x * blockDim.x + threadIdx.x; i < n; i += gridDim.x * blockDim.x)
+    {
+        if (i < n_dp) routes[l.dp[i]] = 1u;
+        if (i < n_b)  routes[l.class_b[i]] = 3u;
+        if (i < n_a)  routes[l.class_a[i]] = 2u;
+        if (i < n_r)  routes[l.redo[i]] |= 8u;
+    }
+}
+
+template <int TYPE>
+static bool pk_binary16_ok(const BatchDev& b, const SchemeDev& sc)
+{
     const bool two = (b.algo & NVBIO_ALN_PK_THREE_WAVES) == 0;
     int64_t step = 0;
     { const int c[] = { sc.mm_min, sc.mm_max, -sc.pat_go, -sc.pat_ge, -sc.txt_go, -sc.txt_ge }; for (int v : c) if (v > step) step = v; }
-    const bool fp = two && sc.match == 0 && TYPE == NVBIO_SEMI_GLOBAL && !(b.algo & NVBIO_ALN_NO_F16_DP) && ((int64_t)b.max_read_len + 32) * step <= 2040 && sc.mm_max <= 400;
+    return two && sc.match == 0 && TYPE == NVBIO_SEMI_GLOBAL && !(b.algo & NVBIO_ALN_NO_F16_DP) && ((int64_t)b.max_read_len + 32) * step <= 2040 && sc.mm_max <= 400;
+}
+
+template <int TYPE, int RB>
+static nvbio_status launch_pk_kernel(const BatchDev& b, const SchemeDev& sc, const uint32_t pairs, int32_t* scores, uint2* sinks,
+                                     const uint32_t* job_list, const uint32_t* job_count, hipStream_t s, const NarrowJobs* narrow = nullptr)
+{
+    const dim3 grid( (pairs + 127u) / 128u ), block( 128 );
+    const bool two = (b.algo & NVBIO_ALN_PK_THREE_WAVES) == 0;
+    const bool fp = pk_binary16_ok<TYPE>( b, sc );
+    const NarrowJobs nj = {};
+    if (narrow)
+    {
+        constexpr int T = (TYPE == NVBIO_SEMI_GLOBAL) ? TYPE : NVBIO_SEMI_GLOBAL;
+        return NVB_LAUNCH( (banded_gotoh_band31_pk_kernel<T,RB,2,true,false,true,true>), dim3( grid.x + 2u ), block, s, b, sc, scores, sinks, job_list, job_count, *narrow );
+    }
     if (TYPE == NVBIO_SEMI_GLOBAL && sc.match == 0 && (b.algo & NVBIO_ALN_RAGGED_READS))
     {
         constexpr int T = (TYPE == NVBIO_SEMI_GLOBAL) ? TYPE : NVBIO_SEMI_GLOBAL;
-        if (fp) return NVB_LAUNCH( (banded_gotoh_band31_pk_kernel<T,RB,2,true,true,true>), grid, block, s, b, sc, scores, sinks, job_list, job_count );
-        return         NVB_LAUNCH( (banded_gotoh_band31_pk_kernel<T,RB,2,true,true>), grid, block, s, b, sc, scores, sinks, job_list, job_count );
+        if (fp) return NVB_LAUNCH( (banded_gotoh_band31_pk_kernel<T,RB,2,true,true,true>), grid, block, s, b, sc, scores, sinks, job_list, job_count, nj );
+        return         NVB_LAUNCH( (banded_gotoh_band31_pk_kernel<T,RB,2,true,true>), grid, block, s, b, sc, scores, sinks, job_list, job_count, nj );
     }
     if (TYPE != NVBIO_LOCAL && sc.match == 0)
     {
         constexpr int T = (TYPE == NVBIO_LOCAL) ? NVBIO_SEMI_GLOBAL : TYPE;
-        if (fp)  return NVB_LAUNCH( (banded_gotoh_band31_pk_kernel<NVBIO_SEMI_GLOBAL,RB,2,true,false,true>), grid, block, s, b, sc, scores, sinks, job_list, job_count );
-        if (two) return NVB_LAUNCH( (banded_gotoh_band31_pk_kernel<T,RB,2,true>), grid, block, s, b, sc, scores, sinks, job_list, job_count );
-        return          NVB_LAUNCH( (banded_gotoh_band31_pk_kernel<T,RB,3,true>), grid, block, s, b, sc, scores, sinks, job_list, job_count );
-    }
-    if (two) return NVB_LAUNCH( (banded_gotoh_band31_pk_kernel<TYPE,RB,2,false>), grid, block, s, b, sc, scores, sinks, job_list, job_count );
-    return          NVB_LAUNCH( (banded_gotoh_band31_pk_kernel<TYPE,RB,3,false>), grid, block, s, b, sc, scores, sinks, job_list, job_count );
+        if (fp)  return NVB_LAUNCH( (banded_gotoh_band31_pk_kernel<NVBIO_SEMI_GLOBAL,RB,2,true,false,true>), grid, block, s, b, sc, scores, sinks, job_list, job_count, nj );
+        if (two) return NVB_LAUNCH( (banded_gotoh_band31_pk_kernel<T,RB,2,true>), grid, block, s, b, sc, scores, sinks, job_list, job_count, nj );
+        return          NVB_LAUNCH( (banded_gotoh_band31_pk_kernel<T,RB,3,true>), grid, block, s, b, sc, scores, sinks, job_list, job_count, nj );
+    }
+    if (two) return NVB_LAUNCH( (banded_gotoh_band31_pk_kernel<TYPE,RB,2,false>), grid, block, s, b, sc, scores, sinks, job_list, job_count, nj );
+    return          NVB_LAUNCH( (banded_gotoh_band31_pk_kernel<TYPE,RB,3,false>), grid, block, s, b, sc, scores, sinks, job_list, job_count, nj );
 }
 
 template <int TYPE, int RB>
-static nvbio_status launch_pk(const BatchDev& b, const SchemeDev& sc, int32_t* scores, uint2* sinks, hipStream_t s)
+static nvbio_status launch_pk(const BatchDev& b, const SchemeDev& sc, int32_t* scores, uint2* sinks, hipStream_t s, uint8_t* routes)
 {
     const uint32_t pairs = (b.n + 1u) / 2u;
     int32_t P = 0; bool by_quality = false;
@@ -1788,7 +1910,10 @@
     {
         const int32_t G = sc.pat_go > sc.txt_go ? sc.pat_go : sc.txt_go;
         const bool third = !(b.algo & NVBIO_ALN_NO_THIRD_CHANCE);
-        uint8_t* need_dp; uint32_t *job_list, *list_s, *list_t, *list_p, *counts;
+        uint8_t* need_dp; uint32_t *job_list, *list_s, *list_t, *list_p, *counts, *list_b, *list_a, *list_r;
+        const NarrowRule nr = narrow_rule( b.quals == nullptr && !(b.algo & (NVBIO_ALN_NO_NARROW_DP | NVBIO_ALN_RAGGED_READS)) && pk_binary16_ok<TYPE>( b, sc ),
+                                           P, sc.pat_go, sc.pat_ge );
+        const bool classes = nr.thr_b != 1;
         ScratchBlock aux;
         NVB_CHECK( aux.alloc_layout( "banded_job_list", s, "banded score: out of device memory for the job list", [&](ScratchLayout& c)
         {
@@ -1798,8 +1923,11 @@
             list_t   = c.take<uint32_t>( b.n );
             list_p   = c.take<uint32_t>( (b.n + 1u) / 2u );
             counts   = c.take<uint32_t>( JOB_LIST_COUNT * JOB_COUNT_STRIDE );
+            list_b   = c.take<uint32_t>( classes ? b.n : 1u );
+            list_a   = c.take<uint32_t>( classes ? b.n : 1u );
+            list_r   = c.take<uint32_t>( classes ? b.n : 1u );
         } ) );
-        const JobLists out = { job_list, list_s, list_t, list_p, counts };
+        const JobLists out = { job_list, list_s, list_t, list_p, counts, list_b, list_a, list_r };
         const uint32_t* job_count = counts;
         const uint32_t* count_s   = counts + JOB_COUNT_STRIDE;
         const uint32_t* count_t   = counts + 2u * JOB_COUNT_STRIDE;
@@ -1812,16 +1940,16 @@
         NVB_HIP( hipMemsetAsync( counts, 0, JOB_LIST_COUNT * JOB_COUNT_STRIDE * sizeof(uint32_t), s ) );
         if (by_quality)
             NVB_CHECK( NVB_LAUNCH( (ungapped_e2e31_kernel<RB,0,true>), grid, block, s, b, P, G, sc.pat_go, sc.pat_ge, scores, sinks, need_dp,
-                                   (const uint32_t*)nullptr, (const uint32_t*)nullptr, sc, out, third_mask ) );
+                                   (const uint32_t*)nullptr, (const uint32_t*)nullptr, sc, out, third_mask, nr ) );
         else
             NVB_CHECK( NVB_LAUNCH( (ungapped_e2e31_kernel<RB,0>), grid, block, s, b, P, G, sc.pat_go, sc.pat_ge, scores, sinks, need_dp,
-                                   (const uint32_t*)nullptr, (const uint32_t*)nullptr, sc, out, third_mask ) );
+                                   (const uint32_t*)nullptr, (const uint32_t*)nullptr, sc, out, third_mask, nr ) );
         if (fused)
             NVB_CHECK( NVB_LAUNCH( (chances_e2e31_kernel<RB>), dim3( job_list_grid( b.n ) + 2u ), block, s, b, P, G, lad, sc.pat_go, sc.pat_ge, scores, sinks,
                                    need_dp, (const uint32_t*)list_s, count_s, (const uint32_t*)list_t, count_t, (const uint32_t*)list_p, count_p, out ) );
         else
             NVB_CHECK( NVB_LAUNCH( (ungapped_e2e31_kernel<RB,1>), grid, block, s, b, P, G, sc.pat_go, sc.pat_ge, scores, sinks, need_dp,
-                                   (const uint32_t*)list_s, count_s, SchemeDev{}, out, 0u ) );
+                                   (const uint32_t*)list_s, count_s, SchemeDev{}, out, 0u, NarrowRule{ 1, 1, 0u } ) );
         if (fused)
             ;
         else if (gapc)
@@ -1829,11 +1957,25 @@
                                    need_dp, (const uint32_t*)list_t, count_t, (const uint32_t*)list_p, count_p, out ) );
         else if (third)
             NVB_CHECK( NVB_LAUNCH( (ungapped_e2e31_kernel<RB,2>), grid, block, s, b, P, G, sc.pat_go, sc.pat_ge, scores, sinks, need_dp,
-                                   (const uint32_t*)list_t, count_t, SchemeDev{}, out, 0u ) );
+                                   (const uint32_t*)list_t, count_t, SchemeDev{}, out, 0u, NarrowRule{ 1, 1, 0u } ) );
         const uint32_t* jl = job_list; const uint32_t* jc = job_count; ScratchBlock sorted;
         if (TYPE == NVBIO_SEMI_GLOBAL && sc.match == 0 && (b.algo & NVBIO_ALN_RAGGED_READS) && !(b.algo & NVBIO_ALN_NO_LENGTH_SORT))
             NVB_CHECK( sort_jobs_by_length( b, job_list, job_count, &jl, &jc, &sorted, s ) );
-        NVB_CHECK( (launch_pk_kernel<TYPE,RB>( b, sc, pairs, scores, sinks, jl, jc, s )) );
+        if (classes)
+        {
+            const NarrowJobs nj = { list_b, counts + 4u * JOB_COUNT_STRIDE, list_a, counts + 5u * JOB_COUNT_STRIDE, list_r, counts + 6u * JOB_COUNT_STRIDE };
+            NVB_CHECK( (launch_pk_kernel<TYPE,RB>( b, sc, pairs, scores, sinks, jl, jc, s, &nj )) );
+            NVB_CHECK( (launch_pk_kernel<TYPE,RB>( b, sc, pairs, scores, sinks, list_r, counts + 6u * JOB_COUNT_STRIDE, s )) );
+        }
+        else
+            NVB_CHECK( (launch_pk_kernel<TYPE,RB>( b, sc, pairs, scores, sinks, jl, jc, s )) );
+        if (routes)
+        {
+            const dim3 rgrid( (b.n + 255u) / 256u < 4096u ? (b.n + 255u) / 256u : 4096u );
+            NVB_HIP( hipMemsetAsync( routes, 0, b.n, s ) );
+            NVB_CHECK( NVB_LAUNCH( job_routes_kernel<false>, rgrid, block, s, out, b.n, classes, routes ) );
+            NVB_CHECK( NVB_LAUNCH( job_routes_kernel<true>,  rgrid, block, s, out, b.n, classes, routes ) );
+        }
         return NVBIO_OK;
     }
     if (TYPE == NVBIO_SEMI_GLOBAL && sc.match == 0 && (b.algo & NVBIO_ALN_RAGGED_READS) && !(b.algo & NVBIO_ALN_NO_LENGTH_SORT) && b.n > 1u)
@@ -1847,13 +1989,13 @@
 
 template <int BAND>
 static nvbio_status launch_score(int type, const BatchDev& b, const SchemeDev& sc, uint32_t rbits, uint32_t tbits,
-                                 int32_t* scores, uint2* sinks, hipStream_t s)
+                                 int32_t* scores, uint2* sinks, hipStream_t s, uint8_t* routes)
 {
     return with_value( AlnTypes(), type, [&](auto TYPE)
     {
         if (BAND == 31 && plain_gotoh( sc ) && packed_ok( TYPE, sc, b.max_read_len ) && !(b.algo & NVBIO_ALN_NO_PACKED_DP) &&
             tbits == 2 && (rbits == 4 || rbits == 2))
-            return rbits == 4 ? launch_pk<TYPE,4>( b, sc, scores, sinks, s ) : launch_pk<TYPE,2>( b, sc, scores, sinks, s );
+            return rbits == 4 ? launch_pk<TYPE,4>( b, sc, scores, sinks, s, routes ) : launch_pk<TYPE,2>( b, sc, scores, sinks, s, routes );
         const dim3 grid( (b.n + 127u) / 128u ), block( 128 );
         return with_bits( BitsAll(), rbits, tbits, [&](auto P)
         {
@@ -1945,14 +2087,27 @@
 }
 
 static nvbio_status banded_score(int device, uint32_t band, int type, const SchemeDev sc, const BatchDev& b, const nvbio_alignment_batch* batch,
-                                 int32_t* scores_dev, nvbio_uint2* sinks_dev, void* stream)
+                                 int32_t* scores_dev, nvbio_uint2* sinks_dev, void* stream, uint8_t* routes_dev = nullptr)
 {
     DeviceGuard g( device ); if (!g.ok) return NVBIO_ERR_NO_DEVICE;
     hipStream_t s = (hipStream_t)stream;
+    if (routes_dev) NVB_HIP( hipMemsetAsync( routes_dev, 1, b.n, s ) );
     return with_value( Bands(), band, [&](auto BAND)
     {
-        return launch_score<BAND>( type, b, sc, batch->read_bits, batch->text_bits, scores_dev, (uint2*)sinks_dev, s );
+        return launch_score<BAND>( type, b, sc, batch->read_bits, batch->text_bits, scores_dev, (uint2*)sinks_dev, s, routes_dev );
     }, [] { return NVBIO_ERR_UNSUPPORTED; } );
+}
+
+extern "C" nvbio_status nvbio_banded_gotoh_score_routes(int device, uint32_t band, nvbio_alignment_type type,
+                                                        const nvbio_gotoh_scheme* scheme, const nvbio_alignment_batch* batch,
+                                                        int32_t* scores_dev, nvbio_uint2* sinks_dev, uint8_t* routes_dev, void* stream)
+{
+    NVB_REQUIRE( scheme != nullptr, "scheme is NULL" );
+    BatchDev b; NVB_CHECK( make_batch( batch, &b ) );
+    NVB_CHECK( check_band( band, NVBIO_ERR_UNSUPPORTED ) );
+    if (b.n == 0) return NVBIO_OK;
+    NVB_REQUIRE( scores_dev && sinks_dev && routes_dev, "NULL output pointer" );
+    return banded_score( device, band, type, scheme_dev( scheme ), b, batch, scores_dev, sinks_dev, stream, routes_dev );
 }
 
 extern "C" nvbio_status nvbio_banded_gotoh_score(int device, uint32_t band, nvbio_alignment_type type,
diff --git a/profiles/r09_pk_row_loop_w6.s b/profiles/r09_pk_row_loop_w6.s
--- /dev/null
+++ b/profiles/r09_pk_row_loop_w6.s
@@ -0,0 +1,166 @@
+.LBB236_348:
+	v_lshrrev_b32_e32 v102, v191, v186
+	v_bitop3_b32 v102, v84, v102, 15 bitop3:0x78
+	v_alignbit_b32 v156, v156, v188, 31
+	v_bfe_i32 v200, v102, 0, 1
+	v_bfe_u32 v103, v186, v191, 4
+	v_alignbit_b32 v157, v157, v187, 31
+	v_xor_b32_e32 v200, v156, v200
+	v_bfe_i32 v102, v102, 1, 1
+	s_add_i32 s73, s78, s72
+	v_bitop3_b32 v102, v102, v200, v157 bitop3:0xde
+	v_cmp_gt_u32_e32 vcc, 4, v103
+	v_alignbit_b32 v158, v158, v189, 31
+	v_bfe_u32 v200, v82, v190, 4
+	v_cndmask_b32_e32 v102, -1, v102, vcc
+	v_cmp_ge_u32_e32 vcc, s73, v88
+	v_alignbit_b32 v159, v159, v83, 31
+	v_pk_maximum3_f16 v11, v11, v182, v182
+	v_cndmask_b32_e64 v103, 0, 1, vcc
+	v_or_b32_e32 v102, v102, v103
+	v_lshrrev_b32_e32 v103, v190, v82
+	v_bitop3_b32 v103, v85, v103, 15 bitop3:0x78
+	v_bfe_i32 v201, v103, 0, 1
+	v_xor_b32_e32 v201, v158, v201
+	v_bfe_i32 v103, v103, 1, 1
+	v_bitop3_b32 v103, v103, v201, v159 bitop3:0xde
+	v_cmp_gt_u32_e32 vcc, 4, v200
+	v_add_u32_e32 v191, v191, v97
+	v_lshlrev_b32_e32 v187, 2, v187
+	v_cndmask_b32_e32 v103, -1, v103, vcc
+	v_cmp_ge_u32_e32 vcc, s73, v89
+	v_lshlrev_b32_e32 v188, 2, v188
+	v_add_u32_e32 v190, v190, v99
+	v_cndmask_b32_e64 v200, 0, 1, vcc
+	v_or_b32_e32 v103, v103, v200
+	v_perm_b32 v200, v103, v102, s33
+	v_perm_b32 v102, v103, v102, s80
+	v_lshlrev_b32_e32 v182, 8, v102
+	v_pk_add_f16 v103, v91, v168
+	v_pk_add_f16 v168, v91, v185
+	v_and_b32_e32 v182, 0x20002000, v182
+	v_lshlrev_b32_e32 v83, 2, v83
+	v_lshlrev_b32_e32 v189, 2, v189
+	v_pk_fma_f16 v154, v182, v92, v154
+	v_pk_maximum3_f16 v168, v168, v183, v183
+	v_pk_add_f16 v183, v91, v184
+	v_lshlrev_b32_e32 v182, 9, v102
+	v_pk_maximum3_f16 v154, v168, v154, v154
+	v_and_b32_e32 v184, 0x20002000, v182
+	v_pk_add_f16 v182, v90, v154
+	v_pk_maximum3_f16 v185, v183, v170, v170
+	v_pk_fma_f16 v153, v184, v92, v153
+	v_pk_add_f16 v170, v91, v182
+	v_pk_add_f16 v180, v91, v180
+	v_pk_maximum3_f16 v153, v185, v153, v182
+	v_lshlrev_b32_e32 v183, 10, v102
+	v_and_b32_e32 v201, 0x20002000, v183
+	v_pk_add_f16 v183, v90, v153
+	v_pk_maximum3_f16 v184, v180, v171, v171
+	v_pk_maximum3_f16 v170, v183, v170, v170
+	v_pk_fma_f16 v152, v201, v92, v152
+	v_pk_add_f16 v171, v91, v170
+	v_pk_add_f16 v179, v91, v179
+	v_pk_maximum3_f16 v152, v184, v152, v170
+	v_lshlrev_b32_e32 v170, 11, v102
+	v_and_b32_e32 v201, 0x20002000, v170
+	v_pk_add_f16 v170, v90, v152
+	v_pk_maximum3_f16 v180, v179, v169, v169
+	v_pk_maximum3_f16 v169, v170, v171, v171
+	v_pk_fma_f16 v151, v201, v92, v151
+	v_pk_add_f16 v201, v91, v169
+	v_pk_add_f16 v178, v91, v178
+	v_pk_maximum3_f16 v151, v180, v151, v169
+	v_lshlrev_b32_e32 v169, 12, v102
+	v_and_b32_e32 v169, 0x20002000, v169
+	v_pk_add_f16 v171, v90, v151
+	v_pk_maximum3_f16 v179, v178, v167, v167
+	v_pk_maximum3_f16 v167, v171, v201, v201
+	v_pk_fma_f16 v150, v169, v92, v150
+	v_pk_add_f16 v201, v91, v167
+	v_pk_add_f16 v177, v91, v177
+	v_pk_maximum3_f16 v150, v179, v150, v167
+	v_lshlrev_b32_e32 v102, 13, v102
+	v_and_b32_e32 v102, 0x20002000, v102
+	v_pk_add_f16 v169, v90, v150
+	v_pk_maximum3_f16 v178, v177, v166, v166
+	v_pk_maximum3_f16 v166, v169, v201, v201
+	v_pk_fma_f16 v102, v102, v92, v149
+	v_pk_add_f16 v201, v91, v166
+	v_pk_add_f16 v176, v91, v176
+	v_pk_maximum3_f16 v149, v178, v102, v166
+	v_lshrrev_b32_e32 v102, 2, v200
+	v_and_b32_e32 v102, 0x20002000, v102
+	v_pk_add_f16 v167, v90, v149
+	v_pk_maximum3_f16 v177, v176, v164, v164
+	v_pk_maximum3_f16 v164, v167, v201, v201
+	v_pk_fma_f16 v102, v102, v92, v148
+	v_pk_add_f16 v201, v91, v164
+	v_pk_add_f16 v174, v91, v174
+	v_pk_maximum3_f16 v148, v177, v102, v164
+	v_lshrrev_b32_e32 v102, 1, v200
+	v_and_b32_e32 v102, 0x20002000, v102
+	v_pk_add_f16 v166, v90, v148
+	v_pk_maximum3_f16 v176, v174, v162, v162
+	v_pk_maximum3_f16 v162, v166, v201, v201
+	v_pk_fma_f16 v102, v102, v92, v147
+	v_pk_add_f16 v201, v91, v162
+	v_pk_add_f16 v172, v91, v172
+	v_pk_maximum3_f16 v147, v176, v102, v162
+	v_and_b32_e32 v102, 0x20002000, v200
+	v_pk_add_f16 v164, v90, v147
+	v_pk_maximum3_f16 v174, v172, v165, v165
+	v_pk_maximum3_f16 v162, v164, v201, v201
+	v_pk_fma_f16 v102, v102, v92, v146
+	v_pk_add_f16 v165, v91, v162
+	v_pk_add_f16 v172, v91, v175
+	v_pk_maximum3_f16 v146, v174, v102, v162
+	v_lshlrev_b32_e32 v102, 1, v200
+	v_and_b32_e32 v102, 0x20002000, v102
+	v_pk_add_f16 v162, v90, v146
+	v_pk_maximum3_f16 v172, v172, v163, v163
+	v_pk_maximum3_f16 v163, v162, v165, v165
+	v_pk_fma_f16 v102, v102, v92, v145
+	v_pk_add_f16 v201, v91, v163
+	v_pk_add_f16 v173, v91, v173
+	v_pk_maximum3_f16 v145, v172, v102, v163
+	v_lshlrev_b32_e32 v102, 2, v200
+	v_and_b32_e32 v102, 0x20002000, v102
+	v_pk_add_f16 v165, v90, v145
+	v_pk_maximum3_f16 v175, v173, v161, v161
+	v_pk_maximum3_f16 v161, v165, v201, v201
+	v_pk_fma_f16 v102, v102, v92, v144
+	v_pk_add_f16 v201, v91, v161
+	v_pk_add_f16 v173, v91, v181
+	v_pk_maximum3_f16 v144, v175, v102, v161
+	v_lshlrev_b32_e32 v102, 3, v200
+	v_and_b32_e32 v102, 0x20002000, v102
+	v_pk_add_f16 v163, v90, v144
+	v_pk_maximum3_f16 v173, v173, v160, v160
+	v_pk_maximum3_f16 v160, v163, v201, v201
+	v_pk_fma_f16 v102, v102, v92, v143
+	v_pk_add_f16 v181, v91, v160
+	v_pk_maximum3_f16 v143, v173, v102, v160
+	v_lshlrev_b32_e32 v102, 4, v200
+	v_and_b32_e32 v102, 0x20002000, v102
+	v_pk_add_f16 v161, v90, v143
+	s_nop 0
+	v_pk_maximum3_f16 v160, v161, v181, v181
+	v_pk_fma_f16 v102, v102, v92, v142
+	v_pk_add_f16 v181, v91, v160
+	v_pk_maximum3_f16 v142, v102, v160, v160
+	s_nop 0
+	v_pk_add_f16 v160, v90, v142
+	s_nop 0
+	v_pk_maximum3_f16 v102, v160, v181, v181
+	s_nop 0
+	v_pk_maximum3_f16 v11, v11, v103, v102
+	s_add_i32 s72, s72, 1
+	v_cmp_ge_u32_e32 vcc, s72, v199
+	s_or_b64 s[40:41], vcc, s[40:41]
+	v_mov_b32_e32 v181, 0xf400f400
+	s_andn2_b64 exec, exec, s[40:41]
+	s_cbranch_execnz .LBB236_348
+	s_or_b64 exec, exec, s[40:41]
+	v_mov_b32_e32 v181, 0xf400f400
+	s_branch .LBB236_343
diff --git a/profiles/r09_pk_row_loop_w8.s b/profiles/r09_pk_row_loop_w8.s
--- /dev/null
+++ b/profiles/r09_pk_row_loop_w8.s
@@ -0,0 +1,202 @@
+.LBB236_651:
+	v_lshrrev_b32_e32 v81, v205, v198
+	v_bitop3_b32 v81, v84, v81, 15 bitop3:0x78
+	v_alignbit_b32 v160, v160, v200, 31
+	v_bfe_i32 v213, v81, 0, 1
+	v_bfe_u32 v212, v198, v205, 4
+	v_alignbit_b32 v161, v161, v199, 31
+	v_xor_b32_e32 v213, v160, v213
+	v_bfe_i32 v81, v81, 1, 1
+	s_add_i32 s5, s72, s4
+	v_bitop3_b32 v81, v81, v213, v161 bitop3:0xde
+	v_cmp_gt_u32_e32 vcc, 4, v212
+	v_alignbit_b32 v162, v162, v203, 31
+	v_bfe_u32 v213, v201, v204, 4
+	v_cndmask_b32_e32 v81, -1, v81, vcc
+	v_cmp_ge_u32_e32 vcc, s5, v88
+	v_alignbit_b32 v163, v163, v202, 31
+	v_pk_maximum3_f16 v11, v11, v194, v194
+	v_cndmask_b32_e64 v212, 0, 1, vcc
+	v_or_b32_e32 v81, v81, v212
+	v_lshrrev_b32_e32 v212, v204, v201
+	v_bitop3_b32 v212, v85, v212, 15 bitop3:0x78
+	v_bfe_i32 v214, v212, 0, 1
+	v_xor_b32_e32 v214, v162, v214
+	v_bfe_i32 v212, v212, 1, 1
+	v_bitop3_b32 v212, v212, v214, v163 bitop3:0xde
+	v_cmp_gt_u32_e32 vcc, 4, v213
+	v_add_u32_e32 v205, v205, v135
+	v_lshlrev_b32_e32 v199, 2, v199
+	v_cndmask_b32_e32 v212, -1, v212, vcc
+	v_cmp_ge_u32_e32 vcc, s5, v89
+	v_lshlrev_b32_e32 v200, 2, v200
+	v_add_u32_e32 v204, v204, v137
+	v_cndmask_b32_e64 v213, 0, 1, vcc
+	v_or_b32_e32 v212, v212, v213
+	v_perm_b32 v213, v212, v81, s33
+	v_perm_b32 v81, v212, v81, s74
+	v_lshlrev_b32_e32 v194, 6, v81
+	v_pk_add_f16 v212, v91, v176
+	v_pk_add_f16 v176, v91, v197
+	v_and_b32_e32 v194, 0x20002000, v194
+	v_lshlrev_b32_e32 v202, 2, v202
+	v_lshlrev_b32_e32 v203, 2, v203
+	v_pk_fma_f16 v158, v194, v92, v158
+	v_pk_maximum3_f16 v176, v176, v195, v195
+	v_pk_add_f16 v195, v91, v196
+	v_lshlrev_b32_e32 v194, 7, v81
+	v_pk_maximum3_f16 v158, v176, v158, v158
+	v_and_b32_e32 v196, 0x20002000, v194
+	v_pk_add_f16 v194, v90, v158
+	v_pk_maximum3_f16 v197, v195, v178, v178
+	v_pk_fma_f16 v157, v196, v92, v157
+	v_pk_add_f16 v178, v91, v194
+	v_pk_add_f16 v192, v91, v192
+	v_pk_maximum3_f16 v157, v197, v157, v194
+	v_lshlrev_b32_e32 v195, 8, v81
+	v_and_b32_e32 v214, 0x20002000, v195
+	v_pk_add_f16 v195, v90, v157
+	v_pk_maximum3_f16 v196, v192, v179, v179
+	v_pk_maximum3_f16 v178, v195, v178, v178
+	v_pk_fma_f16 v156, v214, v92, v156
+	v_pk_add_f16 v179, v91, v178
+	v_pk_add_f16 v191, v91, v191
+	v_pk_maximum3_f16 v156, v196, v156, v178
+	v_lshlrev_b32_e32 v178, 9, v81
+	v_and_b32_e32 v214, 0x20002000, v178
+	v_pk_add_f16 v178, v90, v156
+	v_pk_maximum3_f16 v192, v191, v177, v177
+	v_pk_maximum3_f16 v177, v178, v179, v179
+	v_pk_fma_f16 v155, v214, v92, v155
+	v_pk_add_f16 v214, v91, v177
+	v_pk_add_f16 v190, v91, v190
+	v_pk_maximum3_f16 v155, v192, v155, v177
+	v_lshlrev_b32_e32 v177, 10, v81
+	v_and_b32_e32 v177, 0x20002000, v177
+	v_pk_add_f16 v179, v90, v155
+	v_pk_maximum3_f16 v191, v190, v175, v175
+	v_pk_maximum3_f16 v175, v179, v214, v214
+	v_pk_fma_f16 v154, v177, v92, v154
+	v_pk_add_f16 v214, v91, v175
+	v_pk_add_f16 v189, v91, v189
+	v_pk_maximum3_f16 v154, v191, v154, v175
+	v_lshlrev_b32_e32 v175, 11, v81
+	v_and_b32_e32 v175, 0x20002000, v175
+	v_pk_add_f16 v177, v90, v154
+	v_pk_maximum3_f16 v190, v189, v174, v174
+	v_pk_maximum3_f16 v174, v177, v214, v214
+	v_pk_fma_f16 v153, v175, v92, v153
+	v_pk_add_f16 v214, v91, v174
+	v_pk_add_f16 v188, v91, v188
+	v_pk_maximum3_f16 v153, v190, v153, v174
+	v_lshlrev_b32_e32 v174, 12, v81
+	v_and_b32_e32 v174, 0x20002000, v174
+	v_pk_add_f16 v175, v90, v153
+	v_pk_maximum3_f16 v189, v188, v173, v173
+	v_pk_maximum3_f16 v173, v175, v214, v214
+	v_pk_fma_f16 v152, v174, v92, v152
+	v_pk_add_f16 v214, v91, v173
+	v_pk_add_f16 v187, v91, v187
+	v_pk_maximum3_f16 v152, v189, v152, v173
+	v_lshlrev_b32_e32 v81, 13, v81
+	v_and_b32_e32 v81, 0x20002000, v81
+	v_pk_add_f16 v174, v90, v152
+	v_pk_maximum3_f16 v188, v187, v172, v172
+	v_pk_maximum3_f16 v172, v174, v214, v214
+	v_pk_fma_f16 v81, v81, v92, v151
+	v_pk_add_f16 v214, v91, v172
+	v_pk_add_f16 v186, v91, v186
+	v_pk_maximum3_f16 v151, v188, v81, v172
+	v_lshrrev_b32_e32 v81, 2, v213
+	v_and_b32_e32 v81, 0x20002000, v81
+	v_pk_add_f16 v173, v90, v151
+	v_pk_maximum3_f16 v187, v186, v170, v170
+	v_pk_maximum3_f16 v170, v173, v214, v214
+	v_pk_fma_f16 v81, v81, v92, v150
+	v_pk_add_f16 v214, v91, v170
+	v_pk_add_f16 v184, v91, v184
+	v_pk_maximum3_f16 v150, v187, v81, v170
+	v_lshrrev_b32_e32 v81, 1, v213
+	v_and_b32_e32 v81, 0x20002000, v81
+	v_pk_add_f16 v172, v90, v150
+	v_pk_maximum3_f16 v186, v184, v168, v168
+	v_pk_maximum3_f16 v168, v172, v214, v214
+	v_pk_fma_f16 v81, v81, v92, v149
+	v_pk_add_f16 v214, v91, v168
+	v_pk_add_f16 v182, v91, v182
+	v_pk_maximum3_f16 v149, v186, v81, v168
+	v_and_b32_e32 v81, 0x20002000, v213
+	v_pk_add_f16 v170, v90, v149
+	v_pk_maximum3_f16 v184, v182, v171, v171
+	v_pk_maximum3_f16 v168, v170, v214, v214
+	v_pk_fma_f16 v81, v81, v92, v148
+	v_pk_add_f16 v171, v91, v168
+	v_pk_add_f16 v182, v91, v185
+	v_pk_maximum3_f16 v148, v184, v81, v168
+	v_lshlrev_b32_e32 v81, 1, v213
+	v_and_b32_e32 v81, 0x20002000, v81
+	v_pk_add_f16 v168, v90, v148
+	v_pk_maximum3_f16 v182, v182, v169, v169
+	v_pk_maximum3_f16 v169, v168, v171, v171
+	v_pk_fma_f16 v81, v81, v92, v147
+	v_pk_add_f16 v214, v91, v169
+	v_pk_add_f16 v183, v91, v183
+	v_pk_maximum3_f16 v147, v182, v81, v169
+	v_lshlrev_b32_e32 v81, 2, v213
+	v_and_b32_e32 v81, 0x20002000, v81
+	v_pk_add_f16 v171, v90, v147
+	v_pk_maximum3_f16 v185, v183, v167, v167
+	v_pk_maximum3_f16 v167, v171, v214, v214
+	v_pk_fma_f16 v81, v81, v92, v146
+	v_pk_add_f16 v214, v91, v167
+	v_pk_add_f16 v181, v91, v181
+	v_pk_maximum3_f16 v146, v185, v81, v167
+	v_lshlrev_b32_e32 v81, 3, v213
+	v_and_b32_e32 v81, 0x20002000, v81
+	v_pk_add_f16 v169, v90, v146
+	v_pk_maximum3_f16 v183, v181, v166, v166
+	v_pk_maximum3_f16 v166, v169, v214, v214
+	v_pk_fma_f16 v81, v81, v92, v145
+	v_pk_add_f16 v214, v91, v166
+	v_pk_add_f16 v180, v91, v180
+	v_pk_maximum3_f16 v145, v183, v81, v166
+	v_lshlrev_b32_e32 v81, 4, v213
+	v_and_b32_e32 v81, 0x20002000, v81
+	v_pk_add_f16 v167, v90, v145
+	v_pk_maximum3_f16 v181, v180, v165, v165
+	v_pk_maximum3_f16 v165, v167, v214, v214
+	v_pk_fma_f16 v81, v81, v92, v144
+	v_pk_add_f16 v214, v91, v165
+	v_pk_add_f16 v180, v91, v193
+	v_pk_maximum3_f16 v144, v181, v81, v165
+	v_lshlrev_b32_e32 v81, 5, v213
+	v_and_b32_e32 v81, 0x20002000, v81
+	v_pk_add_f16 v166, v90, v144
+	v_pk_maximum3_f16 v180, v180, v164, v164
+	v_pk_maximum3_f16 v164, v166, v214, v214
+	v_pk_fma_f16 v81, v81, v92, v143
+	v_pk_add_f16 v193, v91, v164
+	v_pk_maximum3_f16 v143, v180, v81, v164
+	v_lshlrev_b32_e32 v81, 6, v213
+	v_and_b32_e32 v81, 0x20002000, v81
+	v_pk_add_f16 v165, v90, v143
+	s_nop 0
+	v_pk_maximum3_f16 v164, v165, v193, v193
+	v_pk_fma_f16 v81, v81, v92, v142
+	v_pk_add_f16 v193, v91, v164
+	v_pk_maximum3_f16 v142, v81, v164, v164
+	s_nop 0
+	v_pk_add_f16 v164, v90, v142
+	s_nop 0
+	v_pk_maximum3_f16 v81, v164, v193, v193
+	s_nop 0
+	v_pk_maximum3_f16 v11, v11, v212, v81
+	s_add_i32 s4, s4, 1
+	v_cmp_ge_u32_e32 vcc, s4, v211
+	s_or_b64 s[36:37], vcc, s[36:37]
+	v_mov_b32_e32 v193, 0xf400f400
+	s_andn2_b64 exec, exec, s[36:37]
+	s_cbranch_execnz .LBB236_651
+	s_or_b64 exec, exec, s[36:37]
+	v_mov_b32_e32 v193, 0xf400f400
+	s_branch .LBB236_638
```
